# lihzha/lap

Hardware: AMD Instinct MI355X
Metric: train-step samples/sec LAP-3B bf16 (higher is better)
Workload: dtype bf16; 1 GPU; LAP-3B (SigLIP So400m/14 + Gemma-2B + Gemma-300M expert) full train step fwd+bwd+AdamW+EMA, 2x224x224 images + 48-token prompt + 50-step action chunk, random-init weights; global_batch=32, per_gpu_batch=32, seq_len=610, parallelism=single

## Files before the change

include/lap_hip.h:

```cpp
#ifndef LAP_HIP_H_
#define LAP_HIP_H_
#include <stdint.h>

#ifdef __cplusplus
extern "C" {
#endif

#define LAP_ABI_VERSION 1
int lap_abi_version(void);

#define LAP_GEMM_OUT_F32  1
#define LAP_GEMM_ACCUM    2
#define LAP_GEMM_GELU     4
#define LAP_GEMM_BIAS_F32 8
#define LAP_GEMM_GELU_BF16 32
#define LAP_GEMM_GELU_EXP2 128
#define LAP_GEMM_GEGLU    64
#define LAP_GEMM_PARTIALS 16

int lap_gemm_bf16(const void* A, const void* B, void* C, const void* bias, const void* residual,
                  int M, int N, int K, int lda, int ldb, int ldc, int ldr, float alpha,
                  int a_kc, int b_kc, int flags, void* stream);

int lap_gemm_asm_ok(int a_kc, int b_kc, int out_f32, int M, int N, int K, int lda, int ldb, int ldc);
int lap_gemm_asm(const void* A, const void* B, void* C, int M, int N, int K, int lda, int ldb, int ldc, int a_kc, int b_kc,
                 int out_f32, void* stream);
int lap_gemm_asm_bias_ok(int M, int N, int K, int lda, int ldb, int ldc);
int lap_gemm_asm_bias(const void* A, const void* B, void* C, const float* bias, int M, int N, int K, int lda, int ldb, int ldc,
                      void* stream);
int lap_gemm_asm_res_ok(int biased, int M, int N, int K, int lda, int ldb, int ldc);
int lap_gemm_asm_res(const void* A, const void* B, void* C, const float* bias, const void* residual, int M, int N, int K,
                     int lda, int ldb, int ldc, void* stream);
int lap_gemm_asm_geglu_bwd_ok(int M, int N, int K, int lda, int ldb, int ld);
int lap_gemm_asm_geglu_bwd(const void* dy, const void* W, void* dgu, const void* gu, int M, int N, int K, int lda, int ldb, int ld,
                           void* stream);
int lap_gemm_asm_geglu_fwd_ok(int M, int N, int K, int lda, int ldb, int ld_gu, int ld_act);
int lap_gemm_asm_geglu_fwd(const void* x, const void* W, void* gu, void* act, int M, int N, int K, int lda, int ldb, int ld_gu,
                           int ld_act, void* stream);
int lap_gemm_asm_wgrad(const void* A, const void* B, void* C, int M, int N, int K, int lda, int ldb, int ldc, float* sumsq, void* stream);
int lap_gemm_wgrad_f32(const void* A, const void* B, void* C, int M, int N, int K, int lda, int ldb, int ldc, float* sumsq, int* folded,
                       void* scratch, long long scratch_bytes, void* stream);
int lap_gemm_asm_wgrad_b16(const void* A, const void* B, void* C, int M, int N, int K, int lda, int ldb, int ldc, float* sumsq, void* stream);
int lap_gemm_wgrad_bf16(const void* A, const void* B, void* C, int M, int N, int K, int lda, int ldb, int ldc, float* sumsq, int* folded,
                        void* scratch, long long scratch_bytes, void* stream);
int lap_gemm_asm_bias_gelu(const void* x, const void* W, void* h, void* a, const float* bias, int M, int N, int K, int lda, int ldb,
                           int ldc, void* stream);
int lap_gemm_asm_gelu_bwd(const void* dy, const void* W, void* dh, const void* h, int M, int N, int K, int lda, int ldb, int ld,
                          void* stream);

int lap_gemm_asm_launch_counts(long long* counts, int n);
#define LAP_ROUTE_NO_ASM           1
#define LAP_ROUTE_NO_ASM_NN        2
#define LAP_ROUTE_NO_ASM_RES       4
#define LAP_ROUTE_NO_MSPLIT        8
#define LAP_ROUTE_NO_MSPLIT_LONGK  16
#define LAP_ROUTE_NO_NSPLIT        32
#define LAP_ROUTE_NO_SERVING_TILES 64
#define LAP_ROUTE_NO_PINGPONG      128
#define LAP_ROUTE_NO_KTAIL         256
#define LAP_ROUTE_WGRAD_SUMSQ      65536
#define LAP_LEG_ASM             32
#define LAP_LEG_ASM_BIAS        33
#define LAP_LEG_ASM_RES         34
#define LAP_LEG_ASM_WGRAD_SUMSQ 35
#define LAP_LEG_REDUCE_NONE   0
#define LAP_LEG_REDUCE_SPLITK 1
#define LAP_LEG_REDUCE_TAIL   2
#define LAP_GEMM_MAX_LEGS 6
typedef struct lap_gemm_leg {
  long long off_a, off_b, off_c, off_bias, off_res;
  int engine, M, N;
  int ksplit, tile_base, tile_count, sub256, part_compact;
  int f32_tile;
  int part;
  int reduce;
} lap_gemm_leg;
int lap_gemm_plan(const void* A, const void* B, const void* C, const void* bias, const void* residual,
                  int M, int N, int K, int lda, int ldb, int ldc, int ldr, float alpha,
                  int a_kc, int b_kc, int flags, int tile, int ksplit, const void* scratch, long long scratch_bytes,
                  unsigned switches, lap_gemm_leg* legs, int max_legs, int* n_legs);
int lap_gemm_set_debug(int bits);

int lap_gemm_bf16_ex(const void* A, const void* B, void* C, const void* bias, const void* residual,
                     int M, int N, int K, int lda, int ldb, int ldc, int ldr, float alpha,
                     int a_kc, int b_kc, int flags, int tile, int ksplit, void* scratch, long long scratch_bytes,
                     void* stream);

int lap_gemm_f32(const float* A, const float* B, float* C, const float* bias,
                 int M, int N, int K, int lda, int ldb, int ldc, float alpha,
                 int a_kc, int b_kc, int accum, void* stream);

int lap_rmsnorm_fwd(const void* x, const float* scale, const void* mod, void* y, float* rstd,
                    int rows, int D, int rows_per_sample, int mod_ld, float eps, void* stream);
int lap_rmsnorm_bwd(const void* x, const float* scale, const void* mod, const float* rstd, const void* dy,
                    void* dx, float* dscale, float* dmod,
                    int rows, int D, int rows_per_sample, int mod_ld, int dmod_ld, int accum_dx, void* stream);

int lap_layernorm_fwd(const void* x, const float* gamma, const float* beta, void* y, float* mean, float* rstd,
                      int rows, int D, float eps, void* stream);
int lap_layernorm_bwd(const void* x, const float* gamma, const float* mean, const float* rstd, const void* dy,
                      void* dx, float* dgamma, float* dbeta, int rows, int D, int accum_dx, void* stream);
int lap_layernorm_bwd_sum(const void* x, const float* gamma, const float* mean, const float* rstd, const void* dy,
                          void* dx, float* dgamma, float* dbeta, float* dxsum, int rows, int D, int accum_dx, void* stream);

int lap_rope_split_fwd(const void* qkv, const int32_t* pos, void* q, void* k, void* v,
                       int B, int T_seg, int T_total, int seg_off, int NH, int HD, float q_scale, void* stream);
int lap_rope_split_bwd(const void* dq, const void* dk, const void* dv, const int32_t* pos, void* dqkv,
                       int B, int T_seg, int T_total, int seg_off, int NH, int HD, float q_scale, void* stream);

int lap_geglu_fwd(const void* gu, void* act, int rows, int H, void* stream);
int lap_geglu_bwd(const void* gu, const void* dact, void* dgu, int rows, int H, void* stream);
int lap_geglu_fwd_ld(const void* gu, void* act, int rows, int H, int ld_gu, int ld_act, void* stream);
int lap_geglu_bwd_ld(const void* gu, const void* dact, void* dgu, int rows, int H, int ld_gu, int ld_dact, int ld_dgu, void* stream);
int lap_gelu_fwd(const void* x, void* y, long long n, void* stream);
int lap_gelu_bwd(const void* x, const void* dy, void* dx, long long n, void* stream);

int lap_embed_gather(const float* table, const int32_t* tok, void* out, int rows, int T, int D,
                     int dst_rows_per_sample, int dst_off, float scale, int row_lo, int row_hi, void* stream);
int lap_embed_scatter_add(float* dtable, const int32_t* tok, const void* dout, int rows, int T, int D,
                          int src_rows_per_sample, int src_off, float scale, void* stream);

int lap_gated_residual_fwd(const void* x, const void* u, const void* gate, void* y,
                           int rows, int D, int rows_per_sample, int ldg, void* stream);
int lap_gated_residual_bwd(const void* dy, const void* u, const void* gate, void* du, float* dgate,
                           int rows, int D, int rows_per_sample, int ldg, int ldg_out, void* stream);

int lap_colsum_bf16(const void* x, float* out, int rows, int cols, int ld, void* stream);
int lap_colsum_f32(const float* x, float* out, int rows, int cols, int ld, void* stream);

int lap_cast_f32_to_bf16(const float* x, void* y, long long n, void* stream);
int lap_split_f32_hilo(const float* x, int rows, int cols, int ld, void* hi, void* lo, int ld_out, void* stream);
int lap_cast_bf16_to_f32(const void* x, float* y, long long n, void* stream);
int lap_add_bf16(const void* a, const void* b, void* y, long long n, void* stream);
int lap_copy2d_bf16(const void* src, void* dst, int rows, int cols, int lds, int ldd, void* stream);
int lap_copy_rows_bf16(const void* src, void* dst, int rows, int T, int D,
                       int src_rps, int src_off, int dst_rps, int dst_off, int accumulate, void* stream);

int lap_im2col_patch(const float* img, float* out, int B, int H, int W, int C, int P, void* stream);
int lap_augment_images(const float* img, float* out, const float* params, int B, int H, int W, void* stream);
int lap_add_posemb_cast(const float* x, const float* pos, void* y, int rows, int T, int D, void* stream);
int lap_add_posemb_cast_bwd(const void* dy, float* dx, float* dpos, int rows, int T, int D, void* stream);

typedef struct {
  const void* q[2]; void* o[2];
  const void* k[2]; const void* v[2];
  int q_len[2]; int k_len[2];
  int q_rs[2]; int kv_rs[2]; int o_rs[2];
  const int32_t* qinfo; const int32_t* kinfo;
  float* lse;
  float* scratch;
  long long scratch_floats;
  float scale;
  int nsplit;
  int B, NH, NKV, HD;
} lap_attn_fwd_args;
int lap_attention_fwd(const lap_attn_fwd_args* a, void* stream);
int lap_attention_serve_splits(int k_len0, int k_len1, int B, int NH, int q_len1);
int lap_attention_serve(const lap_attn_fwd_args* a, void* stream);

#define LAP_CHAIN_MAX_DEPTH 32
typedef struct {
  int depth, B, S, D, H, NH, HD, prefix_len;
  const void* x_in; void* x_out;
  const void* mod; int mod_slot_stride;
  const void* wqkv[LAP_CHAIN_MAX_DEPTH]; const void* wo[LAP_CHAIN_MAX_DEPTH];
  const void* wgu[LAP_CHAIN_MAX_DEPTH]; const void* wd[LAP_CHAIN_MAX_DEPTH];
  const void* cache_k[LAP_CHAIN_MAX_DEPTH]; const void* cache_v[LAP_CHAIN_MAX_DEPTH];
  int kv_rs;
  const float* rope_table; const int32_t* qinfo; const int32_t* kinfo;
  float q_scale, eps;
  void *q, *k, *v, *o, *xa, *act;
  float* attn_scratch; long long attn_scratch_floats;
  unsigned* counters;
  void* debug_clock;
  int packed;
  void* xs;
  float* tp_slabs;
  void *tp_xs, *tp_xn;
  void *tp_k, *tp_v;
} lap_serve_chain_args;
int lap_serve_chain_ok(int B, int S, int D, int H, int NH, int HD, int NKV, int prefix_len);
int lap_serve_chain_tp_ok(int B, int S, int D, int H, int NH, int HD, int NKV, int prefix_len);
int lap_serve_chain_counter_words(void);
int lap_serve_chain_status(const unsigned* counters, int* status);
int lap_serve_chain(const lap_serve_chain_args* a, void* stream);
int lap_serve_pack_weight(const void* w, void* out, int N, int K, int kind, int HD, void* stream);

typedef struct {
  const void* q[2]; const void* o[2]; const void* d_o[2];
  const void* k[2]; const void* v[2];
  void* dq[2]; void* dk[2]; void* dv[2];
  int q_len[2]; int k_len[2];
  int q_rs[2]; int kv_rs[2]; int o_rs[2];
  const int32_t* qinfo; const int32_t* kinfo;
  const float* lse;
  float* delta;
  float* scratch;
  long long scratch_floats;
  float scale;
  int hsplit;
  int B, NH, NKV, HD;
  int stop_q1_to_k0;
} lap_attn_bwd_args;
int lap_attention_bwd(const lap_attn_bwd_args* a, void* stream);
int lap_attention_set_variant(int variant);

int lap_gemm_fp8(const void* A8, const void* B8, void* C, const void* residual, const float* scale_a, const float* scale_b,
                 int M, int N, int K, int lda, int ldb, int ldc, int ldr, float alpha, int flags, void* stream);
int lap_amax_bf16(const void* x, long long rows, int cols, long long ld, float* amax, void* stream);
int lap_quantize_fp8(const void* x, long long rows, int cols, long long ld, const float* amax, void* out8, long long ldo,
                     float* scale, void* stream);
int lap_quantize_fp8_weight(const void* w, int rows, int cols, const float* amax, void* out8, void* out8_t, float* scale,
                            void* stream);

int lap_serve_qkv_rope(const void* x, const void* mod, int mod_ld, int rows_per_sample, const void* wqkv,
                       const float* rope_table, void* q, void* k, void* v, int M, int D, int NH, int HD, float q_scale,
                       float eps, void* stream);
int lap_serve_gate_up(const void* x, const void* mod, int mod_ld, int rows_per_sample, const void* wgu, void* act, int M,
                      int D, int H, float eps, void* stream);
// ... 125 lines not shown
```

lap_amd/csrc/elementwise.hip:

```cpp
#include <cstdlib>

#include "common.hpp"
#include "../../include/lap_hip.h"

namespace {

__device__ __forceinline__ void ld8(const bf16* p, float (&v)[8]) {
  bf16x8 t = *reinterpret_cast<const bf16x8*>(p);
#pragma unroll
  for (int e = 0; e < 8; ++e) v[e] = (float)t[e];
}
__device__ __forceinline__ void st8(bf16* p, const float (&v)[8]) {
  bf16x8 t;
#pragma unroll
  for (int e = 0; e < 8; ++e) t[e] = f2bf(v[e]);
  *reinterpret_cast<bf16x8*>(p) = t;
}

template <bool NT>
__device__ __forceinline__ void ld8s(const bf16* p, float (&v)[8]) {
  bf16x8 t = NT ? __builtin_nontemporal_load(reinterpret_cast<const bf16x8*>(p)) : *reinterpret_cast<const bf16x8*>(p);
#pragma unroll
  for (int e = 0; e < 8; ++e) v[e] = (float)t[e];
}
template <bool NT>
__device__ __forceinline__ void st8s(bf16* p, const float (&v)[8]) {
  bf16x8 t;
#pragma unroll
  for (int e = 0; e < 8; ++e) t[e] = f2bf(v[e]);
  if (NT) __builtin_nontemporal_store(t, reinterpret_cast<bf16x8*>(p));
  else *reinterpret_cast<bf16x8*>(p) = t;
}

inline bool stream_nt() {
  static const bool nt = getenv("LAP_STREAM_NT") ? atoi(getenv("LAP_STREAM_NT")) != 0 : true;
  return nt;
}

inline dim3 flat_grid(long long n, int per_block = 256) { return dim3((unsigned)((n + per_block - 1) / per_block)); }

template <bool BWD, bool HSPLIT = false>
__global__ __launch_bounds__(256) void rope_split_kernel(const bf16* __restrict__ a0, const bf16* __restrict__ a1,
                                                         const bf16* __restrict__ a2, const int32_t* __restrict__ pos,
                                                         bf16* __restrict__ o0, bf16* __restrict__ o1,
                                                         bf16* __restrict__ o2, int rows, int T_seg, int T_total,
                                                         int seg_off, int NH, int HD, float q_scale) {
  const int cph = HD / 16;
  long long gid = (long long)blockIdx.x * 256 + threadIdx.x;
  int h_lo = 0, h_hi = NH + 2;
  if (HSPLIT) {
    if (gid >= (long long)rows * cph * (NH + 2)) return;
    h_lo = (int)(gid % (NH + 2)); h_hi = h_lo + 1;
    gid /= (NH + 2);
  } else if (gid >= (long long)rows * cph) {
    return;
  }
  const int row = (int)(gid / cph);
  const int c = (int)(gid % cph);
  const int b = row / T_seg, t = row % T_seg;
  const int W = (NH + 2) * HD;
  const int half = HD / 2;
  const float p = (float)pos[(long long)b * T_total + seg_off + t];
  float sn[8], cs[8];
#pragma unroll
  for (int e = 0; e < 8; ++e) rope_sincos(p, c * 8 + e, HD, sn[e], cs[e]);
#pragma unroll 2
  for (int h = h_lo; h < h_hi; ++h) {
    const bf16* src;
    if (!BWD) src = a0 + (long long)row * W + h * HD;
    else if (h < NH) src = a0 + (long long)row * NH * HD + h * HD;
    else if (h == NH) src = a1 + (long long)row * HD;
    else src = a2 + (long long)row * HD;
    float x1[8], x2[8], y1[8], y2[8];
    ld8(src + c * 8, x1);
    ld8(src + half + c * 8, x2);
    if (h <= NH) {
#pragma unroll
      for (int e = 0; e < 8; ++e) {
        if (!BWD) {
          float r1, r2;
          rope_rotate(x1[e], x2[e], sn[e], cs[e], r1, r2);
          r1 = round_bf16((r1)); r2 = round_bf16((r2));
          if (h < NH) { r1 *= q_scale; r2 *= q_scale; }
          y1[e] = r1; y2[e] = r2;
        } else {
          float d1 = x1[e], d2 = x2[e];
          if (h < NH) { d1 *= q_scale; d2 *= q_scale; }
          rope_rotate(d1, d2, -sn[e], cs[e], y1[e], y2[e]);
        }
      }
    } else {
#pragma unroll
      for (int e = 0; e < 8; ++e) { y1[e] = x1[e]; y2[e] = x2[e]; }
    }
    bf16* dst;
    if (BWD) dst = o0 + (long long)row * W + h * HD;
    else if (h < NH) dst = o0 + (long long)row * NH * HD + h * HD;
    else if (h == NH) dst = o1 + (long long)row * HD;
    else dst = o2 + (long long)row * HD;
    st8(dst + c * 8, y1);
    st8(dst + half + c * 8, y2);
  }
}

template <bool NT>
__global__ __launch_bounds__(256) void geglu_fwd_kernel(const bf16* __restrict__ gu, bf16* __restrict__ act,
                                                        long long nchunk, int H8, long long ld_gu, long long ld_act) {
  const long long gid = (long long)blockIdx.x * 256 + threadIdx.x;
  if (gid >= nchunk) return;
  const long long row = gid / H8;
  const int c = (int)(gid % H8) * 8;
  const long long H = (long long)H8 * 8;
  float g[8], u[8], o[8];
  ld8s<NT>(gu + row * ld_gu + c, g);
  ld8s<NT>(gu + row * ld_gu + H + c, u);
#pragma unroll
  for (int e = 0; e < 8; ++e) o[e] = round_bf16((gelu_tanh_f(g[e]))) * u[e];
  st8s<NT>(act + row * ld_act + c, o);
}
template <bool NT>
__global__ __launch_bounds__(256) void geglu_bwd_kernel(const bf16* __restrict__ gu, const bf16* __restrict__ dact,
                                                        bf16* __restrict__ dgu, long long nchunk, int H8, long long ld_gu,
                                                        long long ld_act, long long ld_dgu) {
  const long long gid = (long long)blockIdx.x * 256 + threadIdx.x;
  if (gid >= nchunk) return;
  const long long row = gid / H8;
  const int c = (int)(gid % H8) * 8;
  const long long H = (long long)H8 * 8;
  float g[8], u[8], d[8], dg[8], du[8];
  ld8s<NT>(gu + row * ld_gu + c, g);
  ld8s<NT>(gu + row * ld_gu + H + c, u);
  ld8s<NT>(dact + row * ld_act + c, d);
#pragma unroll
  for (int e = 0; e < 8; ++e) {
    dg[e] = d[e] * u[e] * gelu_tanh_grad_f(g[e]);
    du[e] = d[e] * round_bf16((gelu_tanh_f(g[e])));
  }
  st8s<NT>(dgu + row * ld_dgu + c, dg);
  st8s<NT>(dgu + row * ld_dgu + H + c, du);
}

template <bool NT>
__global__ __launch_bounds__(256) void gelu_fwd_kernel(const bf16* __restrict__ x, bf16* __restrict__ y, long long n8) {
  const long long gid = (long long)blockIdx.x * 256 + threadIdx.x;
  if (gid >= n8) return;
  float v[8];
  ld8s<NT>(x + gid * 8, v);
#pragma unroll
  for (int e = 0; e < 8; ++e) v[e] = gelu_tanh_f(v[e]);
  st8s<NT>(y + gid * 8, v);
}
template <bool NT>
__global__ __launch_bounds__(256) void gelu_bwd_kernel(const bf16* __restrict__ x, const bf16* __restrict__ dy,
                                                       bf16* __restrict__ dx, long long n8) {
  const long long gid = (long long)blockIdx.x * 256 + threadIdx.x;
  if (gid >= n8) return;
  float v[8], d[8];
  ld8s<NT>(x + gid * 8, v);
  ld8s<NT>(dy + gid * 8, d);
#pragma unroll
  for (int e = 0; e < 8; ++e) d[e] *= gelu_tanh_grad_f(v[e]);
  st8s<NT>(dx + gid * 8, d);
}

__global__ __launch_bounds__(256) void embed_gather_kernel(const float* __restrict__ table, const int32_t* __restrict__ tok,
                                                           bf16* __restrict__ out, int rows, int T, int D8,
                                                           int dst_rps, int dst_off, float scale, int row_lo, int row_hi) {
  const long long gid = (long long)blockIdx.x * 256 + threadIdx.x;
  if (gid >= (long long)rows * D8) return;
  const int r = (int)(gid / D8), c = (int)(gid % D8) * 8;
  const long long D = (long long)D8 * 8;
  const int t = tok[r];
  float o[8] = {0.f, 0.f, 0.f, 0.f, 0.f, 0.f, 0.f, 0.f};
  if (t >= row_lo && t < row_hi) {
    const float* src = table + (long long)(t - row_lo) * D + c;
    f32x4 a = *reinterpret_cast<const f32x4*>(src), b = *reinterpret_cast<const f32x4*>(src + 4);
#pragma unroll
    for (int e = 0; e < 4; ++e) { o[e] = a[e] * scale; o[4 + e] = b[e] * scale; }
  }
  const long long drow = (long long)(r / T) * dst_rps + dst_off + r % T;
// ... 69 lines not shown
        if (t < rps) {
          const long long r = (long long)b * rps + t;
          float o[8];
#pragma unroll
          for (int e = 0; e < 8; ++e) { const float d = (float)dv[i][e]; o[e] = d * gv[e]; acc[e] += d * (float)uv[i][e]; }
          st8(du + r * D + c, o);
        }
      }
    }
  }
#pragma unroll
  for (int e = 0; e < 8; ++e) part[rl][cl][e] = acc[e];
  __syncthreads();
  if (rl == 0 && live) {
#pragma unroll
    for (int e = 0; e < 8; ++e) {
      float t = 0.f;
#pragma unroll
      for (int j = 0; j < 8; ++j) t += part[j][cl][e];
      dgate[(long long)b * ldg_out + c + e] = t;
    }
  }
}

__global__ __launch_bounds__(256) void cast_f32_bf16_kernel(const float* __restrict__ x, bf16* __restrict__ y, long long n) {
  const long long i = ((long long)blockIdx.x * 256 + threadIdx.x) * 8;
  if (i + 8 <= n) {
    f32x4 a = *reinterpret_cast<const f32x4*>(x + i), b = *reinterpret_cast<const f32x4*>(x + i + 4);
    float o[8] = {a[0], a[1], a[2], a[3], b[0], b[1], b[2], b[3]};
    st8(y + i, o);
  } else {
    for (long long j = i; j < n; ++j) y[j] = f2bf(x[j]);
  }
}
__global__ __launch_bounds__(256) void split_hilo_kernel(const float* __restrict__ x, int rows, int cols, int ld,
                                                         bf16* __restrict__ hi, bf16* __restrict__ lo, int ld_out) {
  const int cpr = ld_out / 8;
  const long long gid = (long long)blockIdx.x * 256 + threadIdx.x;
  if (gid >= (long long)rows * cpr) return;
  const int r = (int)(gid / cpr), c0 = (int)(gid % cpr) * 8;
  float h[8], l[8];
#pragma unroll
  for (int e = 0; e < 8; ++e) {
    const float v = (c0 + e < cols) ? x[(long long)r * ld + c0 + e] : 0.f;
    h[e] = round_bf16(v);
    l[e] = v - h[e];
  }
  st8(hi + (long long)r * ld_out + c0, h);
  st8(lo + (long long)r * ld_out + c0, l);
}
__global__ __launch_bounds__(256) void cast_bf16_f32_kernel(const bf16* __restrict__ x, float* __restrict__ y, long long n) {
  const long long i = ((long long)blockIdx.x * 256 + threadIdx.x) * 8;
  if (i + 8 <= n) {
    float v[8];
    ld8(x + i, v);
    *reinterpret_cast<f32x4*>(y + i) = f32x4{v[0], v[1], v[2], v[3]};
    *reinterpret_cast<f32x4*>(y + i + 4) = f32x4{v[4], v[5], v[6], v[7]};
  } else {
    for (long long j = i; j < n; ++j) y[j] = bf2f(x[j]);
  }
}
__global__ __launch_bounds__(256) void add_bf16_kernel(const bf16* __restrict__ a, const bf16* __restrict__ b,
                                                       bf16* __restrict__ y, long long n) {
  const long long i = ((long long)blockIdx.x * 256 + threadIdx.x) * 8;
  if (i + 8 <= n) {
    float u[8], v[8];
    ld8(a + i, u); ld8(b + i, v);
#pragma unroll
    for (int e = 0; e < 8; ++e) u[e] += v[e];
    st8(y + i, u);
  } else {
    for (long long j = i; j < n; ++j) y[j] = f2bf(bf2f(a[j]) + bf2f(b[j]));
  }
}
__global__ __launch_bounds__(256) void copy2d_kernel(const bf16* __restrict__ src, bf16* __restrict__ dst, int rows,
                                                     int cols8, int lds_, int ldd) {
  const long long gid = (long long)blockIdx.x * 256 + threadIdx.x;
  if (gid >= (long long)rows * cols8) return;
  const int r = (int)(gid / cols8), c = (int)(gid % cols8) * 8;
  *reinterpret_cast<bf16x8*>(dst + (long long)r * ldd + c) = *reinterpret_cast<const bf16x8*>(src + (long long)r * lds_ + c);
}
__global__ __launch_bounds__(256) void copy_rows_kernel(const bf16* __restrict__ src, bf16* __restrict__ dst, int rows,
                                                        int T, int D8, int src_rps, int src_off, int dst_rps,
                                                        int dst_off, int accumulate) {
  const long long gid = (long long)blockIdx.x * 256 + threadIdx.x;
  if (gid >= (long long)rows * D8) return;
  const int r = (int)(gid / D8), c = (int)(gid % D8) * 8;
  const long long D = (long long)D8 * 8;
  const long long srow = (long long)(r / T) * src_rps + src_off + r % T;
  const long long drow = (long long)(r / T) * dst_rps + dst_off + r % T;
  if (accumulate) {
    float a[8], b[8];
    ld8(src + srow * D + c, a);
    ld8(dst + drow * D + c, b);
#pragma unroll
    for (int e = 0; e < 8; ++e) a[e] += b[e];
    st8(dst + drow * D + c, a);
  } else {
    *reinterpret_cast<bf16x8*>(dst + drow * D + c) = *reinterpret_cast<const bf16x8*>(src + srow * D + c);
  }
}

constexpr int CS_ROWS = 256;
template <typename T>
__global__ __launch_bounds__(256) void colsum_kernel(const T* __restrict__ x, float* __restrict__ out, int rows, int cols,
                                                     int ld) {
  __shared__ float red[4][512];
  const int lane = threadIdx.x & 63, w = threadIdx.x >> 6;
  const int c0 = blockIdx.x * 512 + lane * 8;
  const int r0 = blockIdx.y * CS_ROWS, r1 = min(rows, r0 + CS_ROWS);
  float acc[8] = {0.f, 0.f, 0.f, 0.f, 0.f, 0.f, 0.f, 0.f};
  const bool vec = (c0 + 8 <= cols) && ((ld * (int)sizeof(T)) % 16 == 0) && ((((uintptr_t)x) & 15) == 0) && (c0 * (int)sizeof(T)) % 16 == 0;
  if (vec) {
    for (int r = r0 + w; r < r1; r += 32) {
      if constexpr (sizeof(T) == 2) {
        bf16x8 v[8];
#pragma unroll
        for (int u = 0; u < 8; ++u) {
          const int rr = r + 4 * u;
          v[u] = rr < r1 ? *reinterpret_cast<const bf16x8*>(x + (long long)rr * ld + c0) : bf16x8{0, 0, 0, 0, 0, 0, 0, 0};
        }
#pragma unroll
        for (int u = 0; u < 8; ++u)
#pragma unroll
          for (int e = 0; e < 8; ++e) acc[e] += (float)v[u][e];
      } else {
        f32x4 a[8], b[8];
#pragma unroll
        for (int u = 0; u < 8; ++u) {
          const int rr = r + 4 * u;
          const bool ok = rr < r1;
          a[u] = ok ? *reinterpret_cast<const f32x4*>(x + (long long)rr * ld + c0) : f32x4{0.f, 0.f, 0.f, 0.f};
          b[u] = ok ? *reinterpret_cast<const f32x4*>(x + (long long)rr * ld + c0 + 4) : f32x4{0.f, 0.f, 0.f, 0.f};
        }
#pragma unroll
        for (int u = 0; u < 8; ++u)
#pragma unroll
          for (int e = 0; e < 4; ++e) { acc[e] += a[u][e]; acc[4 + e] += b[u][e]; }
      }
    }
  } else {
    for (int r = r0 + w; r < r1; r += 4) {
      const T* row = x + (long long)r * ld;
#pragma unroll
      for (int e = 0; e < 8; ++e)
        if (c0 + e < cols) acc[e] += (float)row[c0 + e];
    }
  }
#pragma unroll
  for (int e = 0; e < 8; ++e) red[w][lane * 8 + e] = acc[e];
  __syncthreads();
  for (int c = threadIdx.x; c < 512; c += 256) {
    const int col = blockIdx.x * 512 + c;
    if (col < cols) atomicAdd(out + col, red[0][c] + red[1][c] + red[2][c] + red[3][c]);
  }
}

__global__ __launch_bounds__(256) void im2col_kernel(const float* __restrict__ img, float* __restrict__ out, int B, int H,
                                                     int W, int C, int P) {
  const int GH = H / P, GW = W / P;
  const int PC = P * C;
  const long long total = (long long)B * GH * GW * P * PC;
  const long long gid = (long long)blockIdx.x * 256 + threadIdx.x;
  if (gid >= total) return;
  const int x = (int)(gid % PC);
  long long t = gid / PC;
  const int ph = (int)(t % P); t /= P;
  const int gw = (int)(t % GW); t /= GW;
  const int gh = (int)(t % GH);
  const int b = (int)(t / GH);
  out[gid] = img[(((long long)b * H + gh * P + ph) * W + gw * P) * C + x];
}
// ... 77 lines not shown
  const float cf = coef ? coef[b] : 0.f;
  float acc = 0.f;
  for (int i = threadIdx.x; i < n_per; i += 256) {
    const float d = v[(long long)b * n_per + i] - u[(long long)b * n_per + i];
    acc += d * d;
    if (dv) dv[(long long)b * n_per + i] = cf * 2.0f * d / (float)n_per;
  }
  acc = block_sum<4>(acc, red);
  if (threadIdx.x == 0) per_sample[b] = acc / (float)n_per;
}
__global__ __launch_bounds__(256) void axpy_kernel(float* __restrict__ x, const float* __restrict__ v, float dt, long long n) {
  const long long i = (long long)blockIdx.x * 256 + threadIdx.x;
  if (i < n) x[i] += dt * v[i];
}

__device__ __forceinline__ float aug_brightness(float v, float b) { return b < 0.f ? v * (1.f + b) : v * (1.f - b) + b; }
__device__ __forceinline__ float aug_contrast(float v, float c) {
  const float slant = tanf((c + 1.f) * 0.78539816339744831f);
  if (fabsf(slant - 1.f) < 1e-6f) return v;
  const float p1 = (slant - slant * slant) / (2.f * (1.f - slant * slant)), p2 = 1.f - p1;
  if (v < p1) return v / slant;
  if (v > p2) return v / slant + 1.f - 1.f / slant;
  return slant * (v - 0.5f) + 0.5f;
}
__global__ __launch_bounds__(256) void augment_kernel(const float* __restrict__ img, float* __restrict__ out,
                                                      const float* __restrict__ par, int B, int H, int W) {
  const long long gid = (long long)blockIdx.x * 256 + threadIdx.x;
  if (gid >= (long long)B * H * W) return;
  const int x = (int)(gid % W), y = (int)((gid / W) % H), b = (int)(gid / ((long long)W * H));
  const float* q = par + b * 12;
  const float* src = img + (long long)b * H * W * 3;
  float* dst = out + gid * 3;
  if (q[9] != 0.f) {
    const float* s3 = src + ((long long)y * W + x) * 3;
    dst[0] = s3[0]; dst[1] = s3[1]; dst[2] = s3[2];
    return;
  }
  const float xc = (float)x + 0.5f - 0.5f * (float)W, yc = (float)y + 0.5f - 0.5f * (float)H;
  const float xr = q[4] * xc - q[5] * yc, yr = q[5] * xc + q[4] * yc;
  const float xs = q[0] + 0.5f * q[2] + xr * (q[2] / (float)W) - 0.5f;
  const float ys = q[1] + 0.5f * q[3] + yr * (q[3] / (float)H) - 0.5f;
  const float xf = floorf(xs), yf = floorf(ys);
  const int x0 = (int)xf, y0 = (int)yf;
  const float ax = xs - xf, ay = ys - yf;
  float px[3] = {0.f, 0.f, 0.f};
#pragma unroll
  for (int dy = 0; dy < 2; ++dy)
#pragma unroll
    for (int dx = 0; dx < 2; ++dx) {
      const int xx = x0 + dx, yy = y0 + dy;
      if (xx < 0 || xx >= W || yy < 0 || yy >= H) continue;
      const float wgt = (dx ? ax : 1.f - ax) * (dy ? ay : 1.f - ay);
      const float* s3 = src + ((long long)yy * W + xx) * 3;
#pragma unroll
      for (int c = 0; c < 3; ++c) px[c] += wgt * (s3[c] * 0.5f + 0.5f);
    }
  float r = px[0], g = px[1], bl = px[2];
  r = aug_brightness(r, q[6]); g = aug_brightness(g, q[6]); bl = aug_brightness(bl, q[6]);
  r = aug_contrast(r, q[7]); g = aug_contrast(g, q[7]); bl = aug_contrast(bl, q[7]);
  {
    const float mx = fmaxf(r, fmaxf(g, bl)), mn = fminf(r, fminf(g, bl));
    const float sat = mx > 0.f ? (mx - mn) / mx : 0.f;
    const float s2 = fminf(fmaxf(aug_brightness(sat, q[8]), 0.f), 1.f);
    const float k = sat > 0.f ? s2 / sat : 0.f;
    r = mx - (mx - r) * k; g = mx - (mx - g) * k; bl = mx - (mx - bl) * k;
  }
  dst[0] = fminf(fmaxf(r, 0.f), 1.f) * 2.f - 1.f;
  dst[1] = fminf(fmaxf(g, 0.f), 1.f) * 2.f - 1.f;
  dst[2] = fminf(fmaxf(bl, 0.f), 1.f) * 2.f - 1.f;
}

}

#define S_ ((hipStream_t)stream)

extern "C" int lap_abi_version(void) { return LAP_ABI_VERSION; }

extern "C" int lap_rope_split_fwd(const void* qkv, const int32_t* pos, void* q, void* k, void* v, int B, int T_seg,
                                  int T_total, int seg_off, int NH, int HD, float q_scale, void* stream) {
  if (B <= 0 || T_seg <= 0 || (HD & 15) || NH <= 0) return LAP_ERR_ARG;
  const long long n = (long long)B * T_seg * (HD / 16);
  if (n < 65536)
    hipLaunchKernelGGL((rope_split_kernel<false, true>), flat_grid(n * (NH + 2)), dim3(256), 0, S_, (const bf16*)qkv, nullptr, nullptr, pos,
                       (bf16*)q, (bf16*)k, (bf16*)v, B * T_seg, T_seg, T_total, seg_off, NH, HD, q_scale);
  else
    hipLaunchKernelGGL(rope_split_kernel<false>, flat_grid(n), dim3(256), 0, S_, (const bf16*)qkv, nullptr, nullptr, pos,
                       (bf16*)q, (bf16*)k, (bf16*)v, B * T_seg, T_seg, T_total, seg_off, NH, HD, q_scale);
  LAP_CHECK_LAUNCH();
  return LAP_OK;
}
extern "C" int lap_rope_split_bwd(const void* dq, const void* dk, const void* dv, const int32_t* pos, void* dqkv, int B,
                                  int T_seg, int T_total, int seg_off, int NH, int HD, float q_scale, void* stream) {
  if (B <= 0 || T_seg <= 0 || (HD & 15) || NH <= 0) return LAP_ERR_ARG;
  const long long n = (long long)B * T_seg * (HD / 16);
  hipLaunchKernelGGL(rope_split_kernel<true>, flat_grid(n), dim3(256), 0, S_, (const bf16*)dq, (const bf16*)dk,
                     (const bf16*)dv, pos, (bf16*)dqkv, nullptr, nullptr, B * T_seg, T_seg, T_total, seg_off, NH, HD,
                     q_scale);
  LAP_CHECK_LAUNCH();
  return LAP_OK;
}

extern "C" int lap_geglu_fwd_ld(const void* gu, void* act, int rows, int H, int ld_gu, int ld_act, void* stream) {
  if (rows <= 0 || H <= 0 || (H & 7) || ld_gu < 2 * H || ld_act < H || (ld_gu & 7) || (ld_act & 7)) return LAP_ERR_ARG;
  const long long n = (long long)rows * (H / 8);
  const bool nt = stream_nt();
  if (nt) hipLaunchKernelGGL(geglu_fwd_kernel<true>, flat_grid(n), dim3(256), 0, S_, (const bf16*)gu, (bf16*)act, n, H / 8, (long long)ld_gu, (long long)ld_act);
  else hipLaunchKernelGGL(geglu_fwd_kernel<false>, flat_grid(n), dim3(256), 0, S_, (const bf16*)gu, (bf16*)act, n, H / 8, (long long)ld_gu, (long long)ld_act);
  LAP_CHECK_LAUNCH();
  return LAP_OK;
}
extern "C" int lap_geglu_fwd(const void* gu, void* act, int rows, int H, void* stream) {
  return lap_geglu_fwd_ld(gu, act, rows, H, 2 * H, H, stream);
}
extern "C" int lap_geglu_bwd_ld(const void* gu, const void* dact, void* dgu, int rows, int H, int ld_gu, int ld_dact, int ld_dgu, void* stream) {
  if (rows <= 0 || H <= 0 || (H & 7) || ld_gu < 2 * H || ld_dact < H || ld_dgu < 2 * H || ((ld_gu | ld_dact | ld_dgu) & 7)) return LAP_ERR_ARG;
  const long long n = (long long)rows * (H / 8);
  const bool nt = stream_nt();
  if (nt) hipLaunchKernelGGL(geglu_bwd_kernel<true>, flat_grid(n), dim3(256), 0, S_, (const bf16*)gu, (const bf16*)dact, (bf16*)dgu, n,
                             H / 8, (long long)ld_gu, (long long)ld_dact, (long long)ld_dgu);
  else hipLaunchKernelGGL(geglu_bwd_kernel<false>, flat_grid(n), dim3(256), 0, S_, (const bf16*)gu, (const bf16*)dact, (bf16*)dgu, n,
                          H / 8, (long long)ld_gu, (long long)ld_dact, (long long)ld_dgu);
  LAP_CHECK_LAUNCH();
  return LAP_OK;
}
extern "C" int lap_geglu_bwd(const void* gu, const void* dact, void* dgu, int rows, int H, void* stream) {
  return lap_geglu_bwd_ld(gu, dact, dgu, rows, H, 2 * H, H, 2 * H, stream);
}
extern "C" int lap_gelu_fwd(const void* x, void* y, long long n, void* stream) {
  if (n <= 0 || (n & 7)) return LAP_ERR_ARG;
  if (stream_nt()) hipLaunchKernelGGL(gelu_fwd_kernel<true>, flat_grid(n / 8), dim3(256), 0, S_, (const bf16*)x, (bf16*)y, n / 8);
  else hipLaunchKernelGGL(gelu_fwd_kernel<false>, flat_grid(n / 8), dim3(256), 0, S_, (const bf16*)x, (bf16*)y, n / 8);
  LAP_CHECK_LAUNCH();
  return LAP_OK;
}
extern "C" int lap_gelu_bwd(const void* x, const void* dy, void* dx, long long n, void* stream) {
  if (n <= 0 || (n & 7)) return LAP_ERR_ARG;
  if (stream_nt()) hipLaunchKernelGGL(gelu_bwd_kernel<true>, flat_grid(n / 8), dim3(256), 0, S_, (const bf16*)x, (const bf16*)dy, (bf16*)dx, n / 8);
  else hipLaunchKernelGGL(gelu_bwd_kernel<false>, flat_grid(n / 8), dim3(256), 0, S_, (const bf16*)x, (const bf16*)dy, (bf16*)dx, n / 8);
  LAP_CHECK_LAUNCH();
  return LAP_OK;
}

extern "C" int lap_embed_gather(const float* table, const int32_t* tok, void* out, int rows, int T, int D,
                                int dst_rows_per_sample, int dst_off, float scale, int row_lo, int row_hi, void* stream) {
  if (rows <= 0 || T <= 0 || (D & 7) || row_hi < row_lo) return LAP_ERR_ARG;
  hipLaunchKernelGGL(embed_gather_kernel, flat_grid((long long)rows * (D / 8)), dim3(256), 0, S_, table, tok, (bf16*)out,
                     rows, T, D / 8, dst_rows_per_sample, dst_off, scale, row_lo, row_hi);
  LAP_CHECK_LAUNCH();
  return LAP_OK;
}
extern "C" int lap_embed_scatter_add(float* dtable, const int32_t* tok, const void* dout, int rows, int T, int D,
                                     int src_rows_per_sample, int src_off, float scale, void* stream) {
  if (rows <= 0 || T <= 0 || (D & 7)) return LAP_ERR_ARG;
  hipLaunchKernelGGL(embed_scatter_kernel, flat_grid((long long)rows * (D / 8)), dim3(256), 0, S_, dtable, tok,
                     (const bf16*)dout, rows, T, D / 8, src_rows_per_sample, src_off, scale);
  LAP_CHECK_LAUNCH();
  return LAP_OK;
}

extern "C" int lap_gated_residual_fwd(const void* x, const void* u, const void* gate, void* y, int rows, int D,
                                      int rows_per_sample, int ldg, void* stream) {
  if (rows <= 0 || (D & 7) || (gate && (rows_per_sample <= 0 || (ldg & 7)))) return LAP_ERR_ARG;
  hipLaunchKernelGGL(gated_res_fwd_kernel, flat_grid((long long)rows * (D / 8)), dim3(256), 0, S_, (const bf16*)x,
                     (const bf16*)u, (const bf16*)gate, (bf16*)y, rows, D / 8, rows_per_sample > 0 ? rows_per_sample : 1,
                     ldg);
  LAP_CHECK_LAUNCH();
  return LAP_OK;
}
extern "C" int lap_gated_residual_bwd(const void* dy, const void* u, const void* gate, void* du, float* dgate, int rows,
                                      int D, int rows_per_sample, int ldg, int ldg_out, void* stream) {
  if (rows <= 0 || (D & 7) || !gate || rows_per_sample <= 0 || rows % rows_per_sample || (ldg & 7)) return LAP_ERR_ARG;
  dim3 grid((D / 8 + 31) / 32, rows / rows_per_sample);
  hipLaunchKernelGGL(gated_res_bwd_kernel, grid, dim3(256), 0, S_, (const bf16*)dy, (const bf16*)u, (const bf16*)gate,
                     (bf16*)du, dgate, D / 8, rows_per_sample, ldg, ldg_out);
  LAP_CHECK_LAUNCH();
  return LAP_OK;
}

extern "C" int lap_colsum_bf16(const void* x, float* out, int rows, int cols, int ld, void* stream) {
  if (rows <= 0 || cols <= 0) return LAP_ERR_ARG;
  hipLaunchKernelGGL(colsum_kernel<bf16>, dim3((cols + 511) / 512, (rows + CS_ROWS - 1) / CS_ROWS), dim3(256), 0, S_, (const bf16*)x,
                     out, rows, cols, ld);
  LAP_CHECK_LAUNCH();
  return LAP_OK;
}
extern "C" int lap_colsum_f32(const float* x, float* out, int rows, int cols, int ld, void* stream) {
  if (rows <= 0 || cols <= 0) return LAP_ERR_ARG;
  hipLaunchKernelGGL(colsum_kernel<float>, dim3((cols + 511) / 512, (rows + CS_ROWS - 1) / CS_ROWS), dim3(256), 0, S_, x, out, rows,
                     cols, ld);
  LAP_CHECK_LAUNCH();
  return LAP_OK;
}

extern "C" int lap_cast_f32_to_bf16(const float* x, void* y, long long n, void* stream) {
  if (n <= 0) return LAP_ERR_ARG;
  hipLaunchKernelGGL(cast_f32_bf16_kernel, flat_grid((n + 7) / 8), dim3(256), 0, S_, x, (bf16*)y, n);
  LAP_CHECK_LAUNCH();
  return LAP_OK;
}
extern "C" int lap_split_f32_hilo(const float* x, int rows, int cols, int ld, void* hi, void* lo, int ld_out, void* stream) {
  if (rows <= 0 || cols <= 0 || ld < cols || ld_out < cols || (ld_out & 7) || !x || !hi || !lo) return LAP_ERR_ARG;
  hipLaunchKernelGGL(split_hilo_kernel, flat_grid((long long)rows * (ld_out / 8)), dim3(256), 0, S_, x, rows, cols, ld, (bf16*)hi,
                     (bf16*)lo, ld_out);
  LAP_CHECK_LAUNCH();
  return LAP_OK;
}
extern "C" int lap_cast_bf16_to_f32(const void* x, float* y, long long n, void* stream) {
  if (n <= 0) return LAP_ERR_ARG;
  hipLaunchKernelGGL(cast_bf16_f32_kernel, flat_grid((n + 7) / 8), dim3(256), 0, S_, (const bf16*)x, y, n);
  LAP_CHECK_LAUNCH();
  return LAP_OK;
}
extern "C" int lap_add_bf16(const void* a, const void* b, void* y, long long n, void* stream) {
  if (n <= 0) return LAP_ERR_ARG;
  hipLaunchKernelGGL(add_bf16_kernel, flat_grid((n + 7) / 8), dim3(256), 0, S_, (const bf16*)a, (const bf16*)b, (bf16*)y,
                     n);
  LAP_CHECK_LAUNCH();
  return LAP_OK;
}
extern "C" int lap_copy2d_bf16(const void* src, void* dst, int rows, int cols, int lds, int ldd, void* stream) {
  if (rows <= 0 || cols <= 0 || (cols & 7) || (lds & 7) || (ldd & 7)) return LAP_ERR_ARG;
  hipLaunchKernelGGL(copy2d_kernel, flat_grid((long long)rows * (cols / 8)), dim3(256), 0, S_, (const bf16*)src,
                     (bf16*)dst, rows, cols / 8, lds, ldd);
  LAP_CHECK_LAUNCH();
  return LAP_OK;
}
extern "C" int lap_copy_rows_bf16(const void* src, void* dst, int rows, int T, int D, int src_rps, int src_off,
                                  int dst_rps, int dst_off, int accumulate, void* stream) {
  if (rows <= 0 || T <= 0 || (D & 7)) return LAP_ERR_ARG;
  hipLaunchKernelGGL(copy_rows_kernel, flat_grid((long long)rows * (D / 8)), dim3(256), 0, S_, (const bf16*)src,
                     (bf16*)dst, rows, T, D / 8, src_rps, src_off, dst_rps, dst_off, accumulate);
  LAP_CHECK_LAUNCH();
  return LAP_OK;
}

extern "C" int lap_im2col_patch(const float* img, float* out, int B, int H, int W, int C, int P, void* stream) {
  if (B <= 0 || P <= 0 || H % P || W % P) return LAP_ERR_ARG;
  const long long n = (long long)B * H * W * C;
  hipLaunchKernelGGL(im2col_kernel, flat_grid(n), dim3(256), 0, S_, img, out, B, H, W, C, P);
  LAP_CHECK_LAUNCH();
  return LAP_OK;
}
extern "C" int lap_augment_images(const float* img, float* out, const float* params, int B, int H, int W, void* stream) {
  if (!img || !out || !params || img == out || B <= 0 || H <= 0 || W <= 0) return LAP_ERR_ARG;
  hipLaunchKernelGGL(augment_kernel, flat_grid((long long)B * H * W), dim3(256), 0, S_, img, out, params, B, H, W);
  LAP_CHECK_LAUNCH();
  return LAP_OK;
}
extern "C" int lap_add_posemb_cast(const float* x, const float* pos, void* y, int rows, int T, int D, void* stream) {
  if (rows <= 0 || T <= 0 || (D & 7)) return LAP_ERR_ARG;
  hipLaunchKernelGGL(add_posemb_cast_kernel, flat_grid((long long)rows * (D / 8)), dim3(256), 0, S_, x, pos, (bf16*)y,
                     rows, T, D / 8);
  LAP_CHECK_LAUNCH();
  return LAP_OK;
}
extern "C" int lap_add_posemb_cast_bwd(const void* dy, float* dx, float* dpos, int rows, int T, int D, void* stream) {
  if (rows <= 0 || T <= 0 || rows % T || (D & 7)) return LAP_ERR_ARG;
  dim3 grid((D / 8 + 255) / 256, T);
  hipLaunchKernelGGL(add_posemb_cast_bwd_kernel, grid, dim3(256), 0, S_, (const bf16*)dy, dx, dpos, rows / T, T, D / 8);
  LAP_CHECK_LAUNCH();
  return LAP_OK;
}

extern "C" int lap_fm_mix(const float* noise, const float* actions, const float* t, float* x_t, float* u_t, int B,
                          int n_per, void* stream) {
  if (B <= 0 || n_per <= 0) return LAP_ERR_ARG;
  hipLaunchKernelGGL(fm_mix_kernel, flat_grid((long long)B * n_per), dim3(256), 0, S_, noise, actions, t, x_t, u_t, B,
                     n_per);
  LAP_CHECK_LAUNCH();
  return LAP_OK;
}
extern "C" int lap_posemb_sincos(const float* t, float* out, int B, int D, float min_period, float max_period,
                                 void* stream) {
  if (B <= 0 || D <= 0 || (D & 1)) return LAP_ERR_ARG;
  hipLaunchKernelGGL(posemb_sincos_kernel, flat_grid((long long)B * (D / 2)), dim3(256), 0, S_, t, out, B, D, min_period,
                     max_period);
  LAP_CHECK_LAUNCH();
  return LAP_OK;
}
extern "C" int lap_swish_fwd(const float* x, float* y, long long n, void* stream) {
  if (n <= 0) return LAP_ERR_ARG;
  hipLaunchKernelGGL(swish_fwd_kernel, flat_grid(n), dim3(256), 0, S_, x, y, n);
  LAP_CHECK_LAUNCH();
  return LAP_OK;
}
extern "C" int lap_swish_bwd(const float* x, const float* dy, float* dx, long long n, void* stream) {
  if (n <= 0) return LAP_ERR_ARG;
  hipLaunchKernelGGL(swish_bwd_kernel, flat_grid(n), dim3(256), 0, S_, x, dy, dx, n);
  LAP_CHECK_LAUNCH();
  return LAP_OK;
}
extern "C" int lap_mse_fwd_bwd(const float* v, const float* u, const float* coef, float* per_sample, float* dv, int B,
                               int n_per, void* stream) {
  if (B <= 0 || n_per <= 0) return LAP_ERR_ARG;
  hipLaunchKernelGGL(mse_kernel, dim3(B), dim3(256), 0, S_, v, u, coef, per_sample, dv, n_per);
  LAP_CHECK_LAUNCH();
  return LAP_OK;
}
extern "C" int lap_axpy_f32(float* x, const float* v, float dt, long long n, void* stream) {
  if (n <= 0) return LAP_ERR_ARG;
  hipLaunchKernelGGL(axpy_kernel, flat_grid(n), dim3(256), 0, S_, x, v, dt, n);
  LAP_CHECK_LAUNCH();
  return LAP_OK;
}
```

lap_amd/csrc/norm.hip:

```cpp
#include <cstdlib>

#include "common.hpp"
#include "../../include/lap_hip.h"

namespace {

constexpr int NWAVE = 4;

__device__ __forceinline__ void load8(const bf16* p, float (&v)[8]) {
  bf16x8 t = *reinterpret_cast<const bf16x8*>(p);
#pragma unroll
  for (int e = 0; e < 8; ++e) v[e] = (float)t[e];
}
__device__ __forceinline__ void store8(bf16* p, const float (&v)[8]) {
  bf16x8 t;
#pragma unroll
  for (int e = 0; e < 8; ++e) t[e] = f2bf(v[e]);
  *reinterpret_cast<bf16x8*>(p) = t;
}

template <int NCH>
__global__ __launch_bounds__(256) void rmsnorm_fwd_kernel(const bf16* __restrict__ x, const float* __restrict__ scale,
                                                          const bf16* __restrict__ mod, bf16* __restrict__ y,
                                                          float* __restrict__ rstd_out, int rows, int D,
                                                          int rows_per_sample, int mod_ld, float eps) {
  const int lane = threadIdx.x & 63, w = threadIdx.x >> 6;
  const int row = blockIdx.x * NWAVE + w;
  if (row >= rows) return;
  const bf16* xr = x + (long long)row * D;
  float xv[NCH][8];
  float ss = 0.f;
#pragma unroll
  for (int p = 0; p < NCH; ++p) {
    const int c = (lane + 64 * p) * 8;
    if (c < D) {
      load8(xr + c, xv[p]);
#pragma unroll
      for (int e = 0; e < 8; ++e) ss += xv[p][e] * xv[p][e];
    }
  }
  ss = wave_sum(ss);
  const float r = 1.0f / sqrtf(ss / (float)D + eps);
  if (rstd_out && lane == 0) rstd_out[row] = r;
  const bf16* mrow = mod ? mod + (long long)(row / rows_per_sample) * mod_ld : nullptr;
  bf16* yr = y + (long long)row * D;
#pragma unroll
  for (int p = 0; p < NCH; ++p) {
    const int c = (lane + 64 * p) * 8;
    if (c < D) {
      float o[8];
      if (mrow) {
        float sc[8], sh[8];
        load8(mrow + c, sc);
        load8(mrow + D + c, sh);
#pragma unroll
        for (int e = 0; e < 8; ++e) o[e] = xv[p][e] * r * round_bf16((1.0f + sc[e])) + sh[e];
      } else {
#pragma unroll
        for (int e = 0; e < 8; ++e) o[e] = xv[p][e] * r * (1.0f + scale[c + e]);
      }
      store8(yr + c, o);
    }
  }
}

template <int NCH>
__global__ __launch_bounds__(256) void rmsnorm_bwd_kernel(const bf16* __restrict__ x, const float* __restrict__ scale,
                                                          const bf16* __restrict__ mod, const float* __restrict__ rstd,
                                                          const bf16* __restrict__ dy, bf16* __restrict__ dx,
                                                          float* __restrict__ dscale, float* __restrict__ dmod,
                                                          int rows, int D, int G, int mod_ld, int dmod_ld,
                                                          int accum_dx) {
  extern __shared__ __attribute__((aligned(16))) float red[];
  const int lane = threadIdx.x & 63, w = threadIdx.x >> 6;
  const int g = blockIdx.x;
  const int r0 = g * G, r1 = min(rows, r0 + G);
  const bool ada = mod != nullptr;
  const bf16* mrow = ada ? mod + (long long)g * mod_ld : nullptr;

  float wgt[NCH][8];
  float ds[NCH][8], dh[NCH][8];
#pragma unroll
  for (int p = 0; p < NCH; ++p) {
    const int c = (lane + 64 * p) * 8;
#pragma unroll
    for (int e = 0; e < 8; ++e) { ds[p][e] = 0.f; dh[p][e] = 0.f; wgt[p][e] = 0.f; }
    if (c < D) {
      if (ada) {
        float sc[8];
        load8(mrow + c, sc);
#pragma unroll
        for (int e = 0; e < 8; ++e) wgt[p][e] = round_bf16((1.0f + sc[e]));
      } else {
#pragma unroll
        for (int e = 0; e < 8; ++e) wgt[p][e] = 1.0f + scale[c + e];
      }
    }
  }
  bf16x8 nx[NCH], ndy[NCH];
  float nr = 0.f;
  auto fetch = [&](int row) {
#pragma unroll
    for (int p = 0; p < NCH; ++p) {
      const int c = (lane + 64 * p) * 8;
      if (c < D) {
        nx[p] = *reinterpret_cast<const bf16x8*>(x + (long long)row * D + c);
        ndy[p] = *reinterpret_cast<const bf16x8*>(dy + (long long)row * D + c);
      }
    }
    nr = rstd[row];
  };
  if (r0 + w < r1) fetch(r0 + w);
  for (int row = r0 + w; row < r1; row += NWAVE) {
    bf16x8 cx[NCH], cdy[NCH], cold[NCH];
#pragma unroll
    for (int p = 0; p < NCH; ++p) {
      cx[p] = nx[p]; cdy[p] = ndy[p];
      const int c = (lane + 64 * p) * 8;
      if (NCH <= 3 && accum_dx && c < D) cold[p] = *reinterpret_cast<const bf16x8*>(dx + (long long)row * D + c);
    }
    const float r = nr;
    if (row + NWAVE < r1) fetch(row + NWAVE);
    float xv[NCH][8], gv[NCH][8];
    float dot = 0.f;
#pragma unroll
    for (int p = 0; p < NCH; ++p) {
      const int c = (lane + 64 * p) * 8;
      if (c < D) {
        float dyv[8];
#pragma unroll
        for (int e = 0; e < 8; ++e) { xv[p][e] = (float)cx[p][e]; dyv[e] = (float)cdy[p][e]; }
#pragma unroll
        for (int e = 0; e < 8; ++e) {
          gv[p][e] = dyv[e] * wgt[p][e];
          dot += gv[p][e] * xv[p][e];
          ds[p][e] += dyv[e] * xv[p][e] * r;
          dh[p][e] += dyv[e];
        }
      }
    }
    dot = wave_sum(dot);
    const float cc = dot * r * r * r / (float)D;
    bf16* dxr = dx + (long long)row * D;
#pragma unroll
    for (int p = 0; p < NCH; ++p) {
      const int c = (lane + 64 * p) * 8;
      if (c < D) {
        float o[8];
#pragma unroll
        for (int e = 0; e < 8; ++e) o[e] = r * gv[p][e] - xv[p][e] * cc;
        if (accum_dx) {
          if constexpr (NCH > 3) cold[p] = *reinterpret_cast<const bf16x8*>(dxr + c);
#pragma unroll
          for (int e = 0; e < 8; ++e) o[e] += (float)cold[p][e];
        }
        store8(dxr + c, o);
      }
    }
  }
  const int stride = ada ? 2 * D : D;
#pragma unroll
  for (int p = 0; p < NCH; ++p) {
    const int c = (lane + 64 * p) * 8;
    if (c < D) {
#pragma unroll
      for (int e = 0; e < 8; ++e) {
        red[w * stride + c + e] = ds[p][e];
        if (ada) red[w * stride + D + c + e] = dh[p][e];
      }
    }
  }
  __syncthreads();
  for (int c = threadIdx.x; c < stride; c += 256) {
    float t = 0.f;
#pragma unroll
    for (int i = 0; i < NWAVE; ++i) t += red[i * stride + c];
    if (ada) {
      atomicAdd(dmod + (long long)g * dmod_ld + c, t);
    } else {
      atomicAdd(dscale + c, t);
    }
  }
}

template <int NCH>
__global__ __launch_bounds__(256) void layernorm_fwd_kernel(const bf16* __restrict__ x, const float* __restrict__ gamma,
                                                            const float* __restrict__ beta, bf16* __restrict__ y,
                                                            float* __restrict__ mean_out, float* __restrict__ rstd_out,
                                                            int rows, int D, float eps) {
  const int lane = threadIdx.x & 63, w = threadIdx.x >> 6;
  const int row = blockIdx.x * NWAVE + w;
  if (row >= rows) return;
  const bf16* xr = x + (long long)row * D;
  float xv[NCH][8];
  float s = 0.f, ss = 0.f;
#pragma unroll
  for (int p = 0; p < NCH; ++p) {
    const int c = (lane + 64 * p) * 8;
    if (c < D) {
      load8(xr + c, xv[p]);
#pragma unroll
      for (int e = 0; e < 8; ++e) { s += xv[p][e]; ss += xv[p][e] * xv[p][e]; }
    }
  }
  s = wave_sum(s);
  ss = wave_sum(ss);
  const float mean = s / (float)D;
  const float var = fmaxf(ss / (float)D - mean * mean, 0.f);
  const float r = 1.0f / sqrtf(var + eps);
  if (lane == 0) {
    if (mean_out) mean_out[row] = mean;
    if (rstd_out) rstd_out[row] = r;
  }
  bf16* yr = y + (long long)row * D;
#pragma unroll
  for (int p = 0; p < NCH; ++p) {
    const int c = (lane + 64 * p) * 8;
    if (c < D) {
      float o[8];
#pragma unroll
      for (int e = 0; e < 8; ++e) o[e] = (xv[p][e] - mean) * (r * gamma[c + e]) + beta[c + e];
      store8(yr + c, o);
    }
  }
}

template <int NCH>
__global__ __launch_bounds__(256) void layernorm_bwd_kernel(const bf16* __restrict__ x, const float* __restrict__ gamma,
                                                            const float* __restrict__ mean, const float* __restrict__ rstd,
                                                            const bf16* __restrict__ dy, bf16* __restrict__ dx,
                                                            float* __restrict__ dgamma, float* __restrict__ dbeta,
                                                            int rows, int D, int G, int accum_dx, float* __restrict__ dxsum) {
  extern __shared__ __attribute__((aligned(16))) float red[];
  const int lane = threadIdx.x & 63, w = threadIdx.x >> 6;
  const int r0 = blockIdx.x * G, r1 = min(rows, r0 + G);
// ... 52 lines not shown
    s2 = wave_sum(s2) / (float)D;
    bf16* dxr = dx + (long long)row * D;
#pragma unroll
    for (int p = 0; p < NCH; ++p) {
      const int c = (lane + 64 * p) * 8;
      if (c < D) {
        float o[8];
#pragma unroll
        for (int e = 0; e < 8; ++e) o[e] = r * (gv[p][e] - s1 - xh[p][e] * s2);
        if (accum_dx) {
          if constexpr (NCH > 3) cold[p] = *reinterpret_cast<const bf16x8*>(dxr + c);
#pragma unroll
          for (int e = 0; e < 8; ++e) o[e] += (float)cold[p][e];
        }
        store8(dxr + c, o);
        if (dxsum) {
#pragma unroll
          for (int e = 0; e < 8; ++e) dxs[p][e] += (float)f2bf(o[e]);
        }
      }
    }
  }
  const int NS = dxsum ? 3 : 2;
#pragma unroll
  for (int p = 0; p < NCH; ++p) {
    const int c = (lane + 64 * p) * 8;
    if (c < D) {
#pragma unroll
      for (int e = 0; e < 8; ++e) {
        red[w * NS * D + c + e] = dg[p][e];
        red[w * NS * D + D + c + e] = db[p][e];
        if (dxsum) red[w * NS * D + 2 * D + c + e] = dxs[p][e];
      }
    }
  }
  __syncthreads();
  for (int c = threadIdx.x; c < NS * D; c += 256) {
    float t = 0.f;
#pragma unroll
    for (int i = 0; i < NWAVE; ++i) t += red[i * NS * D + c];
    if (c < D) atomicAdd(dgamma + c, t);
    else if (c < 2 * D) atomicAdd(dbeta + (c - D), t);
    else atomicAdd(dxsum + (c - 2 * D), t);
  }
}

inline int nch_for(int D) { return (D / 8 + 63) / 64; }

}

#define DISPATCH_NCH(D, CALL)                          \
  switch (nch_for(D)) {                                \
    case 1: { constexpr int NCH = 1; CALL; } break;    \
    case 2: { constexpr int NCH = 2; CALL; } break;    \
    case 3: { constexpr int NCH = 3; CALL; } break;    \
    case 4: { constexpr int NCH = 4; CALL; } break;    \
    default: return LAP_ERR_ARG;                       \
  }

extern "C" int lap_rmsnorm_fwd(const void* x, const float* scale, const void* mod, void* y, float* rstd,
                               int rows, int D, int rows_per_sample, int mod_ld, float eps, void* stream) {
  if (rows <= 0 || D <= 0 || (D & 7) || (!scale && !mod) || (mod && (rows_per_sample <= 0 || (mod_ld & 7) || (mod_ld != 0 && mod_ld < 3 * D))))
    return LAP_ERR_ARG;
  hipStream_t s = (hipStream_t)stream;
  dim3 grid((rows + NWAVE - 1) / NWAVE);
  DISPATCH_NCH(D, hipLaunchKernelGGL(rmsnorm_fwd_kernel<NCH>, grid, dim3(256), 0, s, (const bf16*)x, scale,
                                     (const bf16*)mod, (bf16*)y, rstd, rows, D, rows_per_sample, mod_ld, eps));
  LAP_CHECK_LAUNCH();
  return LAP_OK;
}

extern "C" int lap_rmsnorm_bwd(const void* x, const float* scale, const void* mod, const float* rstd, const void* dy,
                               void* dx, float* dscale, float* dmod, int rows, int D, int rows_per_sample,
                               int mod_ld, int dmod_ld, int accum_dx, void* stream) {
  if (rows <= 0 || D <= 0 || (D & 7) || !rstd) return LAP_ERR_ARG;
  if (mod ? (!dmod || rows_per_sample <= 0 || rows % rows_per_sample) : (!scale || !dscale)) return LAP_ERR_ARG;
  hipStream_t s = (hipStream_t)stream;
  static const int g_env = getenv("LAP_NORM_BWD_ROWS") ? atoi(getenv("LAP_NORM_BWD_ROWS")) : 64;
  const int G = mod ? rows_per_sample : g_env;
  dim3 grid((rows + G - 1) / G);
  const size_t shm = (size_t)NWAVE * (mod ? 2 : 1) * D * sizeof(float);
  DISPATCH_NCH(D, hipLaunchKernelGGL(rmsnorm_bwd_kernel<NCH>, grid, dim3(256), shm, s, (const bf16*)x, scale,
                                     (const bf16*)mod, rstd, (const bf16*)dy, (bf16*)dx, dscale, dmod, rows, D, G,
                                     mod_ld, dmod_ld, accum_dx));
  LAP_CHECK_LAUNCH();
  return LAP_OK;
}

extern "C" int lap_layernorm_fwd(const void* x, const float* gamma, const float* beta, void* y, float* mean,
                                 float* rstd, int rows, int D, float eps, void* stream) {
  if (rows <= 0 || D <= 0 || (D & 7) || !gamma || !beta) return LAP_ERR_ARG;
  hipStream_t s = (hipStream_t)stream;
  dim3 grid((rows + NWAVE - 1) / NWAVE);
  DISPATCH_NCH(D, hipLaunchKernelGGL(layernorm_fwd_kernel<NCH>, grid, dim3(256), 0, s, (const bf16*)x, gamma, beta,
                                     (bf16*)y, mean, rstd, rows, D, eps));
  LAP_CHECK_LAUNCH();
  return LAP_OK;
}

extern "C" int lap_layernorm_bwd_sum(const void* x, const float* gamma, const float* mean, const float* rstd,
                                     const void* dy, void* dx, float* dgamma, float* dbeta, float* dxsum, int rows, int D,
                                     int accum_dx, void* stream) {
  if (rows <= 0 || D <= 0 || (D & 7) || !gamma || !mean || !rstd || !dgamma || !dbeta) return LAP_ERR_ARG;
  hipStream_t s = (hipStream_t)stream;
  static const int g_env = getenv("LAP_NORM_BWD_ROWS") ? atoi(getenv("LAP_NORM_BWD_ROWS")) : 32;
  const int G = g_env;
  dim3 grid((rows + G - 1) / G);
  const size_t shm = (size_t)NWAVE * (dxsum ? 3 : 2) * D * sizeof(float);
  if (shm > 64 * 1024) return LAP_ERR_ARG;
  DISPATCH_NCH(D, hipLaunchKernelGGL(layernorm_bwd_kernel<NCH>, grid, dim3(256), shm, s, (const bf16*)x, gamma, mean,
                                     rstd, (const bf16*)dy, (bf16*)dx, dgamma, dbeta, rows, D, G, accum_dx, dxsum));
  LAP_CHECK_LAUNCH();
  return LAP_OK;
}
extern "C" int lap_layernorm_bwd(const void* x, const float* gamma, const float* mean, const float* rstd,
                                 const void* dy, void* dx, float* dgamma, float* dbeta, int rows, int D, int accum_dx,
                                 void* stream) {
  return lap_layernorm_bwd_sum(x, gamma, mean, rstd, dy, dx, dgamma, dbeta, nullptr, rows, D, accum_dx, stream);
}
```

lap_amd/hip.py:

```python
from __future__ import annotations

import ctypes as C
import pathlib

import torch

import os as _os

_LIB_PATH = pathlib.Path(__file__).resolve().parent / (
    f"liblap_hip_{_os.environ['LAP_HIP_LIB_VARIANT']}.so" if _os.environ.get("LAP_HIP_LIB_VARIANT") else "liblap_hip.so")

GEMM_OUT_F32 = 1
GEMM_ACCUM = 2
GEMM_GELU = 4
GEMM_BIAS_F32 = 8
GEMM_PARTIALS = 16
GEMM_GELU_BF16 = 32
GEMM_GELU_EXP2 = 128
GEMM_GEGLU = 64


class LapHipError(RuntimeError):
    pass

# ... 19 lines not shown
        ("q_rs", _i * 2), ("kv_rs", _i * 2), ("o_rs", _i * 2),
        ("qinfo", _vp), ("kinfo", _vp), ("lse", _vp),
        ("scratch", _vp), ("scratch_floats", _ll),
        ("scale", _f), ("nsplit", _i),
        ("B", _i), ("NH", _i), ("NKV", _i), ("HD", _i),
    ]


CHAIN_MAX_DEPTH = 32


class ServeChainArgs(C.Structure):
    _fields_ = [
        ("depth", _i), ("B", _i), ("S", _i), ("D", _i), ("H", _i), ("NH", _i), ("HD", _i), ("prefix_len", _i),
        ("x_in", _vp), ("x_out", _vp),
        ("mod", _vp), ("mod_slot_stride", _i),
        ("wqkv", _vp * CHAIN_MAX_DEPTH), ("wo", _vp * CHAIN_MAX_DEPTH), ("wgu", _vp * CHAIN_MAX_DEPTH), ("wd", _vp * CHAIN_MAX_DEPTH),
        ("cache_k", _vp * CHAIN_MAX_DEPTH), ("cache_v", _vp * CHAIN_MAX_DEPTH),
        ("kv_rs", _i),
        ("rope_table", _vp), ("qinfo", _vp), ("kinfo", _vp),
        ("q_scale", _f), ("eps", _f),
        ("q", _vp), ("k", _vp), ("v", _vp), ("o", _vp), ("xa", _vp), ("act", _vp),
        ("attn_scratch", _vp), ("attn_scratch_floats", _ll),
        ("counters", _vp), ("debug_clock", _vp),
        ("packed", _i), ("xs", _vp),
        ("tp_slabs", _vp), ("tp_xs", _vp), ("tp_xn", _vp), ("tp_k", _vp), ("tp_v", _vp),
    ]


class AttnBwdArgs(C.Structure):
    _fields_ = [
        ("q", _vp * 2), ("o", _vp * 2), ("d_o", _vp * 2), ("k", _vp * 2), ("v", _vp * 2),
        ("dq", _vp * 2), ("dk", _vp * 2), ("dv", _vp * 2),
        ("q_len", _i * 2), ("k_len", _i * 2),
        ("q_rs", _i * 2), ("kv_rs", _i * 2), ("o_rs", _i * 2),
        ("qinfo", _vp), ("kinfo", _vp), ("lse", _vp), ("delta", _vp),
        ("scratch", _vp), ("scratch_floats", _ll),
        ("scale", _f), ("hsplit", _i),
        ("B", _i), ("NH", _i), ("NKV", _i), ("HD", _i), ("stop_q1_to_k0", _i),
    ]


class GemmLeg(C.Structure):
    _fields_ = [(n, _ll) for n in ("off_a", "off_b", "off_c", "off_bias", "off_res")] + [
        (n, _i) for n in ("engine", "M", "N", "ksplit", "tile_base", "tile_count", "sub256", "part_compact", "f32_tile", "part", "reduce")]


GEMM_MAX_LEGS = 6
LEG_ASM, LEG_ASM_BIAS, LEG_ASM_RES, LEG_ASM_WGRAD_SUMSQ = 32, 33, 34, 35
ROUTE_WGRAD_SUMSQ = 65536
ROUTE_SWITCHES = {"LAP_GEMM_NO_ASM": 1, "LAP_GEMM_NO_ASM_NN": 2, "LAP_GEMM_NO_ASM_RES": 4, "LAP_GEMM_NO_MSPLIT": 8, "LAP_GEMM_NO_MSPLIT_LONGK": 16,
                  "LAP_GEMM_NO_NSPLIT": 32, "LAP_GEMM_NO_SERVING_TILES": 64, "LAP_GEMM_NO_PINGPONG": 128, "LAP_GEMM_NO_KTAIL": 256}

SIGNATURES: dict[str, list] = {
    "lap_abi_version": [],
    "lap_gemm_bf16": [_vp, _vp, _vp, _vp, _vp, _i, _i, _i, _i, _i, _i, _i, _f, _i, _i, _i, _vp],
    "lap_gemm_bf16_ex": [_vp, _vp, _vp, _vp, _vp, _i, _i, _i, _i, _i, _i, _i, _f, _i, _i, _i, _i, _i, _vp, _ll, _vp],
    "lap_gemm_set_debug": [_i],
    "lap_gemm_asm": [_vp, _vp, _vp, _i, _i, _i, _i, _i, _i, _i, _i, _i, _vp],
    "lap_gemm_asm_ok": [_i, _i, _i, _i, _i, _i, _i, _i, _i],
    "lap_gemm_asm_launch_counts": [C.POINTER(C.c_longlong), _i],
    "lap_gemm_plan": [_vp, _vp, _vp, _vp, _vp, _i, _i, _i, _i, _i, _i, _i, _f, _i, _i, _i, _i, _i, _vp, _ll, C.c_uint, _vp, _i, C.POINTER(_i)],
    "lap_gemm_asm_bias": [_vp, _vp, _vp, _vp, _i, _i, _i, _i, _i, _i, _vp],
    "lap_gemm_asm_bias_ok": [_i, _i, _i, _i, _i, _i],
    "lap_gemm_asm_res": [_vp, _vp, _vp, _vp, _vp, _i, _i, _i, _i, _i, _i, _vp],
    "lap_gemm_asm_res_ok": [_i, _i, _i, _i, _i, _i, _i],
    "lap_gemm_asm_geglu_bwd": [_vp, _vp, _vp, _vp, _i, _i, _i, _i, _i, _i, _vp],
    "lap_gemm_asm_geglu_bwd_ok": [_i, _i, _i, _i, _i, _i],
    "lap_gemm_asm_geglu_fwd": [_vp, _vp, _vp, _vp, _i, _i, _i, _i, _i, _i, _i, _vp],
    "lap_gemm_asm_geglu_fwd_ok": [_i, _i, _i, _i, _i, _i, _i],
    "lap_gemm_asm_wgrad": [_vp, _vp, _vp, _i, _i, _i, _i, _i, _i, _vp, _vp],
    "lap_gemm_wgrad_f32": [_vp, _vp, _vp, _i, _i, _i, _i, _i, _i, _vp, _vp, _vp, _ll, _vp],
    "lap_gemm_asm_wgrad_b16": [_vp, _vp, _vp, _i, _i, _i, _i, _i, _i, _vp, _vp],
    "lap_gemm_wgrad_bf16": [_vp, _vp, _vp, _i, _i, _i, _i, _i, _i, _vp, _vp, _vp, _ll, _vp],
    "lap_gemm_asm_bias_gelu": [_vp, _vp, _vp, _vp, _vp, _i, _i, _i, _i, _i, _i, _vp],
    "lap_gemm_asm_gelu_bwd": [_vp, _vp, _vp, _vp, _i, _i, _i, _i, _i, _i, _vp],
    "lap_gemm_fp8": [_vp, _vp, _vp, _vp, _vp, _vp, _i, _i, _i, _i, _i, _i, _i, _f, _i, _vp],
    "lap_amax_bf16": [_vp, _ll, _i, _ll, _vp, _vp],
    "lap_quantize_fp8": [_vp, _ll, _i, _ll, _vp, _vp, _ll, _vp, _vp],
    "lap_quantize_fp8_weight": [_vp, _i, _i, _vp, _vp, _vp, _vp, _vp],
    "lap_gemm_f32": [_vp, _vp, _vp, _vp, _i, _i, _i, _i, _i, _i, _f, _i, _i, _i, _vp],
    "lap_rmsnorm_fwd": [_vp, _vp, _vp, _vp, _vp, _i, _i, _i, _i, _f, _vp],
    "lap_rmsnorm_bwd": [_vp, _vp, _vp, _vp, _vp, _vp, _vp, _vp, _i, _i, _i, _i, _i, _i, _vp],
    "lap_layernorm_fwd": [_vp, _vp, _vp, _vp, _vp, _vp, _i, _i, _f, _vp],
    "lap_layernorm_bwd": [_vp, _vp, _vp, _vp, _vp, _vp, _vp, _vp, _i, _i, _i, _vp],
    "lap_layernorm_bwd_sum": [_vp, _vp, _vp, _vp, _vp, _vp, _vp, _vp, _vp, _i, _i, _i, _vp],
    "lap_rope_split_fwd": [_vp, _vp, _vp, _vp, _vp, _i, _i, _i, _i, _i, _i, _f, _vp],
    "lap_rope_split_bwd": [_vp, _vp, _vp, _vp, _vp, _i, _i, _i, _i, _i, _i, _f, _vp],
    "lap_geglu_fwd": [_vp, _vp, _i, _i, _vp],
    "lap_geglu_bwd": [_vp, _vp, _vp, _i, _i, _vp],
    "lap_geglu_fwd_ld": [_vp, _vp, _i, _i, _i, _i, _vp],
    "lap_geglu_bwd_ld": [_vp, _vp, _vp, _i, _i, _i, _i, _i, _vp],
    "lap_gelu_fwd": [_vp, _vp, _ll, _vp],
    "lap_gelu_bwd": [_vp, _vp, _vp, _ll, _vp],
    "lap_embed_gather": [_vp, _vp, _vp, _i, _i, _i, _i, _i, _f, _i, _i, _vp],
    "lap_embed_scatter_add": [_vp, _vp, _vp, _i, _i, _i, _i, _i, _f, _vp],
    "lap_gated_residual_fwd": [_vp, _vp, _vp, _vp, _i, _i, _i, _i, _vp],
    "lap_gated_residual_bwd": [_vp, _vp, _vp, _vp, _vp, _i, _i, _i, _i, _i, _vp],
    "lap_colsum_bf16": [_vp, _vp, _i, _i, _i, _vp],
    "lap_colsum_f32": [_vp, _vp, _i, _i, _i, _vp],
    "lap_cast_f32_to_bf16": [_vp, _vp, _ll, _vp],
    "lap_split_f32_hilo": [_vp, _i, _i, _i, _vp, _vp, _i, _vp],
    "lap_cast_bf16_to_f32": [_vp, _vp, _ll, _vp],
    "lap_add_bf16": [_vp, _vp, _vp, _ll, _vp],
    "lap_copy2d_bf16": [_vp, _vp, _i, _i, _i, _i, _vp],
    "lap_copy_rows_bf16": [_vp, _vp, _i, _i, _i, _i, _i, _i, _i, _i, _vp],
    "lap_im2col_patch": [_vp, _vp, _i, _i, _i, _i, _i, _vp],
    "lap_augment_images": [_vp, _vp, _vp, _i, _i, _i, _vp],
    "lap_add_posemb_cast": [_vp, _vp, _vp, _i, _i, _i, _vp],
    "lap_add_posemb_cast_bwd": [_vp, _vp, _vp, _i, _i, _i, _vp],
    "lap_attention_fwd": [C.POINTER(AttnFwdArgs), _vp],
    "lap_attention_serve_splits": [_i, _i, _i, _i, _i],
    "lap_attention_serve": [C.POINTER(AttnFwdArgs), _vp],
    "lap_attention_bwd": [C.POINTER(AttnBwdArgs), _vp],
    "lap_attention_set_variant": [_i],
    "lap_rope_table": [_vp, _vp, _i, _i, _i, _i, _i, _vp],
    "lap_fused_reduce_rope_split": [_vp, _i, _vp, _vp, _vp, _vp, _vp, _i, _i, _i, _i, _i, _i, _f, _vp],
    "lap_fused_reduce_geglu": [_vp, _i, _vp, _i, _i, _vp],
    "lap_fused_reduce_residual_norm": [_vp, _i, _vp, _vp, _i, _vp, _i, _vp, _vp, _i, _i, _i, _f, _vp],
    "lap_fused_reduce_norm": [_vp, _i, _vp, _vp, _i, _vp, _vp, _vp, _vp, _i, _i, _f, _vp],
    "lap_serve_infos": [C.POINTER(_vp), _i, _i, _vp, _vp, _i, _i, _i, _i, _vp, _vp, _vp, _vp, _vp, _vp, _vp],
    "lap_serve_qkv_rope": [_vp, _vp, _i, _i, _vp, _vp, _vp, _vp, _vp, _i, _i, _i, _i, _f, _f, _vp],
    "lap_serve_gate_up": [_vp, _vp, _i, _i, _vp, _vp, _i, _i, _i, _f, _vp],
    "lap_serve_proj_residual": [_vp, _vp, _vp, _vp, _i, _i, _vp, _i, _i, _i, _vp],
    "lap_serve_set_variant": [_i],
    "lap_serve_embed_actions": [_vp, _vp, _vp, _vp, _i, _i, _i, _vp],
    "lap_serve_chain_ok": [_i, _i, _i, _i, _i, _i, _i, _i],
    "lap_serve_chain_tp_ok": [_i, _i, _i, _i, _i, _i, _i, _i],
    "lap_serve_chain_counter_words": [],
    "lap_serve_chain_status": [_vp, C.POINTER(_i)],
    "lap_serve_chain": [C.POINTER(ServeChainArgs), _vp],
    "lap_serve_pack_weight": [_vp, _vp, _i, _i, _i, _i, _vp],
    "lap_serve_final_euler_embed": [_vp, _vp, _i, _i, _vp, _vp, _vp, _vp, _i, _i, _i, _f, _f, _vp, _vp, _vp, _vp],
    "lap_panel_gemm_ok": [_i, _i, _i, _i],
    "lap_panel_gemm_pf": [_vp, _i, _vp, _vp, _i, _vp, _vp, _i, _i, _vp, _vp, _f, _i, _i, _i, _i, _i, _vp, _i, _vp, _ll, _vp],
    "lap_panel_gemm": [_vp, _i, _vp, _vp, _i, _vp, _vp, _i, _i, _vp, _vp, _f, _i, _i, _i, _i, _i, _vp, _i, _vp],
    "lap_serve_final_euler": [_vp, _vp, _i, _i, _vp, _vp, _vp, _vp, _i, _i, _i, _f, _f, _vp],
    "lap_ce_chunk_update": [_vp, _i, _vp, _vp, _vp, _vp, _i, _i, _i, _vp],
    "lap_ce_chunk_update_argmax": [_vp, _i, _vp, _vp, _vp, _vp, _vp, _i, _i, _i, _vp],
    "lap_token_metrics": [_vp, _vp, _vp, _vp, _i, _vp, _vp, _vp, _vp, _i, _i, _vp, _vp, _vp],
    "lap_ce_chunk_grad": [_vp, _i, _vp, _vp, _vp, _vp, _vp, _i, _i, _i, _i, _vp],
    "lap_ce_chunk_grad_hilo": [_vp, _i, _vp, _vp, _vp, _vp, _vp, _vp, _i, _i, _i, _i, _vp],
    "lap_adamw_ema_hilo": [_vp, _vp, _vp, _vp, _vp, _vp, _vp, _ll, _vp, _f, _f, _f, _f, _f, _vp],
    "lap_sumsq_f32": [_vp, _ll, _vp, _vp],
    "lap_sumsq_bf16": [_vp, _ll, _vp, _vp],
    "lap_adamw_ema_g16": [_vp, _vp, _vp, _vp, _vp, _vp, _ll, _vp, _f, _f, _f, _f, _f, _vp],
    "lap_argmax_rows_f32": [_vp, _i, _i, _i, _vp, _vp],
    "lap_gumbel_argmax_rows_f32": [_vp, _i, _i, _i, _f, C.c_uint, C.c_uint, _i, _vp, _vp],
    "lap_adamw_ema": [_vp, _vp, _vp, _vp, _vp, _vp, _ll, _vp, _f, _f, _f, _f, _f, _vp],
    "lap_fm_mix": [_vp, _vp, _vp, _vp, _vp, _i, _i, _vp],
    "lap_posemb_sincos": [_vp, _vp, _i, _i, _f, _f, _vp],
    "lap_swish_fwd": [_vp, _vp, _ll, _vp],
    "lap_swish_bwd": [_vp, _vp, _vp, _ll, _vp],
    "lap_mse_fwd_bwd": [_vp, _vp, _vp, _vp, _vp, _i, _i, _vp],
    "lap_axpy_f32": [_vp, _vp, _f, _ll, _vp],
    "lap_lora_down": [_vp, _i, _i, _vp, _i, _i, _vp, _i, _i, _i, _i, _i, _f, _vp],
    "lap_lora_up_add": [_vp, _i, _vp, _i, _i, _vp, _i, _i, _i, _i, _i, _f, _vp],
    "lap_lora_wgrad": [_vp, _i, _vp, _i, _i, _vp, _i, _i, _i, _i, _i, _i, _i, _f, _i, _vp, _ll, _vp],
    "lap_lora_merge": [_vp, _i, _vp, _i, _vp, _i, _i, _vp, _i, _i, _i, _i, _i, _f, _vp],
    "lap_decode_ok": [_i, _i, _i, _i, _i, _i, _i],
    "lap_decode_state_words": [],
    "lap_decode_lm_blocks": [],
    "lap_decode_attn_scratch_floats": [_i, _i, _i],
    "lap_decode_init": [_vp, _vp, _vp, _i, _i, _vp],
    "lap_decode_embed": [_vp, _vp, _i, _i, _vp, _i, _vp, _i, _i, _f, _vp],
    "lap_decode_qkv": [_vp, _vp, _vp, _vp, _vp, _vp, _vp, _i, _i, _i, _i, _i, _f, _f, _vp],
    "lap_decode_attention": [_vp, _vp, _vp, _vp, _vp, _i, _vp, _vp, _i, _vp, _vp, _ll, _i, _i, _i, _i, _vp],
    "lap_decode_proj_residual": [_vp, _vp, _vp, _vp, _vp, _i, _i, _i, _i, _vp],
    "lap_decode_gate_up": [_vp, _vp, _vp, _vp, _vp, _i, _i, _i, _f, _vp],
    "lap_decode_lm_head": [_vp, _vp, _vp, _vp, _vp, _i, _i, _i, _f, _vp, _vp, _vp, _vp],
    "lap_decode_finish": [_vp, _vp, _vp, _vp, _i, _i, _i, _vp],
    "lap_decode_sampling_words": [],
    "lap_decode_lm_head_sample": [_vp, _vp, _vp, _vp, _vp, _vp, _i, _i, _i, _f, _vp, _vp, _vp, _vp],
    "lap_quantize_fp8_rows": [_vp, _i, _vp, _vp, _ll, _i, _vp],
    "lap_decode_qkv_fp8": [_vp, _vp, _vp, _vp, _vp, _vp, _vp, _vp, _i, _i, _i, _i, _i, _f, _f, _vp],
    "lap_decode_gate_up_fp8": [_vp, _vp, _vp, _vp, _vp, _vp, _i, _i, _i, _f, _vp],
    "lap_decode_proj_residual_fp8": [_vp, _vp, _vp, _vp, _vp, _vp, _i, _i, _i, _i, _vp],
    "lap_decode_lm_head_fp8": [_vp, _vp, _vp, _vp, _vp, _i, _i, _i, _f, _vp, _vp, _vp, _vp],
    "lap_decode_lm_head_sample_fp8": [_vp, _vp, _vp, _vp, _vp, _vp, _i, _i, _i, _f, _vp, _vp, _vp, _vp],
    "lap_decode_lm_head_subset": [_vp, _vp, _vp, _vp, _vp, _vp, _i, _i, _i, _i, _f, _vp, _vp, _vp, _vp],
    "lap_decode_lm_head_subset_sample": [_vp, _vp, _vp, _vp, _vp, _vp, _vp, _i, _i, _i, _i, _f, _vp, _vp, _vp, _vp],
    "lap_decode_lm_head_subset_fp8": [_vp, _vp, _vp, _vp, _vp, _vp, _i, _i, _i, _i, _f, _vp, _vp, _vp, _vp],
    "lap_decode_lm_head_subset_sample_fp8": [_vp, _vp, _vp, _vp, _vp, _vp, _vp, _i, _i, _i, _i, _f, _vp, _vp, _vp, _vp],
}

_fn = {}
for _name, _args in SIGNATURES.items():
    _f_ = getattr(_lib, _name)
    _f_.argtypes = _args
# ... 100 lines not shown
              residual=None, scratch=None, scratch_bytes=0, switches=0):
    legs, n = (GemmLeg * GEMM_MAX_LEGS)(), _i(0)
    _chk(_fn["lap_gemm_plan"](a, b, c, bias, residual, M, N, K, lda, ldb, ldc, ldr, float(alpha), int(a_kc), int(b_kc), flags, tile, ksplit,
                              scratch, scratch_bytes, switches, legs, GEMM_MAX_LEGS, C.byref(n)), "lap_gemm_plan")
    return list(legs[:n.value])


ASM_KERNELS = ("nt", "nn", "tn", "nt_bias", "tn_t", "nt_res", "nt_bias_res", "nn_geglu_bwd", "nt_geglu", "nn_gelu_bwd", "nt_bias_gelu",
               "tn_b16", "tn_t_b16")


def gemm_asm_launch_counts() -> dict:
    buf = (C.c_longlong * len(ASM_KERNELS))()
    _chk(_fn["lap_gemm_asm_launch_counts"](buf, len(ASM_KERNELS)), "lap_gemm_asm_launch_counts")
    return dict(zip(ASM_KERNELS, (int(v) for v in buf)))


def linear_wgrad_sumsq(dy, x, out, sumsq):
    import ctypes
    Mrows, Nout = dy.shape
    Kin = x.shape[1]
    _req(dy, torch.bfloat16, "dy"); _req(x, torch.bfloat16, "x"); _req(sumsq, torch.float32, "sumsq")
    if out.dtype not in (torch.float32, torch.bfloat16):
        raise TypeError("linear_wgrad_sumsq: out must be f32 or bf16")
    folded = ctypes.c_int(0)
    scratch = _gemm_scratch(dy.device)
    call("lap_gemm_wgrad_f32" if out.dtype == torch.float32 else "lap_gemm_wgrad_bf16", _p(dy), _p(x), _p(out), Nout, Kin, Mrows, dy.stride(0), x.stride(0), out.stride(0), _p(sumsq),
         ctypes.byref(folded), _p(scratch), scratch.numel() * 4)
    return bool(folded.value)


def split_f32_hilo(x, ld_out=None):
    _req(x, torch.float32, "x")
    rows, cols = x.shape
    ld_out = (cols + 7) // 8 * 8 if ld_out is None else ld_out
    hi = torch.empty((rows, ld_out), dtype=torch.bfloat16, device=x.device)
    lo = torch.empty_like(hi)
    call("lap_split_f32_hilo", _p(x), rows, cols, x.stride(0), _p(hi), _p(lo), ld_out)
    return hi, lo


def argmax_rows(x, out=None):
    _req(x, torch.float32, "x")
    if out is None:
        out = torch.empty((x.shape[0],), dtype=torch.int32, device=x.device)
    call("lap_argmax_rows_f32", _p(x), x.shape[0], x.shape[1], x.stride(0), _p(out))
    return out


def sampling_words(seed, temperature):
    from lap_amd.sampling import inverse_temperature

    seed = int(seed) & 0xFFFFFFFFFFFFFFFF
    return seed & 0xFFFFFFFF, seed >> 32, float(inverse_temperature(temperature))


def gumbel_argmax_rows(x, temperature, seed, step, out=None):
    _req(x, torch.float32, "x")
    lo, hi, inv_t = sampling_words(seed, temperature)
    if out is None:
        out = torch.empty((x.shape[0],), dtype=torch.int32, device=x.device)
    call("lap_gumbel_argmax_rows_f32", _p(x), x.shape[0], x.shape[1], x.stride(0), inv_t, lo, hi, int(step), _p(out))
    return out


def gemm_f32(a, b, out, *, M, N, K, lda, ldb, ldc, a_kc=True, b_kc=True, bias=None, alpha=1.0, accum=False):
    for t, n in ((a, "A"), (b, "B"), (out, "C")):
        _req(t, torch.float32, n)
    call("lap_gemm_f32", _p(a), _p(b), _p(out), _p(bias), M, N, K, lda, ldb, ldc, float(alpha), int(a_kc), int(b_kc),
         int(accum))
    return out


def rmsnorm_fwd(x, scale=None, mod=None, rows_per_sample=0, eps=1e-6, save_rstd=True, mod_ld=None):
    rows, D = x.shape
    y = torch.empty_like(x)
    rstd = torch.empty(rows, dtype=torch.float32, device=x.device) if save_rstd else None
    if mod_ld is None:
        mod_ld = mod.stride(0) if mod is not None else 0
    call("lap_rmsnorm_fwd", _p(x), _p(scale), _p(mod), _p(y), _p(rstd), rows, D, rows_per_sample, mod_ld, float(eps))
    return y, rstd


def rmsnorm_bwd(x, dy, rstd, scale=None, mod=None, rows_per_sample=0, dx=None, dscale=None, dmod=None, accum_dx=False):
    rows, D = x.shape
    if dx is None:
        dx = torch.empty_like(x)
    call("lap_rmsnorm_bwd", _p(x), _p(scale), _p(mod), _p(rstd), _p(dy), _p(dx), _p(dscale), _p(dmod), rows, D,
         rows_per_sample, mod.stride(0) if mod is not None else 0, dmod.stride(0) if dmod is not None else 0,
         int(accum_dx))
    return dx


def layernorm_fwd(x, gamma, beta, eps=1e-6):
    rows, D = x.shape
    y = torch.empty_like(x)
    mean = torch.empty(rows, dtype=torch.float32, device=x.device)
    rstd = torch.empty(rows, dtype=torch.float32, device=x.device)
    call("lap_layernorm_fwd", _p(x), _p(gamma), _p(beta), _p(y), _p(mean), _p(rstd), rows, D, float(eps))
    return y, mean, rstd


def layernorm_bwd(x, dy, gamma, mean, rstd, dgamma, dbeta, dx=None, accum_dx=False, dxsum=None):
    rows, D = x.shape
    if dx is None:
        dx = torch.empty_like(x)
    call("lap_layernorm_bwd_sum", _p(x), _p(gamma), _p(mean), _p(rstd), _p(dy), _p(dx), _p(dgamma), _p(dbeta), _p(dxsum), rows, D,
         int(accum_dx))
    return dx


def rope_split_fwd(qkv, pos, B, T_seg, T_total, seg_off, NH, HD, q_scale):
    rows = B * T_seg
    q = torch.empty((rows, NH * HD), dtype=torch.bfloat16, device=qkv.device)
    k = torch.empty((rows, HD), dtype=torch.bfloat16, device=qkv.device)
    v = torch.empty((rows, HD), dtype=torch.bfloat16, device=qkv.device)
    call("lap_rope_split_fwd", _p(qkv), _p(pos), _p(q), _p(k), _p(v), B, T_seg, T_total, seg_off, NH, HD, float(q_scale))
    return q, k, v


def rope_split_bwd(dq, dk, dv, pos, B, T_seg, T_total, seg_off, NH, HD, q_scale):
    dqkv = torch.empty((B * T_seg, (NH + 2) * HD), dtype=torch.bfloat16, device=dq.device)
    call("lap_rope_split_bwd", _p(dq), _p(dk), _p(dv), _p(pos), _p(dqkv), B, T_seg, T_total, seg_off, NH, HD,
         float(q_scale))
    return dqkv


def _padded_rows(rows, cols, device, pad):
    return torch.empty((rows, cols + pad), dtype=torch.bfloat16, device=device)[:, :cols]


def _row_pad(cols):
    return 64 if cols * 2 >= 16384 and (cols * 2) % 16384 == 0 else 0


def geglu_fwd(gu, pad=False):
    rows, H2 = gu.shape
    act = _padded_rows(rows, H2 // 2, gu.device, _row_pad(H2 // 2) if pad else 0)
    call("lap_geglu_fwd_ld", _p(gu), _p(act), rows, H2 // 2, gu.stride(0), act.stride(0))
    return act


def linear_bias_gelu_train_ok(x, wt, bias):
    M, K = x.shape
    N = wt.shape[0]
    return (x.dtype == wt.dtype == torch.bfloat16 and bias is not None and bias.dtype == torch.float32 and x.stride(1) == 1 and wt.stride(1) == 1
            and bool(_lib.lap_gemm_asm_bias_ok(M, N, K, x.stride(0), wt.stride(0), N)))


def linear_bias_gelu_train(x, wt, bias):
    M, K = x.shape
    N = wt.shape[0]
    h = torch.empty((M, N), dtype=torch.bfloat16, device=x.device)
    a = torch.empty((M, N), dtype=torch.bfloat16, device=x.device)
    call("lap_gemm_asm_bias_gelu", _p(x), _p(wt), _p(h), _p(a), _p(bias), M, N, K, x.stride(0), wt.stride(0), N)
    return h, a


def dgrad_gelu_bwd_ok(dy, w, h):
    M, K = dy.shape
    N = w.shape[1]
    return (dy.dtype == w.dtype == h.dtype == torch.bfloat16 and tuple(h.shape) == (M, N) and h.stride(1) == 1 and dy.stride(1) == 1 and w.stride(1) == 1
            and w.shape[0] == K and bool(_lib.lap_gemm_asm_ok(1, 0, 0, M, N, K, dy.stride(0), w.stride(0), h.stride(0))))


def linear_dgrad_gelu_bwd(dy, w, h):
    M, K = dy.shape
    N = w.shape[1]
    if tuple(h.shape) != (M, N) or w.shape[0] != K:
        raise LapHipError(f"linear_dgrad_gelu_bwd: dy {tuple(dy.shape)}, w {tuple(w.shape)}, h {tuple(h.shape)} do not fit")
    dh = torch.empty((M, h.stride(0)), dtype=torch.bfloat16, device=h.device)[:, :N]
    call("lap_gemm_asm_gelu_bwd", _p(dy), _p(w), _p(dh), _p(h), M, N, K, dy.stride(0), w.stride(0), h.stride(0))
    return dh


def linear_geglu_train_ok(x, wgu, pad=True):
    M, K = x.shape
    N = wgu.shape[0]
    p = _row_pad(N) if pad else 0
    pa = _row_pad(N // 2) if pad else 0
    return (x.dtype == wgu.dtype == torch.bfloat16 and x.stride(1) == 1 and wgu.stride(1) == 1 and N % 256 == 0
            and bool(_lib.lap_gemm_asm_geglu_fwd_ok(M, N, K, x.stride(0), wgu.stride(0), N + p, N // 2 + pa)))


def linear_geglu_train(x, wgu, pad=True):
    M, K = x.shape
    N = wgu.shape[0]
    gu = _padded_rows(M, N, x.device, _row_pad(N) if pad else 0)
    act = _padded_rows(M, N // 2, x.device, _row_pad(N // 2) if pad else 0)
    call("lap_gemm_asm_geglu_fwd", _p(x), _p(wgu), _p(gu), _p(act), M, N, K, x.stride(0), wgu.stride(0), gu.stride(0), act.stride(0))
    return gu, act


def dgrad_geglu_bwd_ok(dy, w, gu):
    M, K = dy.shape
    N = w.shape[1]
    return (dy.dtype == w.dtype == gu.dtype == torch.bfloat16 and gu.shape == (M, 2 * N) and gu.stride(1) == 1 and dy.stride(1) == 1 and w.stride(1) == 1
            and bool(_lib.lap_gemm_asm_geglu_bwd_ok(M, N, K, dy.stride(0), w.stride(0), gu.stride(0))))


def linear_dgrad_geglu_bwd(dy, w, gu):
    M, K = dy.shape
    N = w.shape[1]
    if tuple(gu.shape) != (M, 2 * N) or w.shape[0] != K:
        raise LapHipError(f"linear_dgrad_geglu_bwd: dy {tuple(dy.shape)}, w {tuple(w.shape)}, gate|up {tuple(gu.shape)} do not fit")
    ld = gu.stride(0)
    dgu = torch.empty((M, ld), dtype=torch.bfloat16, device=gu.device)[:, :2 * N]
    call("lap_gemm_asm_geglu_bwd", _p(dy), _p(w), _p(dgu), _p(gu), M, N, K, dy.stride(0), w.stride(0), ld)
    return dgu


def geglu_bwd(gu, dact, pad=False):
    rows, H2 = gu.shape
    dgu = _padded_rows(rows, H2, gu.device, _row_pad(H2) if pad else 0)
    call("lap_geglu_bwd_ld", _p(gu), _p(dact), _p(dgu), rows, H2 // 2, gu.stride(0), dact.stride(0), dgu.stride(0))
    return dgu


def gelu_fwd(x):
    y = torch.empty_like(x)
    call("lap_gelu_fwd", _p(x), _p(y), x.numel())
    return y


def gelu_bwd(x, dy):
    dx = torch.empty_like(x)
    call("lap_gelu_bwd", _p(x), _p(dy), _p(dx), x.numel())
    return dx


def embed_gather(table, tok, out, rows, T, D, dst_rps, dst_off, scale, row_lo=0, row_hi=None):
    if row_hi is None:
        row_hi = row_lo + table.shape[0]
    call("lap_embed_gather", _p(table), _p(tok), _p(out), rows, T, D, dst_rps, dst_off, float(scale), row_lo, row_hi)


def embed_scatter_add(dtable, tok, dout, rows, T, D, src_rps, src_off, scale):
    call("lap_embed_scatter_add", _p(dtable), _p(tok), _p(dout), rows, T, D, src_rps, src_off, float(scale))


def gated_residual_fwd(x, u, gate=None, rows_per_sample=0, ldg=0):
    y = torch.empty_like(x)
    call("lap_gated_residual_fwd", _p(x), _p(u), _p(gate), _p(y), x.shape[0], x.shape[1], rows_per_sample, ldg)
    return y


def gated_residual_bwd(dy, u, gate, rows_per_sample, ldg, dgate, ldg_out):
    du = torch.empty_like(dy)
    call("lap_gated_residual_bwd", _p(dy), _p(u), _p(gate), _p(du), _p(dgate), dy.shape[0], dy.shape[1],
         rows_per_sample, ldg, ldg_out)
    return du


def colsum(x, out, rows=None, cols=None, ld=None):
    rows = x.shape[0] if rows is None else rows
    cols = x.shape[1] if cols is None else cols
    ld = x.stride(0) if ld is None else ld
    call("lap_colsum_bf16" if x.dtype == torch.bfloat16 else "lap_colsum_f32", _p(x), _p(out), rows, cols, ld)


def cast_f32_to_bf16(x, y=None):
    if y is None:
        y = torch.empty(x.shape, dtype=torch.bfloat16, device=x.device)
    call("lap_cast_f32_to_bf16", _p(x), _p(y), x.numel())
    return y


def cast_bf16_to_f32(x, y=None):
    if y is None:
        y = torch.empty(x.shape, dtype=torch.float32, device=x.device)
    call("lap_cast_bf16_to_f32", _p(x), _p(y), x.numel())
    return y


def add_bf16(a, b, y=None):
    if y is None:
        y = torch.empty_like(a)
    call("lap_add_bf16", _p(a), _p(b), _p(y), a.numel())
    return y


def copy2d_bf16(src, dst, rows, cols, lds, ldd):
    call("lap_copy2d_bf16", _p(src), _p(dst), rows, cols, lds, ldd)


def copy_rows_bf16(src, dst, rows, T, D, src_rps, src_off, dst_rps, dst_off, accumulate=False):
    call("lap_copy_rows_bf16", _p(src), _p(dst), rows, T, D, src_rps, src_off, dst_rps, dst_off, int(accumulate))


def im2col_patch(img, P):
    B, H, W, Cc = img.shape
    out = torch.empty((B * (H // P) * (W // P), P * P * Cc), dtype=torch.float32, device=img.device)
    call("lap_im2col_patch", _p(img), _p(out), B, H, W, Cc, P)
    return out


def add_posemb_cast(x, pos, T):
    rows, D = x.shape
    y = torch.empty((rows, D), dtype=torch.bfloat16, device=x.device)
    call("lap_add_posemb_cast", _p(x), _p(pos), _p(y), rows, T, D)
    return y


def add_posemb_cast_bwd(dy, dpos, T):
    rows, D = dy.shape
    dx = torch.empty((rows, D), dtype=torch.float32, device=dy.device)
    call("lap_add_posemb_cast_bwd", _p(dy), _p(dx), _p(dpos), rows, T, D)
    return dx


def attention_set_variant(variant: int):
    _chk(_fn["lap_attention_set_variant"](int(variant)), "lap_attention_set_variant")


def attention_fwd(q, k, v, q_len, k_len, B, NH, NKV, HD, qinfo=None, kinfo=None, need_lse=True, scale=1.0,
                  q_rs=(0, 0), kv_rs=(0, 0), nsplit_hint=None, o_out=None, lse_out=None):
    a = AttnFwdArgs()
    outs = []
    for s in range(2):
        qs = q[s] if s < len(q) else None
        a.q[s] = _p(qs)
        a.q_rs[s], a.kv_rs[s], a.o_rs[s] = q_rs[s], kv_rs[s], 0
        o = None
        if qs is not None:
            o = torch.empty((B * q_len[s], NH * HD), dtype=torch.bfloat16, device=qs.device) if o_out is None else \
                (o_out[s] if s < len(o_out) else None)
            if o is None or o.shape != (B * q_len[s], NH * HD) or o.dtype != torch.bfloat16 or not o.is_contiguous():
                raise TypeError("o_out must hold packed bf16 [B*len, NH*HD] tensors")
        outs.append(o)
        a.o[s] = _p(o)
        a.k[s] = _p(k[s]) if s < len(k) and k[s] is not None else None
        a.v[s] = _p(v[s]) if s < len(v) and v[s] is not None else None
        a.q_len[s] = q_len[s] if s < len(q_len) else 0
        a.k_len[s] = k_len[s] if s < len(k_len) else 0
    for nm, inf in (("qinfo", qinfo), ("kinfo", kinfo)):
        if inf is not None and (inf.dtype != torch.int32 or not inf.is_contiguous()):
            raise TypeError(f"{nm} must be a contiguous int32 tensor, got {inf.dtype}")
    Tq = a.q_len[0] + a.q_len[1]
    dev = next(t for t in q if t is not None).device
    lse = None
    if need_lse:
        lse = lse_out if lse_out is not None else torch.empty((B, NH, Tq), dtype=torch.float32, device=dev)
        if lse.shape != (B, NH, Tq) or lse.dtype != torch.float32 or not lse.is_contiguous():
            raise TypeError("lse_out must be a contiguous f32 [B, NH, Tq] tensor")
    a.qinfo, a.kinfo, a.lse = _p(qinfo), _p(kinfo), _p(lse)
    a.scale = float(scale)
    a.B, a.NH, a.NKV, a.HD = B, NH, NKV, HD
    if _SERVE_ATTN and HD == 256 and a.q_len[0] == 0 and 0 < a.q_len[1] <= 64 and not need_lse and nsplit_hint is None and scale > 0:
        ns = _fn["lap_attention_serve_splits"](a.k_len[0], a.k_len[1], B, NH, a.q_len[1])
        if 0 < ns <= 16:
            a.nsplit = ns
            scratch = torch.empty(ns * B * Tq * NH * (HD + 1), dtype=torch.float32, device=dev)
            a.scratch, a.scratch_floats = _p(scratch), scratch.numel()
            _chk(_fn["lap_attention_serve"](C.byref(a), _stream()), "lap_attention_serve")
            return outs, None
    ntq = (a.q_len[0] + 63) // 64 + (a.q_len[1] + 63) // 64
    ntk = (a.k_len[0] + 63) // 64 + (a.k_len[1] + 63) // 64
    blocks = B * NH * ntq
    nsplit = 1
    if nsplit_hint is None and _NSPLIT_ENV and blocks < 128 and ntk > 1:
        nsplit_hint = min(int(_NSPLIT_ENV), ntk)
    if nsplit_hint is not None:
        nsplit = nsplit_hint
    elif blocks < 128 and ntk > 1:
        nsplit = min((ntk + 1) // 2, max(1, 256 // blocks))
    a.nsplit = nsplit
    if nsplit > 1:
        scratch = torch.empty(nsplit * B * Tq * NH * (HD + 1), dtype=torch.float32, device=dev)
        a.scratch, a.scratch_floats = _p(scratch), scratch.numel()
    a.B, a.NH, a.NKV, a.HD = B, NH, NKV, HD
# ... 686 lines not shown
```

lap_amd/loss.py:

```python
from __future__ import annotations

from typing import NamedTuple

import torch

from lap_amd import hip
from lap_amd.config import VQA_DATASET_ID_MAP


def vocab_chunks(R: int, V: int, cap_cols: int | None = None) -> list[tuple[int, int]]:
    if cap_cols is None:
        cap_cols = max(1024, (int(1.5e9) // (2 * R)) // 1024 * 1024)
    return [(v0, min(cap_cols, V - v0)) for v0 in range(0, V, cap_cols)]


def lm_logits(model, pl, v0: int, vc: int, out=None):
    R, Dv = pl.shape
    if out is None:
        out = torch.empty((R, vc), dtype=torch.float32, device=pl.device)
    hip.gemm(pl, model.W("llm/embed")[v0:v0 + vc], out, M=R, N=vc, K=Dv, lda=Dv, ldb=Dv, ldc=vc)
    hip.gemm(pl, model.ps.w16lo("llm/embed")[v0:v0 + vc], out, M=R, N=vc, K=Dv, lda=Dv, ldb=Dv, ldc=vc, accum=True)
    return out


class LangHead(NamedTuple):
    lang_loss: torch.Tensor
    lm: torch.Tensor = None
    lm_s: torch.Tensor = None
    cnt: torch.Tensor = None
    sel: torch.Tensor = None
    rowid: torch.Tensor = None
    rows: torch.Tensor = None
    pl: torch.Tensor = None
    rstd_pl: torch.Tensor = None
    targets: torch.Tensor = None
    m: torch.Tensor = None
    lsum: torch.Tensor = None
    chunks: list = None
    logit_chunks: list = None
    Lt: int = 0
    verbose_metrics: dict = {}


def lang_head_fwd(model, xf0, obs, observation, B, Pn, *, backward: bool, verbose: bool, collect) -> LangHead:
    dev = model.device
    Dv, V = model.v.width, model.config.vocab_size
    Lt = obs.tokenized_prompt.shape[1]
    loss_mask = obs.tokenized_langact_mask[:, 1:] & obs.tokenized_prompt_mask[:, 1:]
    if obs.token_loss_mask is not None:
        loss_mask = loss_mask & obs.token_loss_mask[:, 1:]
    lm_bool = loss_mask if obs.sample_mask is None else loss_mask & obs.sample_mask[:, None]
    lm = lm_bool.to(torch.float32)
    cnt = torch.clamp(lm.sum(-1), min=1.0)
    n_sel = observation.loss_rows_max if observation.loss_rows_max is not None else obs.loss_rows_max
    row_mask = lm_bool
    if verbose:
        def prep(mk):
            if mk is None:
                return None
            mk = mk[:, 1:].to(dev, torch.bool)
            return (mk & obs.sample_mask[:, None] if obs.sample_mask is not None else mk).contiguous()

        cls_masks = [prep(obs.critical_token_mask), prep(obs.number_token_mask), prep(obs.direction_token_mask)]
        for mk in cls_masks:
            if mk is not None:
                row_mask = row_mask | mk
        n_sel = observation.metric_rows_max if observation.metric_rows_max is not None else obs.metric_rows_max
    sel = rowid = None
    if n_sel is not None and 0 < n_sel < Lt - 1:
        sel = torch.sort((~row_mask).to(torch.uint8), dim=1, stable=True).indices[:, :n_sel]
        hint_too_small = ((row_mask.sum(-1) if verbose else lm.sum(-1)) > n_sel).any()
        Ls = n_sel
        rowid = (torch.arange(B, device=dev) * Pn + (Pn - Lt))[:, None] + sel
        rows = xf0.index_select(0, rowid.view(-1))
        targets = obs.tokenized_prompt[:, 1:].gather(1, sel).to(torch.int32).contiguous().view(-1)
        lm_s = lm.gather(1, sel)
    else:
        Ls = Lt - 1
        rows = torch.empty((B * Ls, Dv), dtype=torch.bfloat16, device=dev)
        hip.copy_rows_bf16(xf0, rows, B * Ls, Ls, Dv, Pn, Pn - Lt, Ls, 0)
        targets = obs.tokenized_prompt[:, 1:].to(torch.int32).contiguous().view(-1)
        lm_s = lm
    R = B * Ls
    pl, rstd_pl = hip.rmsnorm_fwd(rows, scale=model.F("llm/final_norm"), save_rstd=backward)
    chunks = vocab_chunks(R, V)
    m = torch.full((R,), -3.0e38, dtype=torch.float32, device=dev)
    lsum = torch.zeros(R, dtype=torch.float32, device=dev); tl = torch.zeros(R, dtype=torch.float32, device=dev)
    amax = torch.empty(R, dtype=torch.int32, device=dev) if verbose else None
    logit_chunks = []
    for v0, vc in chunks:
        lg = lm_logits(model, pl, v0, vc)
        if verbose:
            hip.ce_chunk_update_argmax(lg, targets, m, lsum, tl, amax, v0)
        else:
            hip.ce_chunk_update(lg, targets, m, lsum, tl, v0)
        logit_chunks.append(lg if backward else None)
    nll = (m + torch.log(lsum) - tl).view(B, Ls)
    lang_loss = (nll * lm_s).sum(-1) / cnt
    if sel is not None:
        lang_loss = torch.where(hint_too_small, torch.full_like(lang_loss, float("nan")), lang_loss)
    verbose_metrics = {}
    if verbose:
        verbose_metrics = _token_metrics(model, amax, targets, nll, lm, sel, cls_masks, obs.tokenized_prompt[:, 1:])
        if collect is not None:
            collect["predictions"], collect["sel"] = amax.view(B, Ls), sel
    return LangHead(lang_loss, lm, lm_s, cnt, sel, rowid, rows, pl, rstd_pl, targets, m, lsum, chunks, logit_chunks, Lt, verbose_metrics)


def _token_metrics(model, amax, targets, nll, lm, sel, cls_masks, labels):
    crit, num, dirn = cls_masks
    ptl, counts = hip.token_metrics(amax, targets, nll.reshape(-1).contiguous(), lm.contiguous(),
                                    sel=sel.to(torch.int32).contiguous() if sel is not None else None,
                                    critical=crit, number=num, direction=dirn)
    tot = model.comm.all_reduce_sum(counts.sum(0).reshape(8)).view(4, 2)
    acc = tot[:, 0] / torch.clamp(tot[:, 1], min=1.0)
    out = {"token_accuracy": acc[0], "per_token_loss": ptl, "labels": labels}
    for k, (name, mk) in enumerate((("critical", crit), ("number", num), ("direction", dirn)), start=1):
        if mk is not None:
            out[f"{name}_token_accuracy"] = acc[k]
            out[f"per_sample_{name}_correct"] = counts[:, k, 0]
            out[f"per_sample_{name}_total"] = counts[:, k, 1]
    return out


def lang_head_bwd(model, head: LangHead, wl, n_active, B, Pn):
    dev = model.device
    R, Dv = head.pl.shape
    w = (wl[:, None] * head.lm_s / head.cnt[:, None] / n_active).contiguous().view(-1)
    pl2 = torch.cat([head.pl, head.pl], 0)
    dpl32 = torch.empty((2 * R, Dv), dtype=torch.float32, device=dev)
    table16, table_lo, gE = model.W("llm/embed"), model.ps.w16lo("llm/embed"), model.G("llm/embed")
    for ci, (v0, vc) in enumerate(head.chunks):
        dlogits = torch.empty((2 * R, vc), dtype=torch.bfloat16, device=dev)
        hip.ce_chunk_grad(head.logit_chunks[ci], head.targets, head.m, head.lsum, w, dlogits[:R], v0, dlogits_lo=dlogits[R:])
        head.logit_chunks[ci] = None
        if model.ps.is_trainable("llm/embed"):
            hip.linear_wgrad(dlogits, pl2, gE[v0:v0 + vc])
        hip.linear_dgrad(dlogits, table16[v0:v0 + vc], out=dpl32, accum=ci > 0)
        hip.linear_dgrad(dlogits[:R], table_lo[v0:v0 + vc], out=dpl32[:R], accum=True)
        del dlogits
    dpl = hip.cast_f32_to_bf16(dpl32[:R] + dpl32[R:])
    drows = hip.rmsnorm_bwd(head.rows, dpl, head.rstd_pl, scale=model.F("llm/final_norm"), dscale=model.G("llm/final_norm"))
    dx0 = torch.zeros((B * Pn, Dv), dtype=torch.bfloat16, device=dev)
    if head.sel is not None:
        dx0.index_copy_(0, head.rowid.view(-1), drows)
    else:
        hip.copy_rows_bf16(drows, dx0, R, head.Lt - 1, Dv, head.Lt - 1, 0, Pn, Pn - head.Lt)
    return dx0


class ActionHead(NamedTuple):
    pre1: torch.Tensor = None
    pre1f: torch.Tensor = None
    rstd_p1: torch.Tensor = None
    v_t: torch.Tensor = None


def action_head_fwd(model, xf1, mod, B, S, Sx, *, backward: bool) -> ActionHead:
    We = model.e.width
    if model.config.pi05:
        pre1, rstd_p1 = hip.rmsnorm_fwd(xf1, mod=model._mod_slot(mod, 2 * model.v.depth), rows_per_sample=S, save_rstd=backward)
    else:
        pre1_all, rstd_p1 = hip.rmsnorm_fwd(xf1, scale=model.F("llm/final_norm1"), save_rstd=backward)
        pre1 = pre1_all.view(B, Sx, We)[:, 1:].reshape(B * S, We).contiguous()
    pre1f = hip.cast_bf16_to_f32(pre1)
    return ActionHead(pre1, pre1f, rstd_p1, model._lin32(pre1f, "act/out_w", "act/out_b"))


def action_head_bwd(model, head: ActionHead, xf1, mod, dv, B, S, Sx):
    dev, We = model.device, model.e.width
    dpre1f = model._lin32_bwd(head.pre1f, dv.view(B * S, -1), "act/out_w", "act/out_b")
    if model.config.pi05:
        dmod = torch.zeros(mod.shape, dtype=torch.float32, device=dev)
        dx1 = hip.rmsnorm_bwd(xf1, hip.cast_f32_to_bf16(dpre1f), head.rstd_p1, mod=model._mod_slot(mod, 2 * model.v.depth), rows_per_sample=S,
                              dmod=model._mod_slot(dmod, 2 * model.v.depth))
        return dx1, dmod
    dall = torch.zeros((B, Sx, We), dtype=torch.bfloat16, device=dev)
    dall[:, 1:] = hip.cast_f32_to_bf16(dpre1f).view(B, S, We)
    return hip.rmsnorm_bwd(xf1, dall.view(B * Sx, We), head.rstd_p1, scale=model.F("llm/final_norm1"), dscale=model.G("llm/final_norm1")), None


class Mix(NamedTuple):
    wl: torch.Tensor
    act_mask: torch.Tensor
    mixing: bool
    extra_metrics: dict


def mix_sample_weights(cfg, lang_loss, sample_mask, is_vqa, is_pred, vqa_dataset_id, *, lang_on: bool) -> Mix:
    dev, B = lang_loss.device, lang_loss.shape[0]
    fb = lambda t: t.to(torch.float32)
    sm = sample_mask if sample_mask is not None else torch.ones(B, dtype=torch.bool, device=dev)
    vqa = is_vqa.to(dev, torch.bool) if is_vqa is not None else None
    pred = is_pred.to(dev, torch.bool) if is_pred is not None else None
    if not (lang_on and (cfg.enable_vqa_training or cfg.enable_prediction_training)):
        wl = torch.full((B,), cfg.language_loss_weight if lang_on else 0.0, dtype=torch.float32, device=dev)
        act_mask = torch.ones(B, dtype=torch.bool, device=dev)
        if vqa is not None:
            act_mask = act_mask & ~vqa
        if pred is not None:
            act_mask = act_mask & ~pred
        return Mix(wl, act_mask, False, {})
    extra_metrics = {}
    vqa_m = (vqa if vqa is not None else torch.zeros(B, dtype=torch.bool, device=dev)) & sm
    pred_m = (pred if pred is not None else torch.zeros(B, dtype=torch.bool, device=dev)) & sm
    lang_m = ~((vqa if vqa is not None else vqa_m) | (pred if pred is not None else pred_m)) & sm
    vqa_w = torch.full((B,), cfg.vqa_loss_weight, dtype=torch.float32, device=dev)
    if cfg.enable_vqa_training and cfg.vqa_loss_weights and vqa_dataset_id is not None:
        ids = vqa_dataset_id.to(dev)
        for name, wgt in cfg.vqa_loss_weights.items():
            if name in VQA_DATASET_ID_MAP:
                vqa_w = torch.where(ids == VQA_DATASET_ID_MAP[name], torch.full_like(vqa_w, float(wgt)), vqa_w)
    wl = vqa_w * fb(vqa_m) + cfg.prediction_loss_weight * fb(pred_m) + cfg.language_loss_weight * fb(lang_m)
    act_mask = ~vqa_m & ~pred_m
    n_act_loc = fb(sm).sum()
    for pfx, msk in (("vqa_", vqa_m), ("pred_", pred_m), ("langact_", lang_m)):
        if (pfx == "vqa_" and not cfg.enable_vqa_training) or (pfx == "pred_" and not cfg.enable_prediction_training):
            continue
        extra_metrics[pfx + "loss"] = (lang_loss * fb(msk)).sum() / torch.clamp(fb(msk).sum(), min=1.0)
        extra_metrics[pfx + "num_samples"] = fb(msk).sum()
        extra_metrics[pfx + "sample_portion"] = fb(msk).sum() / torch.clamp(n_act_loc, min=1.0)
    if cfg.enable_vqa_training and vqa_dataset_id is not None:
        names = list(VQA_DATASET_ID_MAP)
        idv = torch.tensor([VQA_DATASET_ID_MAP[n] for n in names], dtype=torch.int64, device=dev)
        ind = fb((vqa_dataset_id.to(dev).to(torch.int64).view(B, 1) == idv.view(1, -1)) & vqa_m.view(B, 1))
# ... 9 lines not shown
```

lap_amd/model.py:

```python
from __future__ import annotations

import contextlib
import dataclasses
import math
import os

import torch

from lap_amd import hip
from lap_amd.config import LAPConfig, get_gemma_config, get_siglip_config
from lap_amd.loss import ActionHead, LangHead, action_head_bwd, action_head_fwd, lang_head_bwd, lang_head_fwd, mix_sample_weights
from lap_amd.observation import CoTObservation, preprocess_observation
from lap_amd.params import LORA_PROJ, ParamStore, lora_geometry
from lap_amd.serve_cache import ServeCache

SUFFIX_IDX_BASE = 0x800000


class _NullComm:
    world_size = 1

    def wait_unit(self, name, also=None): pass
    def pace(self, name): pass
    def grads_ready(self, name, also=None): pass
    def before_backward(self): pass
    def all_reduce_sum(self, t): return t


def _gen(rng, device):
    if isinstance(rng, torch.Generator):
        return rng
    g = torch.Generator(device=device)
    g.manual_seed(int(rng) if rng is not None else 0)
    return g


class LAP:
    EOS_TOKEN = 1

    def __init__(self, config: LAPConfig, seed: int = 0, params: dict | None = None, device="cuda", store: ParamStore | None = None,
                 comm=None, with_optimizer: bool = False, with_ema: bool = False, with_grads: bool = True, gemm_dtype: str = "bf16"):
        self.config = config
        if gemm_dtype not in ("bf16", "fp8"):
            raise ValueError(f"gemm_dtype {gemm_dtype!r}: 'bf16' or 'fp8'")
        self.gemm_dtype = gemm_dtype
        self._w8: dict = {}
        self.device = torch.device(device)
        self.v = get_gemma_config(config.paligemma_variant)
        self.e = get_gemma_config(config.action_expert_variant)
        self.s = get_siglip_config(config.siglip_variant)
        self.action_dim, self.action_horizon, self.max_token_len = config.action_dim, config.action_horizon, config.max_token_len
        self.comm = comm if comm is not None else _NullComm()
        if store is None:
            store = ParamStore(config, device, with_optimizer=with_optimizer, with_ema=with_ema, with_grads=with_grads)
            if params is not None:
                store.load_reference_tree(params)
            else:
                store.init_random(seed)
        self.ps = store
        self.n_img_tok = (config.image_size // self.s.patch) ** 2
        self.deterministic = True
        self.dual_stream = os.environ.get("LAP_DUAL_STREAM", "1") != "0"
        self.serve_fusions = os.environ.get("LAP_SERVE_FUSIONS", "1") != "0"
        self.fuse_geglu_bwd = os.environ.get("LAP_FUSE_GEGLU_BWD", "1") != "0" and gemm_dtype != "fp8"
        self.fuse_geglu_fwd = os.environ.get("LAP_FUSE_GEGLU_FWD", "1") != "0" and gemm_dtype != "fp8"
        self.fuse_gelu = os.environ.get("LAP_FUSE_GELU", "1") != "0"
        self.serve_overlap = os.environ.get("LAP_SERVE_OVERLAP", "0") != "0"
        self.serve_chain = os.environ.get("LAP_SERVE_CHAIN", "1") != "0"
        self.serve_packed = os.environ.get("LAP_SERVE_PACKED", "1") != "0"
        self.serve_tp = os.environ.get("LAP_SERVE_TP", "0") != "0"
        self.serve_euler_embed = os.environ.get("LAP_SERVE_EULER_EMBED", "1") != "0"
        self.serve_panel = os.environ.get("LAP_SERVE_PANEL", "1") != "0"
        self._panel_gelu = os.environ.get("LAP_SERVE_PANEL_GELU", "exp2")
        self._panel_llm = os.environ.get("LAP_SERVE_PANEL_LLM", "")
        self._panel_nt = tuple(int(v) for v in os.environ.get("LAP_SERVE_PANEL_NT", "2,1,3,3").split(","))
        self.serve_prefetch = os.environ.get("LAP_SERVE_PREFETCH", "1") != "0"
        self._chain_ctr = None
        self._chain_scratch = None
        self._den = None
        ks = os.environ.get("LAP_PREFILL_KS", "4,1,8,19").split(",")
        self._prefill_ks = tuple(int(k) for k in ks)
        self._sfx = None
        mode = os.environ.get("LAP_WGRAD_STREAM", "sb")
        self.wgrad_stream = "" if mode == "0" else mode
        self._wg = self._wg_obj = self._wg_main = None
        self._wg_dirty = False
        self._wg_ev: dict = {}
        self._lora_geo = {}
        for i, c in enumerate((self.v, self.e)):
            for proj in LORA_PROJ:
                geo = lora_geometry(c, proj, self.v.num_heads, self.v.num_kv_heads, self.v.head_dim)
                if geo is not None:
                    self._lora_geo[f"{proj}{i}"] = (geo[0], geo[2], geo[3])
        self._merge_depth = 0
        self.serving_cache = ServeCache(self.ps, self.device, lambda unit: self.comm.wait_unit(unit))
        if self._lora_geo and gemm_dtype == "fp8":
            raise ValueError("gemm_dtype='fp8' has no LoRA route: use gemm_dtype='bf16' with the LoRA Gemma variants")
        if gemm_dtype == "fp8":
            dims = (self.v.width, self.v.num_heads * self.v.head_dim, self.v.mlp_dim, (self.v.num_heads + 2 * self.v.num_kv_heads) * self.v.head_dim)
            if any(d % 128 for d in dims):
                raise ValueError(f"gemm_dtype='fp8' needs projection dimensions that are multiples of 128, got {dims}")

    def _suffix_stream(self, *tensors):
        if not self.dual_stream or any(t is None or not t.is_cuda for t in tensors) or torch.cuda.is_current_stream_capturing():
            return None
        if self._sfx is None:
            self._sfx = torch.cuda.Stream(self.device, priority=-1)
        self._sfx.wait_stream(torch.cuda.current_stream())
        for t in tensors:
            t.record_stream(self._sfx)
        return self._sfx

    @staticmethod
    def _handoff(src, dst, *tensors):
        if src is not None and dst is not None:
            dst.wait_stream(src)
            for t in tensors:
                if t is not None:
                    t.record_stream(dst)

    def W(self, name):
        if self._merge_depth and name.rsplit("/", 1)[-1] in self._lora_geo:
            return self._merged(name)
        return self.ps.w16(name)

    def F(self, name):
        return self.ps.f32(name)

    def G(self, name):
        return self.ps.g(name)

    def _wgrad(self, dy, x, name, **kw):
        if self.ps.is_trainable(name):
            mode = self.wgrad_stream
            kind = "s" if name.startswith("img/") else ("q" if name.endswith(("wqkv0", "wo0")) else "g")
            fold = not kw and getattr(self.comm, "fold_sumsq", False) and dy.dtype == torch.bfloat16

            def run():
                if fold:
                    if hip.linear_wgrad_sumsq(dy, x, self.G(name), self.comm.sumsq[0:1]):
                        self.comm.folded.add(name)
                else:
                    hip.linear_wgrad(dy, x, self.G(name), **kw)
            if mode == "1" or kind in mode:
                with self._off_path(dy, x):
                    run()
            else:
                run()

# ... 40 lines not shown
        self.comm.grads_ready(name, also=also or None)

    def _wg_begin(self):
        if self.wgrad_stream and self.device.type == "cuda" and not torch.cuda.is_current_stream_capturing():
            if self._wg_obj is None:
                self._wg_obj = torch.cuda.Stream(self.device)
            self._wg, self._wg_main, self._wg_dirty = self._wg_obj, torch.cuda.current_stream(), False

    def _wg_end(self):
        self._wg_join()
        self._wg = None

    def _lora(self, name):
        if not self._lora_geo or self._merge_depth:
            return None
        _, l, key = name.split("/")
        geo = self._lora_geo.get(key)
        if geo is None:
            return None
        return (self.ps.w16(f"llm/{l}/lora_a_{key}"), self.ps.w16(f"llm/{l}/lora_b_{key}"), *geo)

    def _lora_fwd(self, x, y, name):
        lo = self._lora(name)
        if lo is None:
            return None
        A, Bm, G, nsum, s = lo
        t = hip.lora_down(x, A)
        hip.lora_up_add(y, t, Bm, G=G, nsum=nsum, s=s)
        return t

    def _lora_bwd(self, dy, x, t, dx, name):
        lo = self._lora(name)
        if lo is None:
            return
        A, Bm, G, nsum, s = lo
        Ng = Bm.shape[1]
        dt = hip.lora_down(dy, Bm, G=G, nsum=nsum, xg=Ng if G > 1 else 0, s=s)
        _, l, key = name.split("/")
        na, nb = f"llm/{l}/lora_a_{key}", f"llm/{l}/lora_b_{key}"

        def run():
            if self.ps.is_trainable(na):
                hip.lora_wgrad(dt, x, self.G(na))
            if self.ps.is_trainable(nb):
                hip.lora_wgrad(t, dy, self.G(nb), G=G, bg=Ng if G > 1 else 0, ncopy=nsum, s=s)
        mode = self.wgrad_stream
        if mode == "1" or ("q" if key in ("wqkv0", "wo0") else "g") in mode:
            with self._off_path(dy, x, t, dt):
                run()
        else:
            run()
        if dx is not None:
            hip.lora_up_add(dx, dt, A)

    def _merged(self, name):
        def build(old):
            _, l, key = name.split("/")
            self.comm.wait_unit(f"llm{l}")
            G, nsum, s = self._lora_geo[key]
            out = old if old is not None else torch.empty(self.ps.tensor_spec[name].shape, dtype=torch.bfloat16, device=self.device)
            return hip.lora_merge(self.F(name), self.F(f"llm/{l}/lora_a_{key}"), self.F(f"llm/{l}/lora_b_{key}"), out, G=G, nsum=nsum, s=s)
        return self.serving_cache.get(("merged", name), None, build)

    @contextlib.contextmanager
    def _serving_weights(self):
        if not self._lora_geo:
            yield
            return
        if self.comm.world_size != 1:
            raise NotImplementedError("LoRA serving merges the weights from the f32 masters: replicas only")
        self._merge_depth += 1
        try:
            yield
        finally:
            self._merge_depth -= 1

    def _w8_of(self, name):
        ent = self._w8.get(name)
        if ent is None or ent[0] != self.ps.version:
            ent = (self.ps.version, *hip.quantize_fp8_weight(self.W(name)))
            self._w8[name] = ent
        return ent[1:]

    def _lin0(self, x, name, residual=None, out=None):
        if self.gemm_dtype == "fp8":
            x8, sx = hip.quantize_fp8(x)
            w8, _, sw = self._w8_of(name)
            return hip.gemm_fp8(x8, sx, w8, sw, residual=residual)
        if residual is not None and os.environ.get("LAP_UNFUSED_RESIDUAL", "0") == "1":
            return hip.add_bf16(residual, hip.linear_fwd(x, self.W(name)))
        return hip.linear_fwd(x, self.W(name), out, residual=residual)

    def _dgrad0(self, dy, name):
        if self.gemm_dtype == "fp8":
            d8, sd = hip.quantize_fp8(dy)
            _, w8t, sw = self._w8_of(name)
            return hip.gemm_fp8(d8, sd, w8t, sw)
        return hip.linear_dgrad(dy, self.W(name))

    def _prefix_frozen(self) -> bool:
        fr = self.ps.frozen
        if not fr:
            return False
        return all(v for k, v in fr.items() if k.startswith("img/") or k in ("llm/embed", "llm/final_norm")
                   or (k.startswith("llm/") and (k.endswith("0") or k.endswith("n_attn") or k.endswith("n_ffw"))))

    def _lin32(self, x, wname, bname):
        w = self.F(wname)
        out = torch.empty((x.shape[0], w.shape[0]), dtype=torch.float32, device=x.device)
        return hip.gemm_f32(x, w, out, M=x.shape[0], N=w.shape[0], K=w.shape[1], lda=x.stride(0), ldb=w.stride(0), ldc=w.shape[0],
                            bias=self.F(bname))

    def _lin32_bwd(self, x, dy, wname, bname, need_dx=True):
        w = self.F(wname)
        hip.gemm_f32(dy, x, self.G(wname), M=w.shape[0], N=w.shape[1], K=x.shape[0], lda=dy.stride(0), ldb=x.stride(0), ldc=w.shape[1],
                     a_kc=False, b_kc=False, accum=True)
        hip.colsum(dy, self.G(bname))
        if not need_dx:
            return None
        dx = torch.empty_like(x)
        return hip.gemm_f32(dy, w, dx, M=x.shape[0], N=w.shape[1], K=w.shape[0], lda=dy.stride(0), ldb=w.stride(0), ldc=w.shape[1],
                            a_kc=True, b_kc=False)

    def _siglip_fwd(self, images: torch.Tensor, save: bool, collect=None, x_in=None, blocks=None):
        s, T = self.s, self.n_img_tok
        W = s.width
        hd = W // s.num_heads
        ctx = {"blocks": []} if save else None
        if x_in is not None:
            x, N = x_in, x_in.shape[0] // T
            for l in blocks:
                x = self._siglip_block(l, x, N, T, W, hd, None, False)
            return x, None
        N = images.shape[0]
        patches = hip.im2col_patch(images.contiguous(), s.patch)
        p_hi, p_lo = hip.split_f32_hilo(patches)
        w_hi, w_lo = hip.split_f32_hilo(self.F("img/stem_w"))
        del patches
        stem = torch.empty((p_hi.shape[0], W), dtype=torch.float32, device=p_hi.device)
        R, Kp = p_hi.shape
        hip.gemm(p_hi, w_hi, stem, M=R, N=W, K=Kp, lda=Kp, ldb=Kp, ldc=W, bias=self.F("img/stem_b"))
        hip.gemm(p_hi, w_lo, stem, M=R, N=W, K=Kp, lda=Kp, ldb=Kp, ldc=W, accum=True)
        hip.gemm(p_lo, w_hi, stem, M=R, N=W, K=Kp, lda=Kp, ldb=Kp, ldc=W, accum=True)
        x = hip.add_posemb_cast(stem, self.F("img/pos"), T)
        del stem
        if collect is not None:
            collect["img/stem"] = x
        if save:
            ctx["patches"] = (p_hi, p_lo)
        for l in range(s.depth):
            x = self._siglip_block(l, x, N, T, W, hd, ctx, save)
            if collect is not None:
                collect[f"img/block{l:02d}"] = x
        self.comm.wait_unit("img_head")
        enc, mean, rstd = hip.layernorm_fwd(x, self.F("img/norm_g"), self.F("img/norm_b"))
        tok = hip.linear_fwd(enc, self.W("img/head_w"), bias=self.F("img/head_b"))
        if save:
            ctx["final"] = (x, enc, mean, rstd)
        if collect is not None:
            collect["img/out"] = tok
        return tok, ctx

    def _siglip_fwd_serve(self, images: torch.Tensor):
        s, T = self.s, self.n_img_tok
        W = s.width
        hd = W // s.num_heads
        N = images.shape[0]
        patches = hip.im2col_patch(images.contiguous(), s.patch)
        p_hi, p_lo = hip.split_f32_hilo(patches)
        w_hi, w_lo = hip.split_f32_hilo(self.F("img/stem_w"))
        stem = torch.empty((p_hi.shape[0], W), dtype=torch.float32, device=p_hi.device)
        R, Kp = p_hi.shape
        hip.gemm(p_hi, w_hi, stem, M=R, N=W, K=Kp, lda=Kp, ldb=Kp, ldc=W, bias=self.F("img/stem_b"))
        hip.gemm(p_hi, w_lo, stem, M=R, N=W, K=Kp, lda=Kp, ldb=Kp, ldc=W, accum=True)
# ... 199 lines not shown

    def _embed_prefix_bwd(self, pctx, dx0, B, Pn):
        ictx, tokens = pctx
        keys = self.config.image_keys
        T, Lt, Dv = self.n_img_tok, tokens.shape[1], self.v.width
        hip.embed_scatter_add(self.G("llm/embed"), tokens, dx0, B * Lt, Lt, Dv, Pn, T * len(keys), math.sqrt(Dv))
        self.comm.grads_ready("embed")
        dtok = torch.empty((len(keys) * B * T, Dv), dtype=torch.bfloat16, device=self.device)
        for i in range(len(keys)):
            hip.copy_rows_bf16(dx0, dtok[i * B * T:(i + 1) * B * T], B * T, T, Dv, Pn, i * T, T, 0)
        self._siglip_bwd(ictx, dtok)

    def _time_mod(self, time: torch.Tensor, save: bool):
        We = self.e.width
        temb = hip.posemb_sincos(time.contiguous(), We, 4e-3, 4.0)
        h1 = self._lin32(temb, "act/time_in_w", "act/time_in_b")
        s1 = hip.swish_fwd(h1)
        h2 = self._lin32(s1, "act/time_out_w", "act/time_out_b")
        cond = hip.swish_fwd(h2)
        cond16 = hip.cast_f32_to_bf16(cond)
        mod = hip.linear_fwd(cond16, self.W("ada/w"), bias=self.F("ada/b"))
        return mod, ((temb, h1, s1, h2, cond16) if save else None)

    def _embed_actions(self, x_t: torch.Tensor):
        B, S, ad = x_t.shape
        xt2 = x_t.reshape(B * S, ad).contiguous()
        return hip.cast_f32_to_bf16(self._lin32(xt2, "act/in_w", "act/in_b")), xt2

    def _embed_suffix_pi0(self, x_t: torch.Tensor, time: torch.Tensor, state: torch.Tensor, save: bool):
        B, S, ad = x_t.shape
        We = self.e.width
        xt2 = x_t.reshape(B * S, ad).contiguous()
        a = self._lin32(xt2, "act/in_w", "act/in_b")
        temb = hip.posemb_sincos(time.contiguous(), We, 4e-3, 4.0)
        cat = torch.cat([a.view(B, S, We), temb[:, None, :].expand(B, S, We)], -1).reshape(B * S, 2 * We).contiguous()
        h1 = self._lin32(cat, "act/atime_in_w", "act/atime_in_b")
        s1 = hip.swish_fwd(h1)
        at = self._lin32(s1, "act/atime_out_w", "act/atime_out_b")
        st2 = state.to(self.device, torch.float32).reshape(B, ad).contiguous()
        st = self._lin32(st2, "act/state_w", "act/state_b")
        tok = torch.cat([st[:, None, :], at.view(B, S, We)], 1).reshape(B * (S + 1), We).contiguous()
        return hip.cast_f32_to_bf16(tok), ((xt2, cat, h1, s1, st2) if save else None)

    def _embed_suffix_pi0_bwd(self, sctx, dx1, B, S):
        xt2, cat, h1, s1, st2 = sctx
        We = self.e.width
        d = hip.cast_bf16_to_f32(dx1).view(B, S + 1, We)
        self._lin32_bwd(st2, d[:, 0].contiguous(), "act/state_w", "act/state_b", need_dx=False)
        ds1 = self._lin32_bwd(s1, d[:, 1:].reshape(B * S, We).contiguous(), "act/atime_out_w", "act/atime_out_b")
        dh1 = hip.swish_bwd(h1, ds1)
        dcat = self._lin32_bwd(cat, dh1, "act/atime_in_w", "act/atime_in_b")
        self._lin32_bwd(xt2, dcat[:, :We].contiguous(), "act/in_w", "act/in_b", need_dx=False)

    def _embed_suffix(self, x_t: torch.Tensor, time: torch.Tensor, save: bool, overlap: bool = False):
        sfx = self._suffix_stream(x_t, time) if overlap else None
        self.comm.wait_unit("ada", also=sfx)
        with (torch.cuda.stream(sfx) if sfx is not None else contextlib.nullcontext()):
            x1, xt2 = self._embed_actions(x_t)
            mod, tctx = self._time_mod(time, save)
        if sfx is not None:
            mod.record_stream(torch.cuda.current_stream()); x1.record_stream(torch.cuda.current_stream())
        return x1, mod, ((xt2, *tctx) if save else None)

    def _embed_suffix_bwd(self, sctx, dx1, dmod):
        xt2, temb, h1, s1, h2, cond16 = sctx
        sfx = self._suffix_stream(dx1, dmod)
        with (torch.cuda.stream(sfx) if sfx is not None else contextlib.nullcontext()):
            dmod16 = hip.cast_f32_to_bf16(dmod)
            hip.colsum(dmod, self.G("ada/b"))
            self._wgrad(dmod16, cond16, "ada/w")
            dcond = hip.cast_bf16_to_f32(hip.linear_dgrad(dmod16, self.W("ada/w")))
            self.comm.grads_ready("ada")
            dh2 = hip.swish_bwd(h2, dcond)
            ds1 = self._lin32_bwd(s1, dh2, "act/time_out_w", "act/time_out_b")
            dh1 = hip.swish_bwd(h1, ds1)
            self._lin32_bwd(temb, dh1, "act/time_in_w", "act/time_in_b", need_dx=False)
            self._lin32_bwd(xt2, hip.cast_bf16_to_f32(dx1), "act/in_w", "act/in_b", need_dx=False)
        return sfx

    def _mod_slot(self, mod, slot):
        W3 = 3 * self.e.width
        return mod[:, slot * W3:(slot + 1) * W3]

    def _llm_fwd(self, x0, x1, mod, pos, qinfo, kinfo, B, n0, n1, save: bool, kv_cache=None, cache_out=None, collect=None,
                 mod_shared: bool = False, layers=None):
        v, e = self.v, self.e
        NH, HD, KV = v.num_heads, v.head_dim, v.num_kv_heads
        Ttot = pos.shape[1]
        ctx = [] if save else None
        mld = 0 if mod_shared else (mod.stride(0) if mod is not None else 0)
        sfx = self._suffix_stream(*([x1, mod] if mod is not None else [x1])) if (x0 is not None and x1 is not None) else None
        main = torch.cuda.current_stream() if sfx is not None else None
        on_sfx = (lambda: torch.cuda.stream(sfx)) if sfx is not None else contextlib.nullcontext
        for l in (range(v.depth) if layers is None else layers):
            self.comm.wait_unit(f"llm{l}", also=sfx)
            p = f"llm/{l}/"
            q = [None, None]; k = [None, None]; vv = [None, None]; h = [None, None]; rstd_a = [None, None]
            lt = [{}, {}]
            if x0 is not None:
                h[0], rstd_a[0] = hip.rmsnorm_fwd(x0, scale=self.F(p + "n_attn"), save_rstd=save)
                qkv = self._lin0(h[0], p + "wqkv0")
                lt[0]["wqkv"] = self._lora_fwd(h[0], qkv, p + "wqkv0")
                q[0], k[0], vv[0] = hip.rope_split_fwd(qkv, pos, B, n0, Ttot, 0, NH, HD, HD ** -0.5)
                del qkv
            elif kv_cache is not None:
                k[0], vv[0] = kv_cache[l]
            if x1 is not None:
                with on_sfx():
                    if mod is None:
                        h[1], rstd_a[1] = hip.rmsnorm_fwd(x1, scale=self.F(p + "n_attn1"), save_rstd=save)
                    else:
                        h[1], rstd_a[1] = hip.rmsnorm_fwd(x1, mod=self._mod_slot(mod, 2 * l), rows_per_sample=n1, save_rstd=save, mod_ld=mld)
                    qkv = hip.linear_fwd(h[1], self.W(p + "wqkv1"))
                    lt[1]["wqkv"] = self._lora_fwd(h[1], qkv, p + "wqkv1")
                    q[1], k[1], vv[1] = hip.rope_split_fwd(qkv, pos, B, n1, Ttot, Ttot - n1, NH, HD, HD ** -0.5)
                    del qkv
                self._handoff(sfx, main, q[1], k[1], vv[1])
            if cache_out is not None:
                cache_out.append((k[0], vv[0]))
            qlen = [n0 if x0 is not None else 0, n1 if x1 is not None else 0]
            klen = [k[0].shape[0] // B if k[0] is not None else 0, n1 if x1 is not None else 0]
            o, lse = hip.attention_fwd(q, k, vv, qlen, klen, B, NH, KV, HD, qinfo, kinfo, need_lse=save)
            self._handoff(main, sfx, o[1])
            xa = [None, None]; y1 = None; hf = [None, None]; rstd_f = [None, None]; gu = [None, None]; act = [None, None]; y1f = None
            xn = [None, None]
            if x1 is not None and mod is None:
                with on_sfx():
                    xa[1] = hip.linear_fwd(o[1], self.W(p + "wo1"), residual=x1)
                    lt[1]["wo"] = self._lora_fwd(o[1], xa[1], p + "wo1")
                    hf[1], rstd_f[1] = hip.rmsnorm_fwd(xa[1], scale=self.F(p + "n_ffw1"), save_rstd=save)
                    gu[1] = hip.linear_fwd(hf[1], self.W(p + "wgu1"))
                    lt[1]["wgu"] = self._lora_fwd(hf[1], gu[1], p + "wgu1")
                    act[1] = hip.geglu_fwd(gu[1])
                    xn[1] = hip.linear_fwd(act[1], self.W(p + "wd1"), residual=xa[1])
                    lt[1]["wd"] = self._lora_fwd(act[1], xn[1], p + "wd1")
            elif x1 is not None:
                with on_sfx():
                    y1 = hip.linear_fwd(o[1], self.W(p + "wo1"))
                    lt[1]["wo"] = self._lora_fwd(o[1], y1, p + "wo1")
                    xa[1] = hip.gated_residual_fwd(x1, y1, self._mod_slot(mod, 2 * l)[:, 2 * e.width:], n1, mld)
                    hf[1], rstd_f[1] = hip.rmsnorm_fwd(xa[1], mod=self._mod_slot(mod, 2 * l + 1), rows_per_sample=n1, save_rstd=save, mod_ld=mld)
                    gu[1] = hip.linear_fwd(hf[1], self.W(p + "wgu1"))
                    lt[1]["wgu"] = self._lora_fwd(hf[1], gu[1], p + "wgu1")
                    act[1] = hip.geglu_fwd(gu[1])
                    y1f = hip.linear_fwd(act[1], self.W(p + "wd1"))
                    lt[1]["wd"] = self._lora_fwd(act[1], y1f, p + "wd1")
                    xn[1] = hip.gated_residual_fwd(xa[1], y1f, self._mod_slot(mod, 2 * l + 1)[:, 2 * e.width:], n1, mld)
            if x0 is not None:
                xa[0] = self._lin0(o[0], p + "wo0", residual=x0)
                lt[0]["wo"] = self._lora_fwd(o[0], xa[0], p + "wo0")
                hf[0], rstd_f[0] = hip.rmsnorm_fwd(xa[0], scale=self.F(p + "n_ffw"), save_rstd=save)
                self.comm.pace(f"llm{l}")
                if save and self.fuse_geglu_fwd and self._lora(p + "wgu0") is None and hip.linear_geglu_train_ok(hf[0], self.W(p + "wgu0")):
                    gu[0], act[0] = hip.linear_geglu_train(hf[0], self.W(p + "wgu0"))
                else:
                    gu_out = None
                    if save and self.fuse_geglu_bwd:
                        gu_out = hip._padded_rows(hf[0].shape[0], 2 * v.mlp_dim, hf[0].device, hip._row_pad(2 * v.mlp_dim))
                    gu[0] = self._lin0(hf[0], p + "wgu0", out=gu_out)
                    lt[0]["wgu"] = self._lora_fwd(hf[0], gu[0], p + "wgu0")
                    act[0] = hip.geglu_fwd(gu[0], pad=self.gemm_dtype != "fp8")
                xn[0] = self._lin0(act[0], p + "wd0", residual=xa[0])
                lt[0]["wd"] = self._lora_fwd(act[0], xn[0], p + "wd0")
            if save:
                ctx.append(dict(x=[x0, x1], h=h, rstd_a=rstd_a, q=q, k=k, v=vv, o=o, lse=lse, xa=xa, y1=y1, hf=hf, rstd_f=rstd_f,
                                gu=gu, act=act, y1f=y1f, lt=lt))
            x0, x1 = xn
            if collect is not None:
                collect[f"llm/layer{l:02d}/x0"], collect[f"llm/layer{l:02d}/x1"] = x0, x1
        self._handoff(sfx, main, x1)
        return x0, x1, ctx

    def _llm_prefill(self, x0, pos, qinfo, kinfo, B, n0, cache_out, kv_events=None):
        v = self.v
        NH, HD, KV = v.num_heads, v.head_dim, v.num_kv_heads
        Ttot = pos.shape[1]
        Dv = v.width
        scratch = hip._gemm_scratch(self.device)
        tab = hip.rope_table(pos, B, n0, Ttot, 0, HD)
        self.comm.wait_unit("llm0")
        h, _ = hip.rmsnorm_fwd(x0, scale=self.F("llm/0/n_attn"), save_rstd=False)
        rows = x0.shape[0]
        panel = (self.serve_panel and rows <= 640 and hip.panel_gemm_ok(rows, (NH + 2 * KV) * HD, Dv) and hip.panel_gemm_ok(rows, Dv, NH * HD))
        panel_q, panel_o = panel and "q" in self._panel_llm, panel and "o" in self._panel_llm
        pf = (lambda name: self._pw(name)) if panel_o and self.serve_prefetch else (lambda name: None)
        for l in range(v.depth):
            p = f"llm/{l}/"
            if panel_q:
                part, ks = hip.panel_partials(h, self._pw(p + "wqkv0"), (NH + 2 * KV) * HD, scratch, 1, nt=2, prefetch=pf(p + "wo0"))
            else:
                part, ks = hip.linear_partials(h, self.W(p + "wqkv0"), scratch, ksplit=self._prefill_ks[0])
            q, k, vv = hip.fused_reduce_rope_split(part, ks, pos, B, n0, Ttot, 0, NH, HD, HD ** -0.5, table=tab)
            cache_out.append((k, vv))
            if kv_events is not None:
                ev = torch.cuda.Event()
                ev.record()
                kv_events.append(ev)
            o, _ = hip.attention_fwd([q, None], [k, None], [vv, None], [n0, 0], [n0, 0], B, NH, KV, HD, qinfo, kinfo, need_lse=False)
            if panel_o:
                xa = hip.panel_linear(o[0], self._pw(p + "wo0"), Dv, residual=x0, nt=4)
                hf, _ = hip.rmsnorm_fwd(xa, scale=self.F(p + "n_ffw"), save_rstd=False)
            elif self._prefill_ks[1] > 1:
                part, ks = hip.linear_partials(o[0], self.W(p + "wo0"), scratch, ksplit=self._prefill_ks[1])
                xa, hf = hip.fused_reduce_norm(part, ks, rows, Dv, residual=x0, norm=1, gamma=self.F(p + "n_ffw"))
            else:
                xa = hip.linear_fwd(o[0], self.W(p + "wo0"), residual=x0)
                hf, _ = hip.rmsnorm_fwd(xa, scale=self.F(p + "n_ffw"), save_rstd=False)
            if rows <= 640 and (v.mlp_dim & 127) == 0:
                act = hip.linear_geglu(hf, self.W(p + "wgu0"), exp2=self._panel_gelu == "exp2")
            else:
                act = hip.geglu_fwd(hip.linear_fwd(hf, self.W(p + "wgu0")))
            part, ks = hip.linear_partials(act, self.W(p + "wd0"), scratch, ksplit=self._prefill_ks[2], tile=self._prefill_ks[3])
            if l + 1 < v.depth:
                self.comm.wait_unit(f"llm{l + 1}")
                x0, h = hip.fused_reduce_norm(part, ks, rows, Dv, residual=xa, norm=1, gamma=self.F(f"llm/{l + 1}/n_attn"))
            else:
                x0, h = hip.fused_reduce_norm(part, ks, rows, Dv, residual=xa, norm=0)
        return x0

    def _llm_bwd(self, ctx, dx0, dx1, mod, dmod, pos, qinfo, kinfo, B, n0, n1):
        v, e = self.v, self.e
        NH, HD, KV = v.num_heads, v.head_dim, v.num_kv_heads
        Ttot = pos.shape[1]
        has_sfx = dx1 is not None
        ada = has_sfx and mod is not None
        ldm = mod.stride(0) if ada else 0
        zero_do0 = None
        sfx = self._suffix_stream(*([dx1, dmod, mod] if ada else [dx1]))
        main = torch.cuda.current_stream() if sfx is not None else None
        on_sfx = (lambda: torch.cuda.stream(sfx)) if sfx is not None else contextlib.nullcontext
        for l in reversed(range(v.depth)):
            p = f"llm/{l}/"
            c = ctx[l]
            d_o = [None, None]
            slot_f, slot_a = 2 * l + 1, 2 * l
            if has_sfx and not ada:
                with on_sfx():
                    self._wgrad(dx1, c["act"][1], p + "wd1")
                    dact = hip.linear_dgrad(dx1, self.W(p + "wd1"))
                    self._lora_bwd(dx1, c["act"][1], c["lt"][1].get("wd"), dact, p + "wd1")
                    dgu = hip.geglu_bwd(c["gu"][1], dact)
                    self._wgrad(dgu, c["hf"][1], p + "wgu1")
                    dhf = hip.linear_dgrad(dgu, self.W(p + "wgu1"))
                    self._lora_bwd(dgu, c["hf"][1], c["lt"][1].get("wgu"), dhf, p + "wgu1")
                    hip.rmsnorm_bwd(c["xa"][1], dhf, c["rstd_f"][1], scale=self.F(p + "n_ffw1"), dx=dx1, dscale=self.G(p + "n_ffw1"), accum_dx=True)
                    self._wgrad(dx1, c["o"][1], p + "wo1")
                    d_o[1] = hip.linear_dgrad(dx1, self.W(p + "wo1"))
                    self._lora_bwd(dx1, c["o"][1], c["lt"][1].get("wo"), d_o[1], p + "wo1")
                    del dact, dgu, dhf
            elif has_sfx:
                with on_sfx():
                    gate_f = self._mod_slot(mod, slot_f)[:, 2 * e.width:]
                    dy1f = hip.gated_residual_bwd(dx1, c["y1f"], gate_f, n1, ldm, self._mod_slot(dmod, slot_f)[:, 2 * e.width:], dmod.stride(0))
                    self._wgrad(dy1f, c["act"][1], p + "wd1")
                    dact = hip.linear_dgrad(dy1f, self.W(p + "wd1"))
                    self._lora_bwd(dy1f, c["act"][1], c["lt"][1].get("wd"), dact, p + "wd1")
                    dgu = hip.geglu_bwd(c["gu"][1], dact)
                    self._wgrad(dgu, c["hf"][1], p + "wgu1")
                    dhf = hip.linear_dgrad(dgu, self.W(p + "wgu1"))
                    self._lora_bwd(dgu, c["hf"][1], c["lt"][1].get("wgu"), dhf, p + "wgu1")
                    hip.rmsnorm_bwd(c["xa"][1], dhf, c["rstd_f"][1], mod=self._mod_slot(mod, slot_f), rows_per_sample=n1, dx=dx1,
                                    dmod=self._mod_slot(dmod, slot_f), accum_dx=True)
                    gate_a = self._mod_slot(mod, slot_a)[:, 2 * e.width:]
                    dy1 = hip.gated_residual_bwd(dx1, c["y1"], gate_a, n1, ldm, self._mod_slot(dmod, slot_a)[:, 2 * e.width:], dmod.stride(0))
                    self._wgrad(dy1, c["o"][1], p + "wo1")
                    d_o[1] = hip.linear_dgrad(dy1, self.W(p + "wo1"))
                    self._lora_bwd(dy1, c["o"][1], c["lt"][1].get("wo"), d_o[1], p + "wo1")
                    del dy1f, dact, dgu, dhf, dy1
            if dx0 is not None:
                self._wgrad(dx0, c["act"][0], p + "wd0")
                if self.fuse_geglu_bwd and self._lora(p + "wd0") is None and hip.dgrad_geglu_bwd_ok(dx0, self.W(p + "wd0"), c["gu"][0]):
                    dgu = hip.linear_dgrad_geglu_bwd(dx0, self.W(p + "wd0"), c["gu"][0])
                else:
                    dact = self._dgrad0(dx0, p + "wd0")
                    self._lora_bwd(dx0, c["act"][0], c["lt"][0].get("wd"), dact, p + "wd0")
                    dgu = hip.geglu_bwd(c["gu"][0], dact, pad=self.gemm_dtype != "fp8")
                    del dact
                self._wgrad(dgu, c["hf"][0], p + "wgu0")
                dhf = self._dgrad0(dgu, p + "wgu0")
                self._lora_bwd(dgu, c["hf"][0], c["lt"][0].get("wgu"), dhf, p + "wgu0")
                del dgu
                self._wg_join(dx0)
                hip.rmsnorm_bwd(c["xa"][0], dhf, c["rstd_f"][0], scale=self.F(p + "n_ffw"), dx=dx0, dscale=self.G(p + "n_ffw"), accum_dx=True)
                del dhf
                self._wgrad(dx0, c["o"][0], p + "wo0")
                d_o[0] = self._dgrad0(dx0, p + "wo0")
                self._lora_bwd(dx0, c["o"][0], c["lt"][0].get("wo"), d_o[0], p + "wo0")
            else:
                if zero_do0 is None:
                    zero_do0 = torch.zeros_like(c["o"][0])
                d_o[0] = zero_do0
            self._handoff(sfx, main, d_o[1])
            dq, dk, dv = hip.attention_bwd(c["q"], c["k"], c["v"], c["o"], d_o, c["lse"], [n0, n1], [n0, n1], B, NH, KV, HD, qinfo, kinfo,
                                           stop_q1_to_k0=self.config.stop_action_to_vlm_grad)
            self._handoff(main, sfx, dq[1], dk[1], dv[1])
            if has_sfx:
                with on_sfx():
                    dqkv = hip.rope_split_bwd(dq[1], dk[1], dv[1], pos, B, n1, Ttot, Ttot - n1, NH, HD, HD ** -0.5)
                    self._wgrad(dqkv, c["h"][1], p + "wqkv1")
                    dh = hip.linear_dgrad(dqkv, self.W(p + "wqkv1"))
                    self._lora_bwd(dqkv, c["h"][1], c["lt"][1].get("wqkv"), dh, p + "wqkv1")
                    if ada:
                        hip.rmsnorm_bwd(c["x"][1], dh, c["rstd_a"][1], mod=self._mod_slot(mod, slot_a), rows_per_sample=n1, dx=dx1,
                                        dmod=self._mod_slot(dmod, slot_a), accum_dx=True)
                    else:
                        hip.rmsnorm_bwd(c["x"][1], dh, c["rstd_a"][1], scale=self.F(p + "n_attn1"), dx=dx1, dscale=self.G(p + "n_attn1"), accum_dx=True)
                    del dqkv, dh
            if dx0 is not None:
                dqkv = hip.rope_split_bwd(dq[0], dk[0], dv[0], pos, B, n0, Ttot, 0, NH, HD, HD ** -0.5)
                self._wgrad(dqkv, c["h"][0], p + "wqkv0")
                dh = self._dgrad0(dqkv, p + "wqkv0")
                self._lora_bwd(dqkv, c["h"][0], c["lt"][0].get("wqkv"), dh, p + "wqkv0")
                self._wg_join(dx0)
                hip.rmsnorm_bwd(c["x"][0], dh, c["rstd_a"][0], scale=self.F(p + "n_attn"), dx=dx0, dscale=self.G(p + "n_attn"), accum_dx=True)
                del dqkv, dh
            ctx[l] = None
            self._unit_done(f"llm{l}", sfx)
        self._handoff(sfx, main)
        return dx0, dx1

    def _expert_denoise_fwd(self, x1, mod, pos, qinfo, kinfo, B, Pn, S, cache, rope_tab=None):
        v, e = self.v, self.e
        NH, HD, KV = v.num_heads, v.head_dim, v.num_kv_heads
        Ttot = pos.shape[1]
        We = e.width
        scratch = hip._gemm_scratch(self.device)
        slot = lambda j: self._mod_slot(mod, j)
        h, _ = hip.rmsnorm_fwd(x1, mod=slot(0), rows_per_sample=S, save_rstd=False, mod_ld=0)
        x = x1
        for l in range(v.depth):
            self.comm.wait_unit(f"llm{l}")
            p = f"llm/{l}/"
            part, ks = hip.linear_partials(h, self.W(p + "wqkv1"), scratch)
            q, k, vv = hip.fused_reduce_rope_split(part, ks, pos, B, S, Ttot, Ttot - S, NH, HD, HD ** -0.5, table=rope_tab)
            ck, cv = cache[l]
            o, _ = hip.attention_fwd([None, q], [ck, k], [cv, vv], [0, S], [Pn, S], B, NH, KV, HD, qinfo, kinfo, need_lse=False)
            part, ks = hip.linear_partials(o[1], self.W(p + "wo1"), scratch)
            xa, hf = hip.fused_reduce_residual_norm(part, ks, x, slot(2 * l)[:, 2 * We:], 0, slot(2 * l + 1), 0, S)
            part, ks = hip.linear_partials(hf, self.W(p + "wgu1"), scratch)
            act = hip.fused_reduce_geglu(part, ks, B * S, e.mlp_dim)
            part, ks = hip.linear_partials(act, self.W(p + "wd1"), scratch)
            x, h = hip.fused_reduce_residual_norm(part, ks, xa, slot(2 * l + 1)[:, 2 * We:], 0, slot(2 * l + 2), 0, S)
        return h

    def _expert_denoise_skinny(self, x1, mod, qinfo, kinfo, B, Pn, S, cache, rope_tab, kv_events=None):
        v, e = self.v, self.e
        NH, HD, KV = v.num_heads, v.head_dim, v.num_kv_heads
        We = e.width
        slot = lambda j: self._mod_slot(mod, j)
        x = x1
        for l in range(v.depth):
            self.comm.wait_unit(f"llm{l}")
            p = f"llm/{l}/"
            q, k, vv = hip.serve_qkv_rope(x, slot(2 * l), 0, S, self.W(p + "wqkv1"), rope_tab, NH, HD, HD ** -0.5)
            ck, cv = cache[l]
            if kv_events is not None:
                torch.cuda.current_stream().wait_event(kv_events[l])
                ck.record_stream(torch.cuda.current_stream()); cv.record_stream(torch.cuda.current_stream())
            o, _ = hip.attention_fwd([None, q], [ck, k], [cv, vv], [0, S], [Pn, S], B, NH, KV, HD, qinfo, kinfo, need_lse=False)
            xa = hip.serve_proj_residual(o[1], self.W(p + "wo1"), x, slot(2 * l)[:, 2 * We:], 0, S)
            act = hip.serve_gate_up(xa, slot(2 * l + 1), 0, S, self.W(p + "wgu1"))
            x = hip.serve_proj_residual(act, self.W(p + "wd1"), xa, slot(2 * l + 1)[:, 2 * We:], 0, S)
        return x

    def _loss_impl(self, rng, observation: CoTObservation, actions: torch.Tensor, *, train: bool, noise=None, time=None,
                   backward: bool, collect: dict | None = None, verbose: bool = False):
        cfg = self.config
        act_on, lang_on = cfg.enable_action_training, cfg.enable_langact_training
        if not (act_on or lang_on):
            raise ValueError("LAPConfig with neither enable_action_training nor enable_langact_training has no loss")
        dev = self.device
        self.comm.wait_unit("small")
        g = _gen(rng, dev)
        obs = preprocess_observation(observation, train=train, image_keys=cfg.image_keys, image_resolution=cfg.image_resolution,
                                     enable_image_augmentation=cfg.enable_image_augmentation, rng=g)
        actions = actions.to(dev, torch.float32).contiguous()
        B, S, ad = actions.shape
        if S != self.action_horizon:
            raise ValueError(f"actions horizon {S} != action_horizon {self.action_horizon}")
        x1 = mod = sctx = u_t = None
        if act_on:
            if noise is None:
                noise = torch.randn(actions.shape, generator=g, device=dev, dtype=torch.float32)
            if time is None:
                u1 = torch.rand(B, generator=g, device=dev, dtype=torch.float32)
                time = u1.pow(1.0 / 1.5) * 0.999 + 0.001
            noise = noise.to(dev, torch.float32).contiguous(); time = time.to(dev, torch.float32).contiguous()
            x_t, u_t = hip.fm_mix(noise, actions, time)
            if cfg.pi05:
                x1, mod, sctx = self._embed_suffix(x_t, time, backward, overlap=True)
            else:
                if obs.state is None:
                    raise ValueError("pi05=False feeds the continuous state through state_proj: the observation has no `state`")
                x1, sctx = self._embed_suffix_pi0(x_t, time, obs.state, backward)
        Sx = (S + (0 if cfg.pi05 else 1)) if act_on else 0
        x0, Pn, pctx = self._embed_prefix(obs, backward, collect)
        qinfo, kinfo, pos = self._train_infos(obs, S if act_on else 0)
        if collect is not None:
            collect["x0_in"], collect["x1_in"], collect["pos"], collect["mod"] = x0, x1, pos, mod
        xf0, xf1, lctx = self._llm_fwd(x0, x1, mod, pos, qinfo, kinfo, B, Pn, Sx, backward, collect=collect)
        if collect is not None:
            collect["x0_out"], collect["x1_out"] = xf0, xf1

        fb = lambda t: t.to(torch.float32)
        sm = obs.sample_mask if obs.sample_mask is not None else torch.ones(B, dtype=torch.bool, device=dev)
        head = lang_head_fwd(self, xf0, obs, observation, B, Pn, backward=backward, verbose=verbose, collect=collect) if lang_on else \
            LangHead(torch.zeros(B, dtype=torch.float32, device=dev))
        ah = action_head_fwd(self, xf1, mod, B, S, Sx, backward=backward) if act_on else ActionHead()
        lang_loss, v_t = head.lang_loss, ah.v_t
        wl, act_mask, mixing, extra_metrics = mix_sample_weights(
            cfg, lang_loss, sm, obs.is_vqa_sample if cfg.enable_vqa_training else None,
            obs.is_prediction_sample if cfg.enable_prediction_training else None, obs.vqa_dataset_id, lang_on=lang_on)
        n_active = torch.clamp(self.comm.all_reduce_sum(fb(sm).sum().view(1)), min=1.0) if obs.sample_mask is not None else \
            self.comm.all_reduce_sum(torch.tensor([float(B)], device=dev))
        lang_term = (wl * lang_loss).sum() / n_active
        act_loss = torch.zeros(B, dtype=torch.float32, device=dev)
        action_term = 0.0
        dv = None
        if act_on:
            n_action = torch.clamp(self.comm.all_reduce_sum(fb(act_mask).sum().view(1)), min=1.0)
            coef = cfg.action_loss_weight * fb(act_mask) / n_action
            act_loss, dv = hip.mse_fwd_bwd(v_t.view(B, S * ad), u_t.view(B, S * ad), coef, need_grad=backward)
            action_term = (cfg.action_loss_weight * act_loss * fb(act_mask)).sum() / n_action
        loss = self.comm.all_reduce_sum((lang_term + action_term).view(1)).view(())
        metrics = {"lang_loss": lang_loss.mean(), "action_loss": (act_loss * fb(act_mask)).sum() / torch.clamp(fb(act_mask).sum(), min=1.0),
                   "langact_loss": (lang_loss * fb(sm)).sum() / torch.clamp(fb(sm).sum(), min=1.0) if not mixing else extra_metrics["langact_loss"],
                   **{k: v for k, v in extra_metrics.items() if k != "langact_loss"}, **head.verbose_metrics}
        if verbose:
            metrics["per_sample_loss"] = wl * lang_loss + (cfg.action_loss_weight * act_loss * fb(act_mask) if act_on else 0.0)
        if collect is not None:
            collect.update(pl=head.pl, pre1=ah.pre1, v_t=v_t.view(B, S, ad) if v_t is not None else None, u_t=u_t, per_sample_lang=lang_loss,
                           per_sample_action=act_loss)
        if not backward:
            return loss, metrics

        self.comm.before_backward()
        self._wg_begin()
        dx1, dmod = action_head_bwd(self, ah, xf1, mod, dv, B, S, Sx) if act_on else (None, None)
        skip_prefix = self._prefix_frozen()
        dx0 = None
        if not skip_prefix and lang_on:
            dx0 = lang_head_bwd(self, head, wl, n_active, B, Pn)
        elif not skip_prefix:
            dx0 = torch.zeros((B * Pn, self.v.width), dtype=torch.bfloat16, device=dev)
            if self.ps.is_trainable("llm/embed"):
                self.G("llm/embed").zero_()
        dx0, dx1 = self._llm_bwd(lctx, dx0, dx1, mod, dmod, pos, qinfo, kinfo, B, Pn, Sx)
        sfx = None
        if act_on and cfg.pi05:
            sfx = self._embed_suffix_bwd(sctx, dx1, dmod)
        elif act_on:
            self._embed_suffix_pi0_bwd(sctx, dx1, B, S)
        elif "ada" in self.ps.unit_by_name:
            self.comm.grads_ready("ada")
        if not skip_prefix:
            self._embed_prefix_bwd(pctx, dx0, B, Pn)
        self._handoff(sfx, torch.cuda.current_stream() if sfx is not None else None)
        self._wg_end()
        self.comm.grads_ready("small")
        return loss, metrics

    def compute_loss(self, rng, observation, actions, *, train: bool = False, stage_config=None, verbose_mode=None,
                     return_augmented_images: bool = False, noise=None, time=None, collect=None):
        verbose = bool(self.config.verbose_mode if verbose_mode is None else verbose_mode)
        return self._loss_impl(rng, observation, actions, train=train, noise=noise, time=time, backward=False, collect=collect,
                               verbose=verbose)

    def loss_and_grad(self, rng, observation, actions, *, train: bool = True, noise=None, time=None, collect=None):
        return self._loss_impl(rng, observation, actions, train=train, noise=noise, time=time, backward=True, collect=collect,
                               verbose=bool(self.config.verbose_mode))

    @torch.no_grad()
    def sample_actions(self, rng, observation, *, num_steps: int = 10, noise=None, collect=None, fused=True):
        with self._serving_weights():
            return self._sample_actions(rng, observation, num_steps=num_steps, noise=noise, collect=collect, fused=fused)

    def _sample_actions(self, rng, observation, *, num_steps: int = 10, noise=None, collect=None, fused=True):
        cfg = self.config
        dev = self.device
        self.comm.wait_unit("small")
        obs = preprocess_observation(observation, train=False, image_keys=cfg.image_keys, image_resolution=cfg.image_resolution)
        B = obs.tokenized_prompt.shape[0]
        S, ad = self.action_horizon, self.action_dim
        if fused is True:
            fused = "skinny" if hip.serve_supported(self.e.width, self.v.head_dim, self.e.mlp_dim, self.v.num_heads) else "partials"
        if fused not in (False, "skinny", "partials"):
            raise ValueError(f"fused={fused!r}")
        if noise is None:
            noise = torch.randn((B, S, ad), generator=_gen(rng, dev), device=dev, dtype=torch.float32)
        x_t = noise.to(dev, torch.float32).contiguous().clone()
        x0, Pn, _ = self._embed_prefix(obs, False, serve=True)
        qinfo_p, kinfo_p, ppos, qinfo_s, kinfo_all, pos_all = self._serve_infos(obs, S)
        if not cfg.pi05:
            return self._sample_actions_pi0(obs, x_t, x0, Pn, (qinfo_p, kinfo_p, ppos, qinfo_s, kinfo_all, pos_all), num_steps, collect)
        dt = -1.0 / num_steps
        times, t = [], 1.0
        while t >= -dt / 2:
            times.append(t)
            t += dt
        mods = self._serve_mods(len(times), dt)
        rope_tab = hip.rope_table(pos_all, B, S, pos_all.shape[1], pos_all.shape[1] - S, self.v.head_dim) if fused else None
        cache = []
        fast_prefill = self.serve_fusions and collect is None and self.gemm_dtype == "bf16"
        overlap = fast_prefill and fused == "skinny" and self.serve_overlap and dev.type == "cuda" and len(times) > 1
        kv_events = [] if overlap else None
        if overlap:
            if self._den is None:
                self._den = torch.cuda.Stream(dev)
            start = torch.cuda.Event()
            start.record()
        if fast_prefill:
            self._llm_prefill(x0, ppos, qinfo_p, kinfo_p, B, Pn, cache, kv_events=kv_events)
        else:
            self._llm_fwd(x0, None, None, ppos, qinfo_p, kinfo_p, B, Pn, 0, False, cache_out=cache)
        nslot = 2 * self.v.depth
        chain = (fused == "skinny" and self.serve_chain and not overlap and dev.type == "cuda" and self.v.depth <= hip.CHAIN_MAX_DEPTH
                 and hip.serve_chain_ok(B, S, self.e.width, self.e.mlp_dim, self.v.num_heads, self.v.head_dim, self.v.num_kv_heads, Pn))
        if chain:
            if self._chain_ctr is None:
                self._chain_ctr = hip.serve_chain_counters(dev)
            for l in range(self.v.depth):
                self.comm.wait_unit(f"llm{l}")
            tp = (self.serve_packed and self.serve_tp
                  and hip.serve_chain_tp_ok(B, S, self.e.width, self.e.mlp_dim, self.v.num_heads, self.v.head_dim, self.v.num_kv_heads, Pn))
            if self.serve_packed:
                chain_w = self._serve_packed_weights()
                if self._chain_scratch is None or (tp and "tp_slabs" not in self._chain_scratch):
                    self._chain_scratch = hip.serve_chain_scratch(dev, self.e.width, self.e.mlp_dim, self.v.num_heads, self.v.head_dim, tp=tp)
            else:
                chain_w = [tuple(self.W(f"llm/{l}/{n}") for n in ("wqkv1", "wo1", "wgu1", "wd1")) for l in range(self.v.depth)]
# ... 132 lines not shown
```

Baseline: 122.2 samples/s.

## Compute last LLM layer queries and MLP only for loss-relevant prefix rows

In the final prefix (Gemma-2B) layer, only the rows whose outputs feed the language loss are kept as queries. Attention output, the output projection, the MLP and the loss head run on this compacted set, while K/V still cover every row. Indexed rope-split, gather and rmsnorm-backward kernels scatter the gradients back to the full layout. This cuts the last layer's prefix query, GEMM and MLP work in both forward and backward. The cost is extra index bookkeeping and gather kernels, and the set of selected rows depends on the loss masks.

```diff
diff --git a/include/lap_hip.h b/include/lap_hip.h
--- a/include/lap_hip.h
+++ b/include/lap_hip.h
@@ -95,6 +95,8 @@
 int lap_rmsnorm_bwd(const void* x, const float* scale, const void* mod, const float* rstd, const void* dy,
                     void* dx, float* dscale, float* dmod,
                     int rows, int D, int rows_per_sample, int mod_ld, int dmod_ld, int accum_dx, void* stream);
+int lap_rmsnorm_bwd_rows(const void* x, const float* scale, const float* rstd, const void* dy, void* dx, float* dscale,
+                         const int32_t* add_row, const void* addend, int rows, int D, void* stream);
 
 int lap_layernorm_fwd(const void* x, const float* gamma, const float* beta, void* y, float* mean, float* rstd,
                       int rows, int D, float eps, void* stream);
@@ -107,6 +109,10 @@
                        int B, int T_seg, int T_total, int seg_off, int NH, int HD, float q_scale, void* stream);
 int lap_rope_split_bwd(const void* dq, const void* dk, const void* dv, const int32_t* pos, void* dqkv,
                        int B, int T_seg, int T_total, int seg_off, int NH, int HD, float q_scale, void* stream);
+int lap_rope_split_fwd_rows(const void* qkv, const int32_t* pos, const int32_t* qrow, void* q, void* k, void* v,
+                            int B, int T_seg, int T_total, int seg_off, int NH, int HD, float q_scale, void* stream);
+int lap_rope_split_bwd_rows(const void* dq, const void* dk, const void* dv, const int32_t* pos, const int32_t* qrow, void* dqkv,
+                            int B, int T_seg, int T_total, int seg_off, int NH, int HD, float q_scale, void* stream);
 
 int lap_geglu_fwd(const void* gu, void* act, int rows, int H, void* stream);
 int lap_geglu_bwd(const void* gu, const void* dact, void* dgu, int rows, int H, void* stream);
@@ -135,6 +141,7 @@
 int lap_copy2d_bf16(const void* src, void* dst, int rows, int cols, int lds, int ldd, void* stream);
 int lap_copy_rows_bf16(const void* src, void* dst, int rows, int T, int D,
                        int src_rps, int src_off, int dst_rps, int dst_off, int accumulate, void* stream);
+int lap_gather_rows_bf16(const void* src, const int32_t* idx, void* dst, int rows, int D, void* stream);
 
 int lap_im2col_patch(const float* img, float* out, int B, int H, int W, int C, int P, void* stream);
 int lap_augment_images(const float* img, float* out, const float* params, int B, int H, int W, void* stream);
diff --git a/lap_amd/csrc/elementwise.hip b/lap_amd/csrc/elementwise.hip
--- a/lap_amd/csrc/elementwise.hip
+++ b/lap_amd/csrc/elementwise.hip
@@ -39,12 +39,13 @@
 
 inline dim3 flat_grid(long long n, int per_block = 256) { return dim3((unsigned)((n + per_block - 1) / per_block)); }
 
-template <bool BWD, bool HSPLIT = false>
+template <bool BWD, bool HSPLIT = false, bool QIDX = false>
 __global__ __launch_bounds__(256) void rope_split_kernel(const bf16* __restrict__ a0, const bf16* __restrict__ a1,
                                                          const bf16* __restrict__ a2, const int32_t* __restrict__ pos,
                                                          bf16* __restrict__ o0, bf16* __restrict__ o1,
                                                          bf16* __restrict__ o2, int rows, int T_seg, int T_total,
-                                                         int seg_off, int NH, int HD, float q_scale) {
+                                                         int seg_off, int NH, int HD, float q_scale,
+                                                         const int32_t* __restrict__ qrow) {
   const int cph = HD / 16;
   long long gid = (long long)blockIdx.x * 256 + threadIdx.x;
   int h_lo = 0, h_hi = NH + 2;
@@ -61,14 +62,24 @@
   const int W = (NH + 2) * HD;
   const int half = HD / 2;
   const float p = (float)pos[(long long)b * T_total + seg_off + t];
+  long long qr = row;
+  if constexpr (QIDX) qr = qrow[row];
   float sn[8], cs[8];
 #pragma unroll
   for (int e = 0; e < 8; ++e) rope_sincos(p, c * 8 + e, HD, sn[e], cs[e]);
 #pragma unroll 2
   for (int h = h_lo; h < h_hi; ++h) {
+    if (QIDX && h < NH && qr < 0) {
+      if (BWD) {
+        const float z[8] = {0.f, 0.f, 0.f, 0.f, 0.f, 0.f, 0.f, 0.f};
+        st8(o0 + (long long)row * W + h * HD + c * 8, z);
+        st8(o0 + (long long)row * W + h * HD + half + c * 8, z);
+      }
+      continue;
+    }
     const bf16* src;
     if (!BWD) src = a0 + (long long)row * W + h * HD;
-    else if (h < NH) src = a0 + (long long)row * NH * HD + h * HD;
+    else if (h < NH) src = a0 + qr * NH * HD + h * HD;
     else if (h == NH) src = a1 + (long long)row * HD;
     else src = a2 + (long long)row * HD;
     float x1[8], x2[8], y1[8], y2[8];
@@ -95,7 +106,7 @@
     }
     bf16* dst;
     if (BWD) dst = o0 + (long long)row * W + h * HD;
-    else if (h < NH) dst = o0 + (long long)row * NH * HD + h * HD;
+    else if (h < NH) dst = o0 + qr * NH * HD + h * HD;
     else if (h == NH) dst = o1 + (long long)row * HD;
     else dst = o2 + (long long)row * HD;
     st8(dst + c * 8, y1);
@@ -331,12 +342,12 @@
 }
 __global__ __launch_bounds__(256) void copy_rows_kernel(const bf16* __restrict__ src, bf16* __restrict__ dst, int rows,
                                                         int T, int D8, int src_rps, int src_off, int dst_rps,
-                                                        int dst_off, int accumulate) {
+                                                        int dst_off, int accumulate, const int32_t* __restrict__ src_idx) {
   const long long gid = (long long)blockIdx.x * 256 + threadIdx.x;
   if (gid >= (long long)rows * D8) return;
   const int r = (int)(gid / D8), c = (int)(gid % D8) * 8;
   const long long D = (long long)D8 * 8;
-  const long long srow = (long long)(r / T) * src_rps + src_off + r % T;
+  const long long srow = src_idx ? (long long)src_idx[r] : (long long)(r / T) * src_rps + src_off + r % T;
   const long long drow = (long long)(r / T) * dst_rps + dst_off + r % T;
   if (accumulate) {
     float a[8], b[8];
@@ -580,10 +591,23 @@
   const long long n = (long long)B * T_seg * (HD / 16);
   if (n < 65536)
     hipLaunchKernelGGL((rope_split_kernel<false, true>), flat_grid(n * (NH + 2)), dim3(256), 0, S_, (const bf16*)qkv, nullptr, nullptr, pos,
-                       (bf16*)q, (bf16*)k, (bf16*)v, B * T_seg, T_seg, T_total, seg_off, NH, HD, q_scale);
+                       (bf16*)q, (bf16*)k, (bf16*)v, B * T_seg, T_seg, T_total, seg_off, NH, HD, q_scale, nullptr);
   else
     hipLaunchKernelGGL(rope_split_kernel<false>, flat_grid(n), dim3(256), 0, S_, (const bf16*)qkv, nullptr, nullptr, pos,
-                       (bf16*)q, (bf16*)k, (bf16*)v, B * T_seg, T_seg, T_total, seg_off, NH, HD, q_scale);
+                       (bf16*)q, (bf16*)k, (bf16*)v, B * T_seg, T_seg, T_total, seg_off, NH, HD, q_scale, nullptr);
+  LAP_CHECK_LAUNCH();
+  return LAP_OK;
+}
+extern "C" int lap_rope_split_fwd_rows(const void* qkv, const int32_t* pos, const int32_t* qrow, void* q, void* k, void* v, int B,
+                                       int T_seg, int T_total, int seg_off, int NH, int HD, float q_scale, void* stream) {
+  if (B <= 0 || T_seg <= 0 || (HD & 15) || NH <= 0 || !qrow) return LAP_ERR_ARG;
+  const long long n = (long long)B * T_seg * (HD / 16);
+  if (n < 65536)
+    hipLaunchKernelGGL((rope_split_kernel<false, true, true>), flat_grid(n * (NH + 2)), dim3(256), 0, S_, (const bf16*)qkv, nullptr, nullptr,
+                       pos, (bf16*)q, (bf16*)k, (bf16*)v, B * T_seg, T_seg, T_total, seg_off, NH, HD, q_scale, qrow);
+  else
+    hipLaunchKernelGGL((rope_split_kernel<false, false, true>), flat_grid(n), dim3(256), 0, S_, (const bf16*)qkv, nullptr, nullptr, pos,
+                       (bf16*)q, (bf16*)k, (bf16*)v, B * T_seg, T_seg, T_total, seg_off, NH, HD, q_scale, qrow);
   LAP_CHECK_LAUNCH();
   return LAP_OK;
 }
@@ -593,7 +617,18 @@
   const long long n = (long long)B * T_seg * (HD / 16);
   hipLaunchKernelGGL(rope_split_kernel<true>, flat_grid(n), dim3(256), 0, S_, (const bf16*)dq, (const bf16*)dk,
                      (const bf16*)dv, pos, (bf16*)dqkv, nullptr, nullptr, B * T_seg, T_seg, T_total, seg_off, NH, HD,
-                     q_scale);
+                     q_scale, nullptr);
+  LAP_CHECK_LAUNCH();
+  return LAP_OK;
+}
+extern "C" int lap_rope_split_bwd_rows(const void* dq, const void* dk, const void* dv, const int32_t* pos, const int32_t* qrow,
+                                       void* dqkv, int B, int T_seg, int T_total, int seg_off, int NH, int HD, float q_scale,
+                                       void* stream) {
+  if (B <= 0 || T_seg <= 0 || (HD & 15) || NH <= 0 || !qrow) return LAP_ERR_ARG;
+  const long long n = (long long)B * T_seg * (HD / 16);
+  hipLaunchKernelGGL((rope_split_kernel<true, false, true>), flat_grid(n), dim3(256), 0, S_, (const bf16*)dq, (const bf16*)dk,
+                     (const bf16*)dv, pos, (bf16*)dqkv, nullptr, nullptr, B * T_seg, T_seg, T_total, seg_off, NH, HD,
+                     q_scale, qrow);
   LAP_CHECK_LAUNCH();
   return LAP_OK;
 }
@@ -727,7 +762,14 @@
                                   int dst_rps, int dst_off, int accumulate, void* stream) {
   if (rows <= 0 || T <= 0 || (D & 7)) return LAP_ERR_ARG;
   hipLaunchKernelGGL(copy_rows_kernel, flat_grid((long long)rows * (D / 8)), dim3(256), 0, S_, (const bf16*)src,
-                     (bf16*)dst, rows, T, D / 8, src_rps, src_off, dst_rps, dst_off, accumulate);
+                     (bf16*)dst, rows, T, D / 8, src_rps, src_off, dst_rps, dst_off, accumulate, nullptr);
+  LAP_CHECK_LAUNCH();
+  return LAP_OK;
+}
+extern "C" int lap_gather_rows_bf16(const void* src, const int32_t* idx, void* dst, int rows, int D, void* stream) {
+  if (rows <= 0 || D <= 0 || (D & 7) || !idx) return LAP_ERR_ARG;
+  hipLaunchKernelGGL(copy_rows_kernel, flat_grid((long long)rows * (D / 8)), dim3(256), 0, S_, (const bf16*)src,
+                     (bf16*)dst, rows, rows, D / 8, 0, 0, rows, 0, 0, idx);
   LAP_CHECK_LAUNCH();
   return LAP_OK;
 }
diff --git a/lap_amd/csrc/norm.hip b/lap_amd/csrc/norm.hip
--- a/lap_amd/csrc/norm.hip
+++ b/lap_amd/csrc/norm.hip
@@ -64,13 +64,14 @@
   }
 }
 
-template <int NCH>
+template <int NCH, bool IDX = false>
 __global__ __launch_bounds__(256) void rmsnorm_bwd_kernel(const bf16* __restrict__ x, const float* __restrict__ scale,
                                                           const bf16* __restrict__ mod, const float* __restrict__ rstd,
                                                           const bf16* __restrict__ dy, bf16* __restrict__ dx,
                                                           float* __restrict__ dscale, float* __restrict__ dmod,
                                                           int rows, int D, int G, int mod_ld, int dmod_ld,
-                                                          int accum_dx) {
+                                                          int accum_dx, const int32_t* __restrict__ add_row,
+                                                          const bf16* __restrict__ addend) {
   extern __shared__ __attribute__((aligned(16))) float red[];
   const int lane = threadIdx.x & 63, w = threadIdx.x >> 6;
   const int g = blockIdx.x;
@@ -113,11 +114,18 @@
   if (r0 + w < r1) fetch(r0 + w);
   for (int row = r0 + w; row < r1; row += NWAVE) {
     bf16x8 cx[NCH], cdy[NCH], cold[NCH];
+    const bf16* oldr = dx + (long long)row * D;
+    bool has_old = accum_dx;
+    if constexpr (IDX) {
+      const int j = add_row[row];
+      has_old = j >= 0;
+      oldr = addend + (long long)(j >= 0 ? j : 0) * D;
+    }
 #pragma unroll
     for (int p = 0; p < NCH; ++p) {
       cx[p] = nx[p]; cdy[p] = ndy[p];
       const int c = (lane + 64 * p) * 8;
-      if (NCH <= 3 && accum_dx && c < D) cold[p] = *reinterpret_cast<const bf16x8*>(dx + (long long)row * D + c);
+      if (NCH <= 3 && has_old && c < D) cold[p] = *reinterpret_cast<const bf16x8*>(oldr + c);
     }
     const float r = nr;
     if (row + NWAVE < r1) fetch(row + NWAVE);
@@ -149,8 +157,8 @@
         float o[8];
 #pragma unroll
         for (int e = 0; e < 8; ++e) o[e] = r * gv[p][e] - xv[p][e] * cc;
-        if (accum_dx) {
-          if constexpr (NCH > 3) cold[p] = *reinterpret_cast<const bf16x8*>(dxr + c);
+        if (has_old) {
+          if constexpr (NCH > 3) cold[p] = *reinterpret_cast<const bf16x8*>(oldr + c);
 #pragma unroll
           for (int e = 0; e < 8; ++e) o[e] += (float)cold[p][e];
         }
@@ -369,7 +377,23 @@
   const size_t shm = (size_t)NWAVE * (mod ? 2 : 1) * D * sizeof(float);
   DISPATCH_NCH(D, hipLaunchKernelGGL(rmsnorm_bwd_kernel<NCH>, grid, dim3(256), shm, s, (const bf16*)x, scale,
                                      (const bf16*)mod, rstd, (const bf16*)dy, (bf16*)dx, dscale, dmod, rows, D, G,
-                                     mod_ld, dmod_ld, accum_dx));
+                                     mod_ld, dmod_ld, accum_dx, nullptr, nullptr));
+  LAP_CHECK_LAUNCH();
+  return LAP_OK;
+}
+
+extern "C" int lap_rmsnorm_bwd_rows(const void* x, const float* scale, const float* rstd, const void* dy, void* dx,
+                                    float* dscale, const int32_t* add_row, const void* addend, int rows, int D,
+                                    void* stream) {
+  if (rows <= 0 || D <= 0 || (D & 7) || !rstd || !scale || !dscale || !add_row || !addend || dx == addend) return LAP_ERR_ARG;
+  hipStream_t s = (hipStream_t)stream;
+  static const int g_env = getenv("LAP_NORM_BWD_ROWS") ? atoi(getenv("LAP_NORM_BWD_ROWS")) : 64;
+  const int G = g_env;
+  dim3 grid((rows + G - 1) / G);
+  const size_t shm = (size_t)NWAVE * D * sizeof(float);
+  DISPATCH_NCH(D, hipLaunchKernelGGL((rmsnorm_bwd_kernel<NCH, true>), grid, dim3(256), shm, s, (const bf16*)x, scale,
+                                     (const bf16*)nullptr, rstd, (const bf16*)dy, (bf16*)dx, dscale, (float*)nullptr, rows,
+                                     D, G, 0, 0, 0, add_row, (const bf16*)addend));
   LAP_CHECK_LAUNCH();
   return LAP_OK;
 }
diff --git a/lap_amd/hip.py b/lap_amd/hip.py
--- a/lap_amd/hip.py
+++ b/lap_amd/hip.py
@@ -125,11 +125,14 @@
     "lap_gemm_f32": [_vp, _vp, _vp, _vp, _i, _i, _i, _i, _i, _i, _f, _i, _i, _i, _vp],
     "lap_rmsnorm_fwd": [_vp, _vp, _vp, _vp, _vp, _i, _i, _i, _i, _f, _vp],
     "lap_rmsnorm_bwd": [_vp, _vp, _vp, _vp, _vp, _vp, _vp, _vp, _i, _i, _i, _i, _i, _i, _vp],
+    "lap_rmsnorm_bwd_rows": [_vp, _vp, _vp, _vp, _vp, _vp, _vp, _vp, _i, _i, _vp],
     "lap_layernorm_fwd": [_vp, _vp, _vp, _vp, _vp, _vp, _i, _i, _f, _vp],
     "lap_layernorm_bwd": [_vp, _vp, _vp, _vp, _vp, _vp, _vp, _vp, _i, _i, _i, _vp],
     "lap_layernorm_bwd_sum": [_vp, _vp, _vp, _vp, _vp, _vp, _vp, _vp, _vp, _i, _i, _i, _vp],
     "lap_rope_split_fwd": [_vp, _vp, _vp, _vp, _vp, _i, _i, _i, _i, _i, _i, _f, _vp],
     "lap_rope_split_bwd": [_vp, _vp, _vp, _vp, _vp, _i, _i, _i, _i, _i, _i, _f, _vp],
+    "lap_rope_split_fwd_rows": [_vp, _vp, _vp, _vp, _vp, _vp, _i, _i, _i, _i, _i, _i, _f, _vp],
+    "lap_rope_split_bwd_rows": [_vp, _vp, _vp, _vp, _vp, _vp, _i, _i, _i, _i, _i, _i, _f, _vp],
     "lap_geglu_fwd": [_vp, _vp, _i, _i, _vp],
     "lap_geglu_bwd": [_vp, _vp, _vp, _i, _i, _vp],
     "lap_geglu_fwd_ld": [_vp, _vp, _i, _i, _i, _i, _vp],
@@ -148,6 +151,7 @@
     "lap_add_bf16": [_vp, _vp, _vp, _ll, _vp],
     "lap_copy2d_bf16": [_vp, _vp, _i, _i, _i, _i, _vp],
     "lap_copy_rows_bf16": [_vp, _vp, _i, _i, _i, _i, _i, _i, _i, _i, _vp],
+    "lap_gather_rows_bf16": [_vp, _vp, _vp, _i, _i, _vp],
     "lap_im2col_patch": [_vp, _vp, _i, _i, _i, _i, _i, _vp],
     "lap_augment_images": [_vp, _vp, _vp, _i, _i, _i, _vp],
     "lap_add_posemb_cast": [_vp, _vp, _vp, _i, _i, _i, _vp],
@@ -414,10 +418,26 @@
     return y, rstd
 
 
-def rmsnorm_bwd(x, dy, rstd, scale=None, mod=None, rows_per_sample=0, dx=None, dscale=None, dmod=None, accum_dx=False):
+def _row_map(t, n, name):
+    _req(t, torch.int32, name)
+    if t.dim() != 1 or t.numel() != n or not t.is_contiguous():
+        raise ValueError(f"{name}: expected a contiguous int32 [{n}] tensor, got shape {tuple(t.shape)}")
+
+
+def rmsnorm_bwd(x, dy, rstd, scale=None, mod=None, rows_per_sample=0, dx=None, dscale=None, dmod=None, accum_dx=False, add_row=None,
+                addend=None):
     rows, D = x.shape
     if dx is None:
         dx = torch.empty_like(x)
+    if add_row is not None:
+        if mod is not None or accum_dx or addend is None or scale is None or dscale is None:
+            raise ValueError("rmsnorm_bwd: add_row goes with scale / dscale and an addend, not with mod or accum_dx")
+        _row_map(add_row, rows, "add_row")
+        _req(addend, torch.bfloat16, "addend")
+        if addend.dim() != 2 or addend.shape[1] != D or not addend.is_contiguous() or not dx.is_contiguous() or dx.shape != x.shape:
+            raise ValueError(f"rmsnorm_bwd: addend {tuple(addend.shape)} / dx {tuple(dx.shape)} do not fit x {tuple(x.shape)}")
+        call("lap_rmsnorm_bwd_rows", _p(x), _p(scale), _p(rstd), _p(dy), _p(dx), _p(dscale), _p(add_row), _p(addend), rows, D)
+        return dx
     call("lap_rmsnorm_bwd", _p(x), _p(scale), _p(mod), _p(rstd), _p(dy), _p(dx), _p(dscale), _p(dmod), rows, D,
          rows_per_sample, mod.stride(0) if mod is not None else 0, dmod.stride(0) if dmod is not None else 0,
          int(accum_dx))
@@ -442,19 +462,30 @@
     return dx
 
 
-def rope_split_fwd(qkv, pos, B, T_seg, T_total, seg_off, NH, HD, q_scale):
+def rope_split_fwd(qkv, pos, B, T_seg, T_total, seg_off, NH, HD, q_scale, q_row=None, q_rows=0):
     rows = B * T_seg
-    q = torch.empty((rows, NH * HD), dtype=torch.bfloat16, device=qkv.device)
+    q = torch.empty((rows if q_row is None else q_rows, NH * HD), dtype=torch.bfloat16, device=qkv.device)
     k = torch.empty((rows, HD), dtype=torch.bfloat16, device=qkv.device)
     v = torch.empty((rows, HD), dtype=torch.bfloat16, device=qkv.device)
-    call("lap_rope_split_fwd", _p(qkv), _p(pos), _p(q), _p(k), _p(v), B, T_seg, T_total, seg_off, NH, HD, float(q_scale))
+    if q_row is not None:
+        _row_map(q_row, rows, "q_row")
+        if q_rows <= 0:
+            raise ValueError("rope_split_fwd: q_row needs q_rows, the height of the compact q")
+        call("lap_rope_split_fwd_rows", _p(qkv), _p(pos), _p(q_row), _p(q), _p(k), _p(v), B, T_seg, T_total, seg_off, NH, HD, float(q_scale))
+    else:
+        call("lap_rope_split_fwd", _p(qkv), _p(pos), _p(q), _p(k), _p(v), B, T_seg, T_total, seg_off, NH, HD, float(q_scale))
     return q, k, v
 
 
-def rope_split_bwd(dq, dk, dv, pos, B, T_seg, T_total, seg_off, NH, HD, q_scale):
+def rope_split_bwd(dq, dk, dv, pos, B, T_seg, T_total, seg_off, NH, HD, q_scale, q_row=None):
     dqkv = torch.empty((B * T_seg, (NH + 2) * HD), dtype=torch.bfloat16, device=dq.device)
-    call("lap_rope_split_bwd", _p(dq), _p(dk), _p(dv), _p(pos), _p(dqkv), B, T_seg, T_total, seg_off, NH, HD,
-         float(q_scale))
+    if q_row is not None:
+        _row_map(q_row, B * T_seg, "q_row")
+        call("lap_rope_split_bwd_rows", _p(dq), _p(dk), _p(dv), _p(pos), _p(q_row), _p(dqkv), B, T_seg, T_total, seg_off, NH, HD,
+             float(q_scale))
+    else:
+        call("lap_rope_split_bwd", _p(dq), _p(dk), _p(dv), _p(pos), _p(dqkv), B, T_seg, T_total, seg_off, NH, HD,
+             float(q_scale))
     return dqkv
 
 
@@ -618,6 +649,17 @@
 
 def copy_rows_bf16(src, dst, rows, T, D, src_rps, src_off, dst_rps, dst_off, accumulate=False):
     call("lap_copy_rows_bf16", _p(src), _p(dst), rows, T, D, src_rps, src_off, dst_rps, dst_off, int(accumulate))
+
+
+def gather_rows_bf16(src, idx):
+    _req(src, torch.bfloat16, "src")
+    n = idx.numel()
+    _row_map(idx, n, "idx")
+    if src.dim() != 2 or not src.is_contiguous():
+        raise ValueError(f"gather_rows_bf16: src must be a contiguous [rows, D] tensor, got {tuple(src.shape)}")
+    out = torch.empty((n, src.shape[1]), dtype=torch.bfloat16, device=src.device)
+    call("lap_gather_rows_bf16", _p(src), _p(idx), _p(out), n, src.shape[1])
+    return out
 
 
 def im2col_patch(img, P):
diff --git a/lap_amd/loss.py b/lap_amd/loss.py
--- a/lap_amd/loss.py
+++ b/lap_amd/loss.py
@@ -40,11 +40,19 @@
     logit_chunks: list = None
     Lt: int = 0
     verbose_metrics: dict = {}
-
-
-def lang_head_fwd(model, xf0, obs, observation, B, Pn, *, backward: bool, verbose: bool, collect) -> LangHead:
+    compact: bool = False
+
+
+class LossRows(NamedTuple):
+    lm: torch.Tensor
+    cnt: torch.Tensor
+    sel: torch.Tensor = None
+    hint_too_small: torch.Tensor = None
+    cls_masks: list = None
+
+
+def select_loss_rows(model, obs, observation, *, verbose: bool) -> LossRows:
     dev = model.device
-    Dv, V = model.v.width, model.config.vocab_size
     Lt = obs.tokenized_prompt.shape[1]
     loss_mask = obs.tokenized_langact_mask[:, 1:] & obs.tokenized_prompt_mask[:, 1:]
     if obs.token_loss_mask is not None:
@@ -66,16 +74,28 @@
             if mk is not None:
                 row_mask = row_mask | mk
         n_sel = observation.metric_rows_max if observation.metric_rows_max is not None else obs.metric_rows_max
-    sel = rowid = None
+    sel = hint_too_small = None
     if n_sel is not None and 0 < n_sel < Lt - 1:
         sel = torch.sort((~row_mask).to(torch.uint8), dim=1, stable=True).indices[:, :n_sel]
         hint_too_small = ((row_mask.sum(-1) if verbose else lm.sum(-1)) > n_sel).any()
-        Ls = n_sel
+    return LossRows(lm, cnt, sel, hint_too_small, cls_masks if verbose else None)
+
+
+def lang_head_fwd(model, xf0, obs, lr: LossRows, B, Pn, *, backward: bool, verbose: bool, collect, compact: bool = False) -> LangHead:
+    dev = model.device
+    Dv, V = model.v.width, model.config.vocab_size
+    Lt = obs.tokenized_prompt.shape[1]
+    lm, cnt, sel, hint_too_small, cls_masks = lr
+    rowid = None
+    if sel is not None:
+        Ls = sel.shape[1]
         rowid = (torch.arange(B, device=dev) * Pn + (Pn - Lt))[:, None] + sel
-        rows = xf0.index_select(0, rowid.view(-1))
+        rows = xf0 if compact else xf0.index_select(0, rowid.view(-1))
         targets = obs.tokenized_prompt[:, 1:].gather(1, sel).to(torch.int32).contiguous().view(-1)
         lm_s = lm.gather(1, sel)
     else:
+        if compact:
+            raise ValueError("lang_head_fwd: compact rows need a row selection")
         Ls = Lt - 1
         rows = torch.empty((B * Ls, Dv), dtype=torch.bfloat16, device=dev)
         hip.copy_rows_bf16(xf0, rows, B * Ls, Ls, Dv, Pn, Pn - Lt, Ls, 0)
@@ -104,7 +124,8 @@
         verbose_metrics = _token_metrics(model, amax, targets, nll, lm, sel, cls_masks, obs.tokenized_prompt[:, 1:])
         if collect is not None:
             collect["predictions"], collect["sel"] = amax.view(B, Ls), sel
-    return LangHead(lang_loss, lm, lm_s, cnt, sel, rowid, rows, pl, rstd_pl, targets, m, lsum, chunks, logit_chunks, Lt, verbose_metrics)
+    return LangHead(lang_loss, lm, lm_s, cnt, sel, rowid, rows, pl, rstd_pl, targets, m, lsum, chunks, logit_chunks, Lt, verbose_metrics,
+                    compact)
 
 
 def _token_metrics(model, amax, targets, nll, lm, sel, cls_masks, labels):
@@ -141,6 +162,8 @@
         del dlogits
     dpl = hip.cast_f32_to_bf16(dpl32[:R] + dpl32[R:])
     drows = hip.rmsnorm_bwd(head.rows, dpl, head.rstd_pl, scale=model.F("llm/final_norm"), dscale=model.G("llm/final_norm"))
+    if head.compact:
+        return drows
     dx0 = torch.zeros((B * Pn, Dv), dtype=torch.bfloat16, device=dev)
     if head.sel is not None:
         dx0.index_copy_(0, head.rowid.view(-1), drows)
diff --git a/lap_amd/model.py b/lap_amd/model.py
--- a/lap_amd/model.py
+++ b/lap_amd/model.py
@@ -9,7 +9,8 @@
 
 from lap_amd import hip
 from lap_amd.config import LAPConfig, get_gemma_config, get_siglip_config
-from lap_amd.loss import ActionHead, LangHead, action_head_bwd, action_head_fwd, lang_head_bwd, lang_head_fwd, mix_sample_weights
+from lap_amd.loss import (ActionHead, LangHead, action_head_bwd, action_head_fwd, lang_head_bwd, lang_head_fwd, mix_sample_weights,
+                          select_loss_rows)
 from lap_amd.observation import CoTObservation, preprocess_observation
 from lap_amd.params import LORA_PROJ, ParamStore, lora_geometry
 from lap_amd.serve_cache import ServeCache
@@ -33,6 +34,18 @@
     g = torch.Generator(device=device)
     g.manual_seed(int(rng) if rng is not None else 0)
     return g
+
+
+class LastRows:
+
+    def __init__(self, sel, qinfo, B, n0, Lt):
+        dev, n_sel = sel.device, sel.shape[1]
+        self.n_sel = n_sel
+        idx = sel + (n0 - Lt)
+        self.rowid = (torch.arange(B, device=dev)[:, None] * n0 + idx).to(torch.int32).reshape(-1).contiguous()
+        self.inv = torch.full((B * n0,), -1, dtype=torch.int32, device=dev)
+        self.inv[self.rowid.long()] = torch.arange(B * n_sel, dtype=torch.int32, device=dev)
+        self.qinfo = torch.cat([qinfo[:, :n0].gather(1, idx), qinfo[:, n0:]], 1).to(torch.int32).contiguous()
 
 
 class LAP:
@@ -65,6 +78,8 @@
         self.fuse_geglu_bwd = os.environ.get("LAP_FUSE_GEGLU_BWD", "1") != "0" and gemm_dtype != "fp8"
         self.fuse_geglu_fwd = os.environ.get("LAP_FUSE_GEGLU_FWD", "1") != "0" and gemm_dtype != "fp8"
         self.fuse_gelu = os.environ.get("LAP_FUSE_GELU", "1") != "0"
+        self.last_layer_rows = os.environ.get("LAP_LAST_LAYER_ROWS", "1") != "0"
+        self.last_rows_steps = 0
         self.serve_overlap = os.environ.get("LAP_SERVE_OVERLAP", "0") != "0"
         self.serve_chain = os.environ.get("LAP_SERVE_CHAIN", "1") != "0"
         self.serve_packed = os.environ.get("LAP_SERVE_PACKED", "1") != "0"
@@ -271,14 +286,22 @@
             self._w8[name] = ent
         return ent[1:]
 
-    def _lin0(self, x, name, residual=None, out=None):
+    def _lin0(self, x, name, residual=None, out=None, tile=-1):
         if self.gemm_dtype == "fp8":
             x8, sx = hip.quantize_fp8(x)
             w8, _, sw = self._w8_of(name)
             return hip.gemm_fp8(x8, sx, w8, sw, residual=residual)
         if residual is not None and os.environ.get("LAP_UNFUSED_RESIDUAL", "0") == "1":
             return hip.add_bf16(residual, hip.linear_fwd(x, self.W(name)))
-        return hip.linear_fwd(x, self.W(name), out, residual=residual)
+        return hip.linear_fwd(x, self.W(name), out, residual=residual, tile=tile)
+
+    def _rows_res_tile(self, x, name):
+        if os.environ.get("LAP_GEMM_NO_ASM") is not None or os.environ.get("LAP_GEMM_NO_ASM_RES") is not None or \
+                os.environ.get("LAP_UNFUSED_RESIDUAL", "0") == "1":
+            return -1
+        w = self.W(name)
+        ok = hip._lib.lap_gemm_asm_res_ok(0, x.shape[0], w.shape[0], x.shape[1], x.stride(0), w.stride(0), w.shape[0])
+        return 14 if ok and x.stride(1) == 1 else -1
 
     def _dgrad0(self, dy, name):
         if self.gemm_dtype == "fp8":
@@ -644,8 +667,17 @@
         W3 = 3 * self.e.width
         return mod[:, slot * W3:(slot + 1) * W3]
 
+    def _last_layer_rows(self, lr, qinfo, B, n0, Lt, *, save, x1, collect, verbose):
+        if not (self.last_layer_rows and save and x1 is not None and collect is None and not verbose and lr is not None
+                and lr.sel is not None and self.gemm_dtype == "bf16" and not self._prefix_frozen()):
+            return None
+        p = f"llm/{self.v.depth - 1}/"
+        if any(self._lora(p + k) is not None for k in ("wqkv0", "wo0", "wgu0", "wd0")):
+            return None
+        return LastRows(lr.sel, qinfo, B, n0, Lt)
+
     def _llm_fwd(self, x0, x1, mod, pos, qinfo, kinfo, B, n0, n1, save: bool, kv_cache=None, cache_out=None, collect=None,
-                 mod_shared: bool = False, layers=None):
+                 mod_shared: bool = False, layers=None, last_rows=None):
         v, e = self.v, self.e
         NH, HD, KV = v.num_heads, v.head_dim, v.num_kv_heads
         Ttot = pos.shape[1]
@@ -654,16 +686,23 @@
         sfx = self._suffix_stream(*([x1, mod] if mod is not None else [x1])) if (x0 is not None and x1 is not None) else None
         main = torch.cuda.current_stream() if sfx is not None else None
         on_sfx = (lambda: torch.cuda.stream(sfx)) if sfx is not None else contextlib.nullcontext
+        if last_rows is not None and not (save and x0 is not None and x1 is not None and layers is None and collect is None):
+            raise ValueError("_llm_fwd: last_rows goes with a saved two-stream pass over all layers without `collect`")
         for l in (range(v.depth) if layers is None else layers):
             self.comm.wait_unit(f"llm{l}", also=sfx)
             p = f"llm/{l}/"
+            rows0 = last_rows if l == v.depth - 1 else None
             q = [None, None]; k = [None, None]; vv = [None, None]; h = [None, None]; rstd_a = [None, None]
             lt = [{}, {}]
             if x0 is not None:
                 h[0], rstd_a[0] = hip.rmsnorm_fwd(x0, scale=self.F(p + "n_attn"), save_rstd=save)
                 qkv = self._lin0(h[0], p + "wqkv0")
                 lt[0]["wqkv"] = self._lora_fwd(h[0], qkv, p + "wqkv0")
-                q[0], k[0], vv[0] = hip.rope_split_fwd(qkv, pos, B, n0, Ttot, 0, NH, HD, HD ** -0.5)
+                if rows0 is None:
+                    q[0], k[0], vv[0] = hip.rope_split_fwd(qkv, pos, B, n0, Ttot, 0, NH, HD, HD ** -0.5)
+                else:
+                    q[0], k[0], vv[0] = hip.rope_split_fwd(qkv, pos, B, n0, Ttot, 0, NH, HD, HD ** -0.5, q_row=rows0.inv,
+                                                           q_rows=B * rows0.n_sel)
                 del qkv
             elif kv_cache is not None:
                 k[0], vv[0] = kv_cache[l]
@@ -682,7 +721,12 @@
                 cache_out.append((k[0], vv[0]))
             qlen = [n0 if x0 is not None else 0, n1 if x1 is not None else 0]
             klen = [k[0].shape[0] // B if k[0] is not None else 0, n1 if x1 is not None else 0]
-            o, lse = hip.attention_fwd(q, k, vv, qlen, klen, B, NH, KV, HD, qinfo, kinfo, need_lse=save)
+            xfull = x0
+            if rows0 is not None:
+                qlen[0] = rows0.n_sel
+                x0 = hip.gather_rows_bf16(x0, rows0.rowid)
+                self.last_rows_steps += 1
+            o, lse = hip.attention_fwd(q, k, vv, qlen, klen, B, NH, KV, HD, qinfo if rows0 is None else rows0.qinfo, kinfo, need_lse=save)
             self._handoff(main, sfx, o[1])
             xa = [None, None]; y1 = None; hf = [None, None]; rstd_f = [None, None]; gu = [None, None]; act = [None, None]; y1f = None
             xn = [None, None]
@@ -709,7 +753,7 @@
                     lt[1]["wd"] = self._lora_fwd(act[1], y1f, p + "wd1")
                     xn[1] = hip.gated_residual_fwd(xa[1], y1f, self._mod_slot(mod, 2 * l + 1)[:, 2 * e.width:], n1, mld)
             if x0 is not None:
-                xa[0] = self._lin0(o[0], p + "wo0", residual=x0)
+                xa[0] = self._lin0(o[0], p + "wo0", residual=x0, tile=-1 if rows0 is None else self._rows_res_tile(o[0], p + "wo0"))
                 lt[0]["wo"] = self._lora_fwd(o[0], xa[0], p + "wo0")
                 hf[0], rstd_f[0] = hip.rmsnorm_fwd(xa[0], scale=self.F(p + "n_ffw"), save_rstd=save)
                 self.comm.pace(f"llm{l}")
@@ -722,10 +766,10 @@
                     gu[0] = self._lin0(hf[0], p + "wgu0", out=gu_out)
                     lt[0]["wgu"] = self._lora_fwd(hf[0], gu[0], p + "wgu0")
                     act[0] = hip.geglu_fwd(gu[0], pad=self.gemm_dtype != "fp8")
-                xn[0] = self._lin0(act[0], p + "wd0", residual=xa[0])
+                xn[0] = self._lin0(act[0], p + "wd0", residual=xa[0], tile=-1 if rows0 is None else self._rows_res_tile(act[0], p + "wd0"))
                 lt[0]["wd"] = self._lora_fwd(act[0], xn[0], p + "wd0")
             if save:
-                ctx.append(dict(x=[x0, x1], h=h, rstd_a=rstd_a, q=q, k=k, v=vv, o=o, lse=lse, xa=xa, y1=y1, hf=hf, rstd_f=rstd_f,
+                ctx.append(dict(x=[xfull, x1], h=h, rstd_a=rstd_a, q=q, k=k, v=vv, o=o, lse=lse, xa=xa, y1=y1, hf=hf, rstd_f=rstd_f,
                                 gu=gu, act=act, y1f=y1f, lt=lt))
             x0, x1 = xn
             if collect is not None:
@@ -780,7 +824,7 @@
                 x0, h = hip.fused_reduce_norm(part, ks, rows, Dv, residual=xa, norm=0)
         return x0
 
-    def _llm_bwd(self, ctx, dx0, dx1, mod, dmod, pos, qinfo, kinfo, B, n0, n1):
+    def _llm_bwd(self, ctx, dx0, dx1, mod, dmod, pos, qinfo, kinfo, B, n0, n1, last_rows=None):
         v, e = self.v, self.e
         NH, HD, KV = v.num_heads, v.head_dim, v.num_kv_heads
         Ttot = pos.shape[1]
@@ -795,6 +839,7 @@
             p = f"llm/{l}/"
             c = ctx[l]
             d_o = [None, None]
+            rows0 = last_rows if l == v.depth - 1 else None
             slot_f, slot_a = 2 * l + 1, 2 * l
             if has_sfx and not ada:
                 with on_sfx():
@@ -853,7 +898,8 @@
                     zero_do0 = torch.zeros_like(c["o"][0])
                 d_o[0] = zero_do0
             self._handoff(sfx, main, d_o[1])
-            dq, dk, dv = hip.attention_bwd(c["q"], c["k"], c["v"], c["o"], d_o, c["lse"], [n0, n1], [n0, n1], B, NH, KV, HD, qinfo, kinfo,
+            dq, dk, dv = hip.attention_bwd(c["q"], c["k"], c["v"], c["o"], d_o, c["lse"], [n0 if rows0 is None else rows0.n_sel, n1], [n0, n1],
+                                           B, NH, KV, HD, qinfo if rows0 is None else rows0.qinfo, kinfo,
                                            stop_q1_to_k0=self.config.stop_action_to_vlm_grad)
             self._handoff(main, sfx, dq[1], dk[1], dv[1])
             if has_sfx:
@@ -869,12 +915,17 @@
                         hip.rmsnorm_bwd(c["x"][1], dh, c["rstd_a"][1], scale=self.F(p + "n_attn1"), dx=dx1, dscale=self.G(p + "n_attn1"), accum_dx=True)
                     del dqkv, dh
             if dx0 is not None:
-                dqkv = hip.rope_split_bwd(dq[0], dk[0], dv[0], pos, B, n0, Ttot, 0, NH, HD, HD ** -0.5)
+                dqkv = hip.rope_split_bwd(dq[0], dk[0], dv[0], pos, B, n0, Ttot, 0, NH, HD, HD ** -0.5,
+                                          q_row=None if rows0 is None else rows0.inv)
                 self._wgrad(dqkv, c["h"][0], p + "wqkv0")
                 dh = self._dgrad0(dqkv, p + "wqkv0")
                 self._lora_bwd(dqkv, c["h"][0], c["lt"][0].get("wqkv"), dh, p + "wqkv0")
-                self._wg_join(dx0)
-                hip.rmsnorm_bwd(c["x"][0], dh, c["rstd_a"][0], scale=self.F(p + "n_attn"), dx=dx0, dscale=self.G(p + "n_attn"), accum_dx=True)
+                if rows0 is None:
+                    self._wg_join(dx0)
+                    hip.rmsnorm_bwd(c["x"][0], dh, c["rstd_a"][0], scale=self.F(p + "n_attn"), dx=dx0, dscale=self.G(p + "n_attn"), accum_dx=True)
+                else:
+                    dx0 = hip.rmsnorm_bwd(c["x"][0], dh, c["rstd_a"][0], scale=self.F(p + "n_attn"), dscale=self.G(p + "n_attn"),
+                                          add_row=rows0.inv, addend=dx0)
                 del dqkv, dh
             ctx[l] = None
             self._unit_done(f"llm{l}", sfx)
@@ -960,14 +1011,17 @@
         qinfo, kinfo, pos = self._train_infos(obs, S if act_on else 0)
         if collect is not None:
             collect["x0_in"], collect["x1_in"], collect["pos"], collect["mod"] = x0, x1, pos, mod
-        xf0, xf1, lctx = self._llm_fwd(x0, x1, mod, pos, qinfo, kinfo, B, Pn, Sx, backward, collect=collect)
+        lrows = select_loss_rows(self, obs, observation, verbose=verbose) if lang_on else None
+        last_rows = self._last_layer_rows(lrows, qinfo, B, Pn, obs.tokenized_prompt.shape[1], save=backward, x1=x1, collect=collect,
+                                          verbose=verbose)
+        xf0, xf1, lctx = self._llm_fwd(x0, x1, mod, pos, qinfo, kinfo, B, Pn, Sx, backward, collect=collect, last_rows=last_rows)
         if collect is not None:
             collect["x0_out"], collect["x1_out"] = xf0, xf1
 
         fb = lambda t: t.to(torch.float32)
         sm = obs.sample_mask if obs.sample_mask is not None else torch.ones(B, dtype=torch.bool, device=dev)
-        head = lang_head_fwd(self, xf0, obs, observation, B, Pn, backward=backward, verbose=verbose, collect=collect) if lang_on else \
-            LangHead(torch.zeros(B, dtype=torch.float32, device=dev))
+        head = lang_head_fwd(self, xf0, obs, lrows, B, Pn, backward=backward, verbose=verbose, collect=collect,
+                             compact=last_rows is not None) if lang_on else LangHead(torch.zeros(B, dtype=torch.float32, device=dev))
         ah = action_head_fwd(self, xf1, mod, B, S, Sx, backward=backward) if act_on else ActionHead()
         lang_loss, v_t = head.lang_loss, ah.v_t
         wl, act_mask, mixing, extra_metrics = mix_sample_weights(
@@ -1007,7 +1061,7 @@
             dx0 = torch.zeros((B * Pn, self.v.width), dtype=torch.bfloat16, device=dev)
             if self.ps.is_trainable("llm/embed"):
                 self.G("llm/embed").zero_()
-        dx0, dx1 = self._llm_bwd(lctx, dx0, dx1, mod, dmod, pos, qinfo, kinfo, B, Pn, Sx)
+        dx0, dx1 = self._llm_bwd(lctx, dx0, dx1, mod, dmod, pos, qinfo, kinfo, B, Pn, Sx, last_rows=last_rows)
         sfx = None
         if act_on and cfg.pi05:
             sfx = self._embed_suffix_bwd(sctx, dx1, dmod)
```

New measurement: 125.9 samples/s, median of 6. +3.1%, better.
